# TheClimateCorporation/photon-ml

Measured on AMD Instinct MI355X. Metric: examples/sec/node, logistic L-BFGS 1B×1M-sparse, higher is better.
Workload: dtype bf16; 1 GPU; model=logistic_regression_l2_lbfgs, global_batch=125000000, rows_per_gpu=125000000, features=1000000, nnz_per_row=100, parallelism=dp1, optimizer_state=replicated, layout=tiled

## Files before the change

photon_ml_amd/data/synthetic.py:

```python
from __future__ import annotations

import math
from typing import Optional

import numpy as np
import scipy.sparse as sp
import torch

from ..constants import TaskType
from .matrix import LabeledData


INLIER_PROBABILITY = 0.90
INLIER_STANDARD_DEVIATION = 1e-3
OUTLIER_STANDARD_DEVIATION = 1.0
SAMPLE_KINDS = ("benign", "outlier", "invalid_features", "invalid_labels")


def draw_samples(task, kind: str, seed: int, size: int, dimensionality: int,
                 desired_sparsity: float = 0.1) -> LabeledData:
    task = TaskType.parse(task)
    if kind not in SAMPLE_KINDS:
        raise ValueError(f"unknown sample kind {kind!r}, expected one of {SAMPLE_KINDS}")
    rng = np.random.default_rng(5000 * seed)
    n, d = int(size), int(dimensionality)
    u = rng.random(n)
    binary = task in (TaskType.LOGISTIC_REGRESSION, TaskType.SMOOTHED_HINGE_LOSS_LINEAR_SVM)
    if kind == "invalid_labels":
        y = np.array([np.inf, -np.inf, np.nan])[rng.integers(0, 3, n)]
        x0 = 0.1 + 0.9 * u
    elif binary:
        y = (rng.random(n) <= 0.5).astype(np.float64)
        x0 = np.where(y == 1.0, 1.0, -1.0) * (0.1 + 0.9 * u)
    elif task == TaskType.POISSON_REGRESSION:
        y = 1.0 + 10.0 * u
        x0 = (np.log(y) + rng.normal(size=n) * INLIER_STANDARD_DEVIATION) / np.log(11.0)
    elif kind == "benign":
        y = 2.0 * u - 1.0
        x0 = y + rng.normal(size=n) * INLIER_STANDARD_DEVIATION
    else:
        y = 1.0 + u
        x0 = y - 1.0 + rng.normal(size=n) * OUTLIER_STANDARD_DEVIATION
    tail_end = d - 3 if kind == "invalid_features" else d
    mask = rng.random((n, max(tail_end - 1, 0))) < desired_sparsity
    rows, cols = np.nonzero(mask)
    cols = cols + 1
    k = rows.size
    if kind in ("benign", "invalid_labels"):
        vals = 2.0 * (rng.random(k) - 0.5)
    else:
        inlier = rng.random(k) < INLIER_PROBABILITY
        if kind == "outlier":
            bad = np.where(rng.random(k) < 0.5, 1.0, -1.0)
        else:
            bad = np.array([np.nan, np.inf, -np.inf])[rng.integers(0, 3, k)]
        vals = np.where(inlier, rng.normal(size=k) * INLIER_STANDARD_DEVIATION, bad)
    r_all = [np.arange(n), rows]
    c_all = [np.zeros(n, np.int64), cols]
    v_all = [x0, vals]
    if kind == "invalid_features":
        for j, v in zip((d - 3, d - 2, d - 1), (np.nan, np.inf, -np.inf)):
            r_all.append(np.arange(n))
            c_all.append(np.full(n, j))
            v_all.append(np.full(n, v))
    x = sp.csr_matrix((np.concatenate(v_all), (np.concatenate(r_all), np.concatenate(c_all))), shape=(n, d))
    x.sort_indices()
    return LabeledData(x, y)


def generate_glm_data(task, n_rows: int, n_features: int, density: float = 0.2, seed: int = 7,
                      intercept: bool = True, noise: float = 1e-3, kind: str = "benign"):
    task = TaskType.parse(task)
    rng = np.random.default_rng(seed)
    d_feat = n_features - (1 if intercept else 0)
    x = sp.random(n_rows, d_feat, density=density, format="csr", random_state=seed,
                  data_rvs=lambda k: rng.uniform(-1, 1, size=k))
    if kind == "outlier":
        x.data *= np.where(rng.random(x.data.size) < 0.01, 1e3, 1.0)
    if intercept:
        x = sp.hstack([x, np.ones((n_rows, 1))], format="csr")
    w = rng.normal(size=n_features)
    z = x @ w
    if task == TaskType.LOGISTIC_REGRESSION or task == TaskType.SMOOTHED_HINGE_LOSS_LINEAR_SVM:
        y = (rng.random(n_rows) < 1.0 / (1.0 + np.exp(-z))).astype(np.float64)
    elif task == TaskType.POISSON_REGRESSION:
        w *= 0.2
        z = x @ w
        y = rng.poisson(np.exp(np.clip(z, -20, 5))).astype(np.float64)
    else:
        y = z + rng.normal(scale=noise, size=n_rows)
    if kind == "invalid":
        y[0] = np.nan
    return LabeledData(x, y), w


def zipf_cdf(n: int, s: float, device) -> torch.Tensor:
    k = torch.arange(1, n + 1, dtype=torch.float64, device=device)
    p = k.pow(-s)
    c = torch.cumsum(p, 0)
    return (c / c[-1]).to(torch.float32)


def generate_device_shard(n_rows: int, n_features: int, nnz_per_row: int, device="cuda", precision: str = "bf16",
                          seed: int = 1234567890, chunk_rows: int = 1 << 20, zipf_s: float = 1.1,
                          task=TaskType.LOGISTIC_REGRESSION, rank: int = 0, progress=None, layout: str = "auto"):
    from ..ops.device import DeviceGLMData, SegChunk, VAL_DTYPE, resolve_layout
    from ..ops.tiled import TLFwdChunk, TLTChunk, shard_tall

    dev = torch.device(device)
    prec = {"bf16": 0, "f32": 1, "f64": 2}[precision]
    vdt = VAL_DTYPE[prec]
    n_fields = nnz_per_row - 1
    if n_fields < 1:
        raise ValueError("nnz_per_row must be >= 2 (intercept + >= 1 field)")
    fs = (n_features - 1) // n_fields
    if fs < 1:
        raise ValueError("not enough features for the requested nnz per row")
    layout = resolve_layout(layout, n_features, chunk_rows)
    cdf = zipf_cdf(fs, zipf_s, dev)
    field_base = (torch.arange(n_fields, device=dev, dtype=torch.int32) * fs)
    gen = torch.Generator(device=dev)
    gen.manual_seed(seed + 7919 * rank)
    starts = list(range(0, n_rows, chunk_rows)) + [n_rows]
    k = nnz_per_row
    raw = []
    counts = torch.zeros(n_features, dtype=torch.int64, device=dev)
    for ci, (a, b) in enumerate(zip(starts[:-1], starts[1:])):
        m = b - a
        u = torch.rand((m, n_fields), generator=gen, device=dev)
        rank_ = torch.searchsorted(cdf, u).clamp_(max=fs - 1).to(torch.int32)
        del u
        idx = torch.empty((m, k), dtype=torch.int32, device=dev)
        idx[:, :n_fields] = rank_ + field_base
        idx[:, n_fields] = n_features - 1
        del rank_
        val = torch.empty((m, k), dtype=torch.float32, device=dev)
        val[:, :n_fields] = torch.rand((m, n_fields), generator=gen, device=dev) + 0.5
        val[:, n_fields] = 1.0
        idx = idx.reshape(-1)
        counts += torch.bincount(idx.to(torch.int64), minlength=n_features)
        raw.append((idx, val.to(vdt).reshape(-1)))
        if (m + 1) * k >= 2 ** 31:
            raise ValueError("chunk too large for int32 offsets: lower chunk_rows")
    import torch.distributed as dist
    from ..parallel.dist import is_dist
    if is_dist():
        cc = counts if dist.get_backend() == "nccl" else counts.cpu()
        dist.all_reduce(cc)
        counts = cc.to(dev)
    old_of_new = torch.argsort(counts, descending=True, stable=True)
    new_of_old = torch.empty_like(old_of_new)
    new_of_old[old_of_new] = torch.arange(n_features, device=dev)
    new_of_old32 = new_of_old.to(torch.int32)
    del counts
    csr, csc = [], []
    from ..ops.tiled import shard_t_config
    cbits, item_entries = shard_t_config(n_rows * k, n_rows, n_features, chunk_rows)
    for ci, ((a, b), (idx, val)) in enumerate(zip(zip(starts[:-1], starts[1:]), raw)):
        m = b - a
        idx = new_of_old32[idx.to(torch.int64)]
        if layout == "tiled":
            rp = torch.arange(0, (m + 1) * k, k, dtype=torch.int64, device=dev)
            col = idx.to(torch.int64)
            del idx
            csr.append(TLFwdChunk(rp, col, val, n_features, tall=shard_tall(n_features, min(chunk_rows, n_rows))))
            csc.append(TLTChunk(rp, col, val, n_features, chunk_rows, cbits=cbits, item_entries=item_entries))
            raw[ci] = None
            del col, val, rp
            if progress is not None:
                progress(ci + 1, len(starts) - 1)
            continue
        seg_ptr = np.arange(0, (m + 1) * k, k, dtype=np.int64).astype(np.int32)
        csr.append(SegChunk(seg_ptr, idx, val, dev, forward=True))
        perm = torch.argsort(idx, stable=True)
        cidx = (perm // k).to(torch.int32)
        cval = val[perm]
        colptr = torch.zeros(n_features + 1, dtype=torch.int64, device=dev)
        colptr[1:] = torch.cumsum(torch.bincount(idx.to(torch.int64), minlength=n_features), 0)
        del perm
        csc.append(SegChunk(colptr.cpu().numpy().astype(np.int32), cidx, cval, dev))
        raw[ci] = None
        del cidx, cval, colptr, idx, val
        if progress is not None:
            progress(ci + 1, len(starts) - 1)
    y = torch.zeros(n_rows, dtype=torch.float32, device=dev)
    data = DeviceGLMData(csr, csc, starts, y, torch.zeros_like(y), torch.ones_like(y), n_features, precision, dev,
                         old_of_new)
    wgen = torch.Generator(device=dev)
    wgen.manual_seed(seed)
    w_true = torch.randn(n_features, generator=wgen, device=dev, dtype=torch.float64) * 0.3
    w_true[torch.rand(n_features, generator=wgen, device=dev) < 0.5] = 0.0
    w_true[-1] = -1.0
    z = data.margins(w_true)
    p = torch.sigmoid(z)
    task = TaskType.parse(task)
    if task == TaskType.LOGISTIC_REGRESSION:
        yy = (torch.rand(n_rows, generator=gen, device=dev, dtype=torch.float64) < p).to(torch.float32)
    elif task == TaskType.POISSON_REGRESSION:
        yy = torch.poisson(torch.exp(z.clamp(max=5.0)) * 0.2, generator=gen).to(torch.float32)
    else:
        yy = (z + 0.1 * torch.randn(n_rows, generator=gen, device=dev, dtype=torch.float64)).to(torch.float32)
    data.y.copy_(yy.to(data.vdt))
    return data, w_true


def _device_csr_to_host(counts: torch.Tensor, cols: torch.Tensor, vals: torch.Tensor, n_cols: int) -> sp.csr_matrix:
    indptr = torch.zeros(counts.numel() + 1, dtype=torch.int64, device=counts.device)
    torch.cumsum(counts, 0, out=indptr[1:])
    x = sp.csr_matrix((vals.cpu().numpy(), cols.to(torch.int32).cpu().numpy(), indptr.cpu().numpy()),
                      shape=(counts.numel(), n_cols))
    x.has_canonical_format = True
    return x


def generate_game_bench_data_device(n_entities: int, rows_per_entity: int, re_dim: int = 100, re_nnz: int = 10,
                                    fe_dim: int = 100_000, fe_nnz: int = 30, re_vocab: int = 1 << 20, seed: int = 7,
                                    entity_offset: int = 0, task: str = "LOGISTIC_REGRESSION", pool: str = "random",
                                    int_ids: bool = False, sizes: str = "uniform", size_alpha: float = 1.3,
                                    max_rows: int = 20000, device="cuda", label_bias: float = 0.0,
                                    heavy_rows=()):
    from ..data.game_data import GameData
    dev = torch.device(device)
    gen = torch.Generator(device=dev)
    gen.manual_seed(int(seed))
    rnd = lambda *shape: torch.rand(shape, generator=gen, device=dev, dtype=torch.float64)
    if sizes == "powerlaw":
        if pool == "exact":
            raise ValueError("pool='exact' needs equal entity sizes")
        u = rnd(n_entities)
        target = n_entities * rows_per_entity
        xm = float(rows_per_entity) * (size_alpha - 1) / size_alpha
        for _ in range(30):
            cnt = torch.clamp(torch.ceil(xm * u ** (-1.0 / size_alpha)), max=max_rows).to(torch.int64)
            tot = int(cnt.sum())
            if abs(tot - target) <= 0.001 * target:
                break
            xm *= target / tot
    elif sizes == "uniform":
        cnt = torch.full((n_entities,), rows_per_entity, dtype=torch.int64, device=dev)
    else:
        raise ValueError(f"unknown entity size law {sizes!r}")
    if len(heavy_rows):
        cnt[:len(heavy_rows)] = torch.tensor([int(r) for r in heavy_rows], dtype=torch.int64, device=dev)
    n = int(cnt.sum())
    ent_sorted = torch.repeat_interleave(torch.arange(n_entities, device=dev), cnt, output_size=n)
    perm = torch.randperm(n, generator=gen, device=dev)
    ent = ent_sorted[perm]
    p = torch.arange(1, fe_dim, device=dev, dtype=torch.float64) ** -1.1
    cdf = torch.cumsum(p, 0)
    cdf /= cdf[-1].clone()
    fcol = torch.searchsorted(cdf, rnd(n, fe_nnz)).clamp_(max=fe_dim - 2)
    fcol, _ = torch.sort(fcol, dim=1)
    keep = torch.ones_like(fcol, dtype=torch.bool)
    keep[:, 1:] = fcol[:, 1:] != fcol[:, :-1]
    fval = rnd(n, fe_nnz) + 0.5
    fcol = torch.cat([fcol, torch.full((n, 1), fe_dim - 1, device=dev, dtype=fcol.dtype)], 1)
    fval = torch.cat([fval, torch.ones(n, 1, device=dev, dtype=torch.float64)], 1)
    keep = torch.cat([keep, torch.ones(n, 1, device=dev, dtype=torch.bool)], 1)
    xg = _device_csr_to_host(keep.sum(1), fcol[keep], fval[keep], fe_dim)
    wg = torch.randn(fe_dim, generator=gen, device=dev, dtype=torch.float64) * 0.2
    wg[-1] = -0.5
    zg = (fval * wg[fcol] * keep).sum(1)
    del fcol, fval, keep
    if pool == "exact":
        if re_nnz > re_dim:
            raise ValueError("pool='exact' needs re_nnz <= re_dim")
        start = torch.zeros(n_entities, dtype=torch.int64, device=dev)
        torch.cumsum(cnt[:-1], 0, out=start[1:])
        within = perm - start[ent]
        slot = (within[:, None] * re_nnz + torch.arange(re_nnz, device=dev)[None, :]) % re_dim
        del within, start
    else:
        slot = torch.randint(0, re_dim, (n, re_nnz), generator=gen, device=dev)
    del ent_sorted, perm
    gid = ent + entity_offset
    base = (gid * 2654435761) % (re_vocab - 1)
    rcol = (base[:, None] + slot * 40503) % (re_vocab - 1)
    rval = torch.randn(n, re_nnz, generator=gen, device=dev, dtype=torch.float64)
    wgen = torch.Generator(device=dev)
    wgen.manual_seed(int(seed) + 1)
    w_slot = torch.randn(re_dim, generator=wgen, device=dev, dtype=torch.float64) * 0.5
    rcol, order = torch.sort(rcol, dim=1)
    slot = torch.gather(slot, 1, order)
    rval = torch.gather(rval, 1, order)
    del order
    rkeep = torch.ones_like(rcol, dtype=torch.bool)
    rkeep[:, 1:] = rcol[:, 1:] != rcol[:, :-1]
    zr = (rval * w_slot[slot] * rkeep).sum(1) + 0.3 * torch.sin(gid.to(torch.float64))
    del slot
    rcol = torch.cat([rcol, torch.full((n, 1), re_vocab - 1, device=dev, dtype=rcol.dtype)], 1)
    rval = torch.cat([rval, torch.ones(n, 1, device=dev, dtype=torch.float64)], 1)
    rkeep = torch.cat([rkeep, torch.ones(n, 1, device=dev, dtype=torch.bool)], 1)
    xr = _device_csr_to_host(rkeep.sum(1), rcol[rkeep], rval[rkeep], re_vocab)
    del rcol, rval, rkeep
    z = zg + zr
    task = TaskType.parse(task)
    if task == TaskType.LOGISTIC_REGRESSION:
        y = (rnd(n) < torch.sigmoid(z + label_bias)).to(torch.float64)
    elif task == TaskType.POISSON_REGRESSION:
        y = torch.poisson(torch.exp(torch.clamp(z * 0.3, -10, 3)), generator=gen)
    else:
        y = z + 0.1 * torch.randn(n, generator=gen, device=dev, dtype=torch.float64)
    gid_h = gid.cpu().numpy()
    ids = gid_h.copy() if int_ids else np.char.add("e", gid_h.astype(str)).astype(object)
    return GameData(y.cpu().numpy(), {"global": xg, "entity": xr}, {"entityId": ids})


def generate_game_bench_data(n_entities: int, rows_per_entity: int, re_dim: int = 100, re_nnz: int = 10,
                             fe_dim: int = 100_000, fe_nnz: int = 30, re_vocab: int = 1 << 20, seed: int = 7,
                             entity_offset: int = 0, task: str = "LOGISTIC_REGRESSION", pool: str = "random",
                             int_ids: bool = False, sizes: str = "uniform", size_alpha: float = 1.3,
                             max_rows: int = 20000):
    from ..data.game_data import GameData
    rng = np.random.default_rng(seed)
    if sizes == "powerlaw":
        if pool == "exact":
            raise ValueError("pool='exact' needs equal entity sizes")
        u = rng.random(n_entities)
        target = n_entities * rows_per_entity
# ... 74 lines not shown
```

photon_ml_amd/ops/csrc/glm_kernels.hip:

```cpp

#include <hip/hip_runtime.h>
#include <stdint.h>
#include <math.h>
#include <algorithm>
#include <type_traits>

#define NB 4096
#define NTHREADS 256
#define VEC 8
#define MAXSEG 1024

#define LAUNCH_CHECK()                                         \
  do {                                                         \
    hipError_t e_ = hipGetLastError();                         \
    if (e_ != hipSuccess) return (int)e_;                      \
  } while (0)

enum LossId { LOSS_LOGISTIC = 0, LOSS_POISSON = 1, LOSS_SQUARED = 2, LOSS_HINGE = 3 };
enum FwdMode { FWD_MARGIN = 0, FWD_VALUE_GRAD = 1, FWD_HV = 2, FWD_DZZ = 3, FWD_LS = 4 };

struct bf16x8 { uint4 u; };

template <typename VT, typename AT> struct Loader;
template <> struct Loader<uint16_t, float> {
// ... 989 lines not shown
  if (live && !live[b]) return;
  const int* q = blk + 8 * b;
  const unsigned long long* pc = ptrs + 6 * q[0];
  const TLNarrow nar = {(const uint16_t*)pc[2], (const void*)pc[3], (const int*)pc[4], (const int*)pc[5]};
  tl_fwd_block<VT, XT, RT, AT, MAXR, U, NW, P>(b, q[1], q[2], q[3], q[4], q[6], q[7], rbits, (const uint32_t*)pc[0],
                                              (const VT*)pc[1], nar, x + q[5], a, stats, acc, red);
}

#define TL_TALL_BITS 12
#define TL_TALL_SUB 10
template <typename VT, typename XT, typename RT, int PT>
__device__ __forceinline__ void tl_fwd_tall_block(int row_lo, int nrows, int e_lo, int e_hi,
                                                  const int* __restrict__ nq ,
                                                  const uint32_t* __restrict__ pack, const VT* __restrict__ val,
                                                  const TLNarrow& nar, const XT* __restrict__ x,
                                                  const FwdArgs<XT, RT>& a, double* __restrict__ stats, double* acc) {
  constexpr int NW = 4;
  for (int i = threadIdx.x; i < (1 << TL_TALL_BITS); i += NW * 64) acc[i] = 0.0;
  __syncthreads();
  const int w = __builtin_amdgcn_readfirstlane(threadIdx.x >> 6);
  const int n_lo = w == 0 ? nq[0] : nq[1 + w], n_hi = w == NW - 1 ? nq[1] : nq[2 + w];
  if (n_hi > n_lo)
    tl_narrow<VT, XT, double, false, 1, (PT >= 5 ? 4 : 2)>(nar, n_lo, n_hi, TL_TALL_SUB, x, acc + (w << TL_TALL_SUB));
  __syncthreads();
  if (w == 0) {
    if (PT == 6) tl_stream_ring<VT, XT, double, false, 1, 5, 2>(pack, val, x, e_lo, e_hi, TL_TALL_BITS, acc, nar.wbase);
    else if (PT == 5) tl_stream_ring<VT, XT, double, false, 1, 3, 1>(pack, val, x, e_lo, e_hi, TL_TALL_BITS, acc, nar.wbase);
    else tl_stream_ring<VT, XT, double, false, 1, 2, 0>(pack, val, x, e_lo, e_hi, TL_TALL_BITS, acc, nar.wbase);
  }
  __syncthreads();
  const int t = ((w & 1) << 6) | (threadIdx.x & 63);
  double Fk[2], Sk[2];
#pragma unroll
  for (int j = 0; j < 2; ++j) {
    const int k0 = ((w >> 1) * 2 + j) << TL_TALL_SUB;
    const int nk = min(nrows - k0, 1 << TL_TALL_SUB);
    double F = 0.0, S = 0.0;
    for (int r = k0 + t; r < k0 + nk; r += 128) {
      const int s = row_lo + r;
      fwd_finish(a, s, acc[r], fwd_prefetch(a, s), F, S);
    }
    Fk[j] = F; Sk[j] = S;
  }
  if (stats) {
    const int sb = nq[5];
#pragma unroll
    for (int j = 0; j < 2; ++j) { Fk[j] = wave_sum(Fk[j]); Sk[j] = wave_sum(Sk[j]); }
    __syncthreads();
    if ((threadIdx.x & 63) == 0) {
#pragma unroll
      for (int j = 0; j < 2; ++j) {
        const int k = (w >> 1) * 2 + j;
        acc[4 * k + 2 * (w & 1)] = Fk[j]; acc[4 * k + 2 * (w & 1) + 1] = Sk[j];
      }
    }
    __syncthreads();
    const int k = threadIdx.x;
    if (k < 4 && (k << TL_TALL_SUB) < nrows) {
      double F = 0.0, S = 0.0;
      for (int i = 0; i < 2; ++i) { F += acc[4 * k + 2 * i]; S += acc[4 * k + 2 * i + 1]; }
      stats[2 * (sb + k)] = F; stats[2 * (sb + k) + 1] = S;
    }
  }
}

template <typename VT, typename XT, typename RT, int PT>
__global__ __launch_bounds__(256) void tl_fwd_tall_kernel(const int* __restrict__ blk,
                                                           const uint32_t* __restrict__ pack,
                                                           const VT* __restrict__ val, TLNarrow nar,
                                                           const XT* __restrict__ x, FwdArgs<XT, RT> a,
                                                           double* __restrict__ stats,
                                                           const unsigned char* __restrict__ live) {
  __shared__ double acc[1 << TL_TALL_BITS];
  const int b = blockIdx.x;
  if (live && !live[b]) return;
  const int* q = blk + 10 * b;
  tl_fwd_tall_block<VT, XT, RT, PT>(q[0], q[1], q[2], q[3], q + 4, pack, val, nar, x, a, stats, acc);
}

template <typename VT, typename XT, typename RT, int PT>
__global__ __launch_bounds__(256) void tl_fwd_tall_multi_kernel(const int* __restrict__ blk,
                                                                 const unsigned long long* __restrict__ ptrs,
                                                                 const XT* __restrict__ x, FwdArgs<XT, RT> a,
                                                                 double* __restrict__ stats,
                                                                 const unsigned char* __restrict__ live) {
  __shared__ double acc[1 << TL_TALL_BITS];
  const int b = blockIdx.x;
  if (live && !live[b]) return;
  const int* q = blk + 12 * b;
  const unsigned long long* pc = ptrs + 6 * q[0];
  const TLNarrow nar = {(const uint16_t*)pc[2], (const void*)pc[3], (const int*)pc[4], (const int*)pc[5]};
  tl_fwd_tall_block<VT, XT, RT, PT>(q[1], q[2], q[3], q[4], q + 6, (const uint32_t*)pc[0], (const VT*)pc[1], nar,
                                    x + q[5], a, stats, acc);
}

template <typename VT, typename XT, typename AT, bool SQ, int MAXR, int U, int NW, int P>
__device__ __forceinline__ void tl_t_item(int tile, int e_lo, int e_hi, int part, int n_lo, int n_hi, int cbits,
                                          const uint32_t* __restrict__ pack, const VT* __restrict__ val,
                                          const TLNarrow& nar, const XT* __restrict__ x, double* __restrict__ G,
                                          int dim, double* __restrict__ parts, AT (*acc)[MAXR]) {
  const int C = 1 << cbits;
  for (int i = threadIdx.x; i < C; i += NW * 64)
#pragma unroll
    for (int w = 0; w < NW; ++w) acc[w][i] = AT(0);
  __syncthreads();
  if (n_hi > n_lo)
    tl_narrow<VT, XT, AT, SQ, NW, (P >= 5 ? 4 : 2)>(nar, n_lo, n_hi, cbits, x, acc[threadIdx.x >> 6]);
  tl_stream<VT, XT, AT, SQ, U, NW, P>(pack, val, x, e_lo, e_hi, cbits, acc[threadIdx.x >> 6], nar.wbase);
  __syncthreads();
  const int c0 = tile << cbits;
  for (int c = threadIdx.x; c < C; c += NW * 64) {
    double s = static_cast<double>(acc[0][c]);
#pragma unroll
    for (int w = 1; w < NW; ++w) s += static_cast<double>(acc[w][c]);
    if (part < 0) {
      if (c0 + c < dim) G[c0 + c] += s;
    } else {
      parts[(size_t)part * C + c] = s;
    }
  }
}

template <typename VT, typename XT, typename AT, bool SQ, int MAXR, int U, int NW, int P>
__global__ __launch_bounds__(NW * 64) void tl_t_kernel(const int* __restrict__ items, int cbits,
                                                        const uint32_t* __restrict__ pack,
                                                        const VT* __restrict__ val, TLNarrow nar,
                                                        const XT* __restrict__ x, double* __restrict__ G, int dim,
                                                        double* __restrict__ parts,
                                                        const unsigned char* __restrict__ live) {
  __shared__ AT acc[NW][MAXR];
  if (live && !live[blockIdx.x]) return;
  const int* q = items + 6 * blockIdx.x;
  tl_t_item<VT, XT, AT, SQ, MAXR, U, NW, P>(q[0], q[1], q[2], q[3], q[4], q[5], cbits, pack, val, nar, x, G, dim,
                                            parts, acc);
}

template <typename VT, typename XT, typename AT, bool SQ, int MAXR, int U, int NW, int P>
__global__ __launch_bounds__(NW * 64) void tl_t_multi_kernel(const int* __restrict__ items, int cbits,
                                                              const unsigned long long* __restrict__ ptrs,
                                                              const XT* __restrict__ x, double* __restrict__ G,
                                                              int dim, double* __restrict__ parts,
                                                              const unsigned char* __restrict__ live,
                                                              const int* __restrict__ gate) {
  __shared__ AT acc[NW][MAXR];
  if (gate && *gate == 0) return;
  if (live && !live[blockIdx.x]) return;
  const int* q = items + 8 * blockIdx.x;
  const unsigned long long* pc = ptrs + 6 * q[0];
  const TLNarrow nar = {(const uint16_t*)pc[2], (const void*)pc[3], (const int*)pc[4], (const int*)pc[5]};
  tl_t_item<VT, XT, AT, SQ, MAXR, U, NW, P>(q[1], q[2], q[3], q[4], q[6], q[7], cbits, (const uint32_t*)pc[0],
                                            (const VT*)pc[1], nar, x + q[5], G, dim, parts, acc);
}

__device__ __forceinline__ double rows_sum64(const double* __restrict__ src, int C, int r0, int r1, int c,
                                             double* sh) {
  const int w = threadIdx.x >> 6, lane = threadIdx.x & 63;
  const int n = r1 - r0;
  const int q0 = r0 + (n * w) / 4, q1 = r0 + (n * (w + 1)) / 4;
  double s0 = 0.0, s1 = 0.0, s2 = 0.0, s3 = 0.0;
  if (c < C) {
    int r = q0;
    for (; r + 3 < q1; r += 4) {
      s0 += src[(size_t)r * C + c];
      s1 += src[(size_t)(r + 1) * C + c];
      s2 += src[(size_t)(r + 2) * C + c];
      s3 += src[(size_t)(r + 3) * C + c];
    }
    for (; r < q1; ++r) s0 += src[(size_t)r * C + c];
  }
  sh[w * 64 + lane] = (s0 + s1) + (s2 + s3);
  __syncthreads();
  return (sh[lane] + sh[64 + lane]) + (sh[128 + lane] + sh[192 + lane]);
}

__global__ __launch_bounds__(NTHREADS) void tl_t_combine1_kernel(const int* __restrict__ cu, int cbits,
                                                                 const double* __restrict__ parts,
                                                                 double* __restrict__ l1,
                                                                 const unsigned char* __restrict__ live_mt) {
  __shared__ double sh[NTHREADS];
  const int u = blockIdx.x;
  if (live_mt && !live_mt[cu[3 * u]]) return;
  const int C = 1 << cbits;
  const int c = blockIdx.y * 64 + (threadIdx.x & 63);
  const double s = rows_sum64(parts, C, cu[3 * u + 1], cu[3 * u + 2], c, sh);
  if (threadIdx.x < 64 && c < C) l1[(size_t)u * C + c] = s;
}

__global__ __launch_bounds__(NTHREADS) void tl_t_combine2_kernel(const int* __restrict__ mt_tiles,
                                                                 const int* __restrict__ mt_ptr, int cbits,
                                                                 const double* __restrict__ l1,
                                                                 double* __restrict__ G, int dim,
                                                                 const unsigned char* __restrict__ live_mt) {
  __shared__ double sh[NTHREADS];
  const int t = blockIdx.x;
  if (live_mt && !live_mt[t]) return;
  const int C = 1 << cbits;
  const int c = blockIdx.y * 64 + (threadIdx.x & 63);
  const double s = rows_sum64(l1, C, mt_ptr[t], mt_ptr[t + 1], c, sh);
  if (threadIdx.x < 64 && c < C) {
    const int col = (mt_tiles[t] << cbits) + c;
    if (col < dim) G[col] += s;
  }
}

struct TLFwdDesc { const int* blk; int nblk; int rbits; const uint32_t* pack; const void* val; int il; TLNarrow nar;
                  const unsigned char* live; int tbits; };
struct TLFwdMultiDesc { const int* blk; int nblk; int rbits; const unsigned long long* ptrs; int il;
                       const unsigned char* live; int tbits; };
struct TLTDesc {
  const int* items; int nitems; int cbits; const uint32_t* pack; const void* val;
  const int* mt_tiles; const int* mt_ptr; int nmt; int dim;
  const int* cu; int ncu;
  int nparts_total;
  int il;
  TLNarrow nar;
  const unsigned char* live;
  const unsigned char* live_mt;
};
struct TLTMultiDesc {
  const int* items; int nitems; int cbits; const unsigned long long* ptrs;
  const int* mt_tiles; const int* mt_ptr; int nmt; int dim;
  const int* cu; int ncu; int nparts_total; int il;
  const unsigned char* live;
  const unsigned char* live_mt;
};

static int g_ablate = 0;
static double* g_ls_z0 = nullptr;
static double g_ls_t0 = 0.0, g_ls_tpend = 0.0;
static const int* g_gate = nullptr;
static const double* g_ls_z0_in = nullptr;
static const double* g_ls_zd_in = nullptr;
template <typename A>
static inline A& with_ls_in(A& a) {
  a.z0_in = g_ls_z0_in ? g_ls_z0_in : g_ls_z0;
  a.zd_in = g_ls_zd_in ? g_ls_zd_in : a.z_out;
  return a;
}
template <typename XT>
static FwdArgs<XT, XT> fwd_args(int mode, int loss, double shift, const void* y, const void* off, const void* wt,
                                void* coef, void* dzz, double* z_out, int with_offset) {
  FwdArgs<XT, XT> a{mode, loss, shift, (const XT*)y, (const XT*)off, (const XT*)wt, (XT*)coef, (XT*)dzz, z_out,
                    with_offset, g_ablate, 0, g_ls_z0, g_ls_t0, g_ls_tpend};
  return with_ls_in(a);
}
template <typename F>
static int with_prec(int prec, F f) {
  if (prec == 2) return f(double{}, double{});
  if (prec == 1) return f(float{}, float{});
  return f(uint16_t{}, float{});
}
template <typename F>
static int with_prec_sq(int prec, int square, F f) {
  return with_prec(prec, [&](auto vt, auto xt) {
    return square ? f(vt, xt, std::true_type{}) : f(vt, xt, std::false_type{});
  });
}
static int g_tl_acc64 = 1;
static int g_tl_waves = 4;
static int g_tl_waves_t = 4;
static int g_tl_pipe = 0;
static int g_tl_pipe_t = 0;
static int g_rs_variant = 5;
static int g_tl_deep = 0;
static int g_tl_deep_t = 0;

#ifdef PML_TL_EXPERIMENT
constexpr bool TL_EXPERIMENT = true;
#else
constexpr bool TL_EXPERIMENT = false;
#endif

template <typename AT_, int MAXR_> struct TLAcc { using AT = AT_; static constexpr int MAXR = MAXR_; };
template <int NW_, int P_> struct TLPipe { static constexpr int NW = NW_, P = P_; };

template <typename XT> static inline int tl_maxbits() { return sizeof(XT) == 8 ? 11 : TL_MAXBITS; }
template <typename XT, typename F>
static int tl_with_acc(int bits, F f) {
  if (bits < 1 || bits > tl_maxbits<XT>()) return -22;
  if constexpr (sizeof(XT) != 8) {
    if (bits == 12) { f(TLAcc<float, 4096>{}); return 0; }
    if constexpr (TL_EXPERIMENT) {
      if (!g_tl_acc64) {
        if (bits <= 10) f(TLAcc<float, 1024>{}); else f(TLAcc<float, 2048>{});
        return 0;
      }
    }
  }
  if (bits <= 10) f(TLAcc<double, 1024>{}); else f(TLAcc<double, 2048>{});
  return 0;
}

template <int NW_PROD, int ALT_P, typename F>
static void tl_with_pipe(int il, int waves, int deep, int pipe, F f) {
  if constexpr (!TL_EXPERIMENT) {
    if (il) f(TLPipe<NW_PROD, 3>{}); else f(TLPipe<NW_PROD, 0>{});
  } else {
    auto with_p = [&](auto nw) {
      constexpr int NW = decltype(nw)::value;
      if (il) {
        if (deep == 2) f(TLPipe<NW, 6>{}); else if (deep) f(TLPipe<NW, 5>{}); else f(TLPipe<NW, 3>{});
      } else if (pipe == ALT_P) f(TLPipe<NW, ALT_P>{});
      else f(TLPipe<NW, 0>{});
    };
    if (waves == 2) with_p(std::integral_constant<int, 2>{}); else with_p(std::integral_constant<int, 4>{});
  }
}

#define TL_TALL_P 6
template <typename XT, typename F>
static int tl_with_tall(int tbits, int rbits, int il, F f) {
  if constexpr (sizeof(XT) == 8) {
    return -22;
  } else {
    if (tbits != TL_TALL_BITS || rbits != TL_TALL_SUB || !il) return -22;
    if constexpr (TL_EXPERIMENT) {
      if (g_tl_deep == 2) f(std::integral_constant<int, 6>{});
      else if (g_tl_deep) f(std::integral_constant<int, 5>{});
      else f(std::integral_constant<int, 3>{});
    } else {
      f(std::integral_constant<int, TL_TALL_P>{});
    }
    return 0;
  }
}

template <typename VT, typename XT, typename RT>
static int tl_fwd_impl(const TLFwdDesc* c, const void* x, FwdArgs<XT, RT> a, double* stats, hipStream_t st) {
  if (c->nblk <= 0) return 0;
  if (c->tbits) {
    const int rt = tl_with_tall<XT>(c->tbits, c->rbits, c->il, [&](auto pt) {
      hipLaunchKernelGGL((tl_fwd_tall_kernel<VT, XT, RT, decltype(pt)::value>), dim3(c->nblk), dim3(256), 0, st,
                         c->blk, c->pack, (const VT*)c->val, c->nar, (const XT*)x, a, stats, c->live);
    });
    if (rt) return rt;
    LAUNCH_CHECK();
    return 0;
  }
  const int rc = tl_with_acc<XT>(c->rbits, [&](auto acc) {
    tl_with_pipe<2, 1>(c->il, g_tl_waves, g_tl_deep, g_tl_pipe, [&](auto pipe) {
      using A = decltype(acc); using Q = decltype(pipe);
      hipLaunchKernelGGL((tl_fwd_kernel<VT, XT, RT, typename A::AT, A::MAXR, 2, Q::NW, Q::P>), dim3(c->nblk),
                         dim3(Q::NW * 64), 0, st, c->blk, c->rbits, c->pack, (const VT*)c->val, c->nar, (const XT*)x,
                         a, stats, c->live);
    });
  });
  if (rc) return rc;
  LAUNCH_CHECK();
  return 0;
}

template <typename VT, typename XT, typename RT>
static int tl_fwd_multi_impl(const TLFwdMultiDesc* c, const void* x, FwdArgs<XT, RT> a, double* stats,
                             hipStream_t st) {
  if (c->nblk <= 0) return 0;
  if (c->tbits) {
    const int rt = tl_with_tall<XT>(c->tbits, c->rbits, c->il, [&](auto pt) {
      hipLaunchKernelGGL((tl_fwd_tall_multi_kernel<VT, XT, RT, decltype(pt)::value>), dim3(c->nblk), dim3(256), 0,
                         st, c->blk, c->ptrs, (const XT*)x, a, stats, c->live);
    });
    if (rt) return rt;
    LAUNCH_CHECK();
    return 0;
  }
  const int rc = tl_with_acc<XT>(c->rbits, [&](auto acc) {
    tl_with_pipe<2, 2>(c->il, g_tl_waves, g_tl_deep, g_tl_pipe, [&](auto pipe) {
      using A = decltype(acc); using Q = decltype(pipe);
      hipLaunchKernelGGL((tl_fwd_multi_kernel<VT, XT, RT, typename A::AT, A::MAXR, 2, Q::NW, Q::P>), dim3(c->nblk),
                         dim3(Q::NW * 64), 0, st, c->blk, c->rbits, c->ptrs, (const XT*)x, a, stats, c->live);
    });
  });
  if (rc) return rc;
  LAUNCH_CHECK();
  return 0;
}

template <typename Desc>
static int tl_t_combine(const Desc* c, double* G, double* parts, hipStream_t st) {
  if (c->nmt <= 0) return 0;
  const int C = 1 << c->cbits;
  double* l1 = parts + (size_t)c->nparts_total * C;
  hipLaunchKernelGGL(tl_t_combine1_kernel, dim3(c->ncu, (C + 63) / 64), dim3(NTHREADS), 0, st, c->cu, c->cbits,
                     parts, l1, c->live_mt);
  LAUNCH_CHECK();
  hipLaunchKernelGGL(tl_t_combine2_kernel, dim3(c->nmt, (C + 63) / 64), dim3(NTHREADS), 0, st,
                     c->mt_tiles, c->mt_ptr, c->cbits, l1, G, c->dim, c->live_mt);
  LAUNCH_CHECK();
  return 0;
}

template <typename VT, typename XT, bool SQ>
static int tl_t_impl(const TLTDesc* c, const void* x, double* G, double* parts, hipStream_t st) {
  if (c->nitems <= 0) return 0;
  const int rc = tl_with_acc<XT>(c->cbits, [&](auto acc) {
    tl_with_pipe<4, 1>(c->il, g_tl_waves_t, g_tl_deep_t, g_tl_pipe_t, [&](auto pipe) {
      using A = decltype(acc); using Q = decltype(pipe);
      hipLaunchKernelGGL((tl_t_kernel<VT, XT, typename A::AT, SQ, A::MAXR, 2, Q::NW, Q::P>), dim3(c->nitems),
                         dim3(Q::NW * 64), 0, st, c->items, c->cbits, c->pack, (const VT*)c->val, c->nar, (const XT*)x,
                         G, c->dim, parts, c->live);
    });
  });
  if (rc) return rc;
  LAUNCH_CHECK();
  return tl_t_combine(c, G, parts, st);
}

template <typename VT, typename XT, bool SQ>
static int tl_t_multi_impl(const TLTMultiDesc* c, const void* x, double* G, double* parts, hipStream_t st) {
  if (c->nitems <= 0) return 0;
  const int rc = tl_with_acc<XT>(c->cbits, [&](auto acc) {
    tl_with_pipe<4, 2>(c->il, g_tl_waves_t, g_tl_deep_t, g_tl_pipe_t, [&](auto pipe) {
      using A = decltype(acc); using Q = decltype(pipe);
      hipLaunchKernelGGL((tl_t_multi_kernel<VT, XT, typename A::AT, SQ, A::MAXR, 2, Q::NW, Q::P>), dim3(c->nitems),
                         dim3(Q::NW * 64), 0, st, c->items, c->cbits, c->ptrs, (const XT*)x, G, c->dim, parts, c->live,
                         g_gate);
    });
  });
  if (rc) return rc;
  LAUNCH_CHECK();
  return tl_t_combine(c, G, parts, st);
}

template <typename VT> __device__ __forceinline__ void cs_vals(const typename TLVals<VT>::Raw& raw, double* v) {
  typename TLValT<VT>::T t[TL_VEC];
  TLVals<VT>::get(raw, t);
#pragma unroll
  for (int k = 0; k < TL_VEC; ++k) v[k] = static_cast<double>(t[k]);
}

template <typename VT, int NW, typename F>
__device__ __forceinline__ void cs_for_each(const int* __restrict__ q, int cbits, const uint32_t* __restrict__ pack,
                                            const VT* __restrict__ val, const TLNarrow& nar, int il, F f) {
  typedef typename TLVals<VT>::Raw Raw;
  const int lane = threadIdx.x & 63;
  const int w = __builtin_amdgcn_readfirstlane(threadIdx.x >> 6);
  const uint32_t smask = (1u << cbits) - 1u;
  const int e_lo = q[1], e_hi = q[2], n_lo = q[4], n_hi = q[5];
  double v[TL_VEC];
  {
    const int nr = n_hi - n_lo;
    const int r0 = n_lo + (int)(((long long)nr * w) / NW), r1 = n_lo + (int)(((long long)nr * (w + 1)) / NW);
    bool fused = false;
    if constexpr (sizeof(VT) == 2) fused = nar.val == nullptr;
    for (int r = r0; r < r1; ++r) {
      const size_t e = (size_t)r * TL_ROUND + lane * TL_VEC;
      v2u pk;
      if (fused) {
        if constexpr (sizeof(VT) == 2) {
          const v4u rec = ldg_nt((const v4u*)(nar.pack + 2 * e));
          pk.x = rec.x; pk.y = rec.y;
          v2u u; u.x = rec.z; u.y = rec.w;
          cs_vals<VT>(u, v);
        }
      } else {
        pk = ldg_nt((const v2u*)(nar.pack + e));
        const Raw raw = TLVals<VT>::load((const VT*)nar.val + e);
        cs_vals<VT>(raw, v);
      }
      f(pk.x & 0xffffu & smask, v[0]);
      f((pk.x >> 16) & smask, v[1]);
      f(pk.y & 0xffffu & smask, v[2]);
      f((pk.y >> 16) & smask, v[3]);
    }
  }
  if (il) {
    const int n = e_hi - e_lo;
    const int nr = (n + TL_ROUND - 1) / TL_ROUND;
    const int r0 = (int)(((long long)nr * w) / NW), r1 = (int)(((long long)nr * (w + 1)) / NW);
    for (int r = r0; r < r1; ++r) {
      const size_t e = (size_t)e_lo + (size_t)r * TL_ROUND + lane * TL_VEC;
      const v4u pk = ldg_nt((const v4u*)(pack + e));
      const Raw raw = TLVals<VT>::load(val + e);
      cs_vals<VT>(raw, v);
      const int j = r * TL_ROUND + lane;
#pragma unroll
      for (int k = 0; k < TL_VEC; ++k)
        if (j + 64 * k < n) f(pk[k] & smask, v[k]);
    }
  } else {
    const int lo = e_lo & ~(TL_VEC - 1);
    const int nr = (e_hi - lo + TL_ROUND - 1) / TL_ROUND;
    const int r0 = (int)(((long long)nr * w) / NW), r1 = (int)(((long long)nr * (w + 1)) / NW);
    for (int r = r0; r < r1; ++r) {
      const int e = lo + r * TL_ROUND + lane * TL_VEC;
      if (e >= e_hi) continue;
      const v4u pk = ldg_nt((const v4u*)(pack + e));
      const Raw raw = TLVals<VT>::load(val + e);
      cs_vals<VT>(raw, v);
#pragma unroll
      for (int k = 0; k < TL_VEC; ++k)
        if (e + k >= e_lo && e + k < e_hi) f(pk[k] & smask, v[k]);
    }
  }
}

template <typename VT, int MAXR, int NW>
__global__ __launch_bounds__(NW * 64) void tl_colsum_kernel(const int* __restrict__ items, int cbits,
                                                            const uint32_t* __restrict__ pack,
                                                            const VT* __restrict__ val, TLNarrow nar, int il,
                                                            int which, double* __restrict__ G, int dim,
                                                            double* __restrict__ parts) {
  __shared__ double acc[NW][MAXR];
  const int* q = items + 6 * blockIdx.x;
  const int C = 1 << cbits;
  for (int i = threadIdx.x; i < C; i += NW * 64)
#pragma unroll
    for (int w = 0; w < NW; ++w) acc[w][i] = 0.0;
  __syncthreads();
  double* mine = acc[threadIdx.x >> 6];
  cs_for_each<VT, NW>(q, cbits, pack, val, nar, il, [&](uint32_t slot, double v) {
    const double t = which == 0 ? v : which == 1 ? v * v : which == 2 ? fabs(v) : 1.0;
    atomicAdd(&mine[slot], t);
  });
  __syncthreads();
  const int c0 = q[0] << cbits, part = q[3];
  for (int c = threadIdx.x; c < C; c += NW * 64) {
    double s = acc[0][c];
#pragma unroll
    for (int w = 1; w < NW; ++w) s += acc[w][c];
    if (part < 0) {
      if (c0 + c < dim) G[c0 + c] += s;
    } else {
      parts[(size_t)part * C + c] = s;
    }
  }
}

template <typename VT, int MAXR>
__global__ __launch_bounds__(NTHREADS) void tl_colminmax_kernel(const int* __restrict__ items, int cbits,
                                                                const uint32_t* __restrict__ pack,
                                                                const VT* __restrict__ val, TLNarrow nar, int il,
                                                                double* __restrict__ mx, double* __restrict__ mn,
                                                                int dim) {
  __shared__ double smx[MAXR];
  __shared__ double smn[MAXR];
  const int* q = items + 6 * blockIdx.x;
  const int C = 1 << cbits;
  for (int i = threadIdx.x; i < C; i += NTHREADS) { smx[i] = -INFINITY; smn[i] = INFINITY; }
  __syncthreads();
  cs_for_each<VT, TL_WAVES>(q, cbits, pack, val, nar, il, [&](uint32_t slot, double v) {
    __hip_atomic_fetch_max(&smx[slot], v, __ATOMIC_RELAXED, __HIP_MEMORY_SCOPE_WORKGROUP);
    __hip_atomic_fetch_min(&smn[slot], v, __ATOMIC_RELAXED, __HIP_MEMORY_SCOPE_WORKGROUP);
  });
  __syncthreads();
  const int c0 = q[0] << cbits;
  for (int c = threadIdx.x; c < C; c += NTHREADS) {
    if (c0 + c >= dim || smx[c] == -INFINITY) continue;
    __hip_atomic_fetch_max(&mx[c0 + c], smx[c], __ATOMIC_RELAXED, __HIP_MEMORY_SCOPE_AGENT);
    __hip_atomic_fetch_min(&mn[c0 + c], smn[c], __ATOMIC_RELAXED, __HIP_MEMORY_SCOPE_AGENT);
  }
}

template <typename VT>
static int tl_colstats_impl(const TLTDesc* c, double* const* sums, double* mx, double* mn, double* parts,
                            hipStream_t st) {
  if (c->cbits < 1 || c->cbits > (sizeof(VT) == 8 ? 11 : TL_MAXBITS)) return -22;
  if (c->nitems <= 0) return 0;
  for (int which = 0; which < 4; ++which) {
    auto launch = [&](auto maxr, auto nw) {
      constexpr int MAXR = decltype(maxr)::value, NW = decltype(nw)::value;
      hipLaunchKernelGGL((tl_colsum_kernel<VT, MAXR, NW>), dim3(c->nitems), dim3(NW * 64), 0, st, c->items, c->cbits,
                         c->pack, (const VT*)c->val, c->nar, c->il, which, sums[which], c->dim, parts);
    };
    if (c->cbits <= 10) launch(std::integral_constant<int, 1024>{}, std::integral_constant<int, 4>{});
    else if (c->cbits == 11) launch(std::integral_constant<int, 2048>{}, std::integral_constant<int, 4>{});
    else if constexpr (sizeof(VT) != 8) launch(std::integral_constant<int, 4096>{}, std::integral_constant<int, 2>{});
    LAUNCH_CHECK();
    const int rc = tl_t_combine(c, sums[which], parts, st);
    if (rc) return rc;
  }
  auto launch_mm = [&](auto maxr) {
    constexpr int MAXR = decltype(maxr)::value;
    hipLaunchKernelGGL((tl_colminmax_kernel<VT, MAXR>), dim3(c->nitems), dim3(NTHREADS), 0, st, c->items, c->cbits,
                       c->pack, (const VT*)c->val, c->nar, c->il, mx, mn, c->dim);
  };
  if (c->cbits <= 11) launch_mm(std::integral_constant<int, 2048>{});
  else if constexpr (sizeof(VT) != 8) launch_mm(std::integral_constant<int, 4096>{});
  LAUNCH_CHECK();
  return 0;
}

__global__ __launch_bounds__(NTHREADS) void segdot_kernel(const double* __restrict__ a, const double* __restrict__ b,
                                                          int mode, const long long* __restrict__ ptr, int nseg,
                                                          double* __restrict__ out) {
  const int wv = (blockIdx.x * NTHREADS + threadIdx.x) >> 6;
  const int lane = threadIdx.x & 63;
  if (wv >= nseg) return;
  const long long lo = ptr[wv], hi = ptr[wv + 1];
  double s = 0.0;
  for (long long i = lo + lane; i < hi; i += 64) {
    const double x = a[i];
    s += mode == 0 ? x * b[i] : (mode == 1 ? x : fabs(x));
  }
  s = wave_sum(s);
  if (lane == 0) out[wv] = s;
}

#define SEGDOT_C 4096
__device__ __forceinline__ int seg_of(const long long* __restrict__ ptr, int nseg, long long i) {
  int lo = 0, hi = nseg - 1;
  while (lo < hi) {
    const int mid = (lo + hi + 1) >> 1;
    if (ptr[mid] <= i) lo = mid; else hi = mid - 1;
  }
  return lo;
}

__device__ __forceinline__ double seg_range_sum(const double* __restrict__ a, const double* __restrict__ b, int mode,
                                                long long lo, long long hi, int lane) {
  double s = 0.0;
  for (long long i = lo + lane; i < hi; i += 64) {
    const double x = a[i];
    s += mode == 0 ? x * b[i] : (mode == 1 ? x : fabs(x));
  }
  return wave_sum(s);
}

__global__ __launch_bounds__(NTHREADS) void segdot_long_kernel(const double* __restrict__ a,
                                                               const double* __restrict__ b, int mode,
                                                               const long long* __restrict__ ptr, int nseg,
                                                               int nseg_w, long long n, double* __restrict__ head,
                                                               double* __restrict__ tail, double* __restrict__ out) {
  const int wv = (blockIdx.x * NTHREADS + threadIdx.x) >> 6;
  const int lane = threadIdx.x & 63;
  if (wv < nseg_w) {
    if (wv >= nseg) return;
    const long long lo = ptr[wv], hi = ptr[wv + 1];
    if (hi - lo > SEGDOT_C) return;
    const double s = seg_range_sum(a, b, mode, lo, hi, lane);
    if (lane == 0) out[wv] = s;
    return;
  }
  const long long w = wv - nseg_w;
  const long long c0 = w * SEGDOT_C, c1 = c0 + SEGDOT_C < n ? c0 + SEGDOT_C : n;
  if (c0 >= n) return;
  const int s0 = seg_of(ptr, nseg, c0), s1 = seg_of(ptr, nseg, c1 - 1);
  double h = 0.0, t = 0.0;
  if (ptr[s0 + 1] - ptr[s0] > SEGDOT_C) h = seg_range_sum(a, b, mode, c0, ptr[s0 + 1] < c1 ? ptr[s0 + 1] : c1, lane);
  if (s1 != s0 && ptr[s1 + 1] - ptr[s1] > SEGDOT_C) t = seg_range_sum(a, b, mode, ptr[s1], c1, lane);
  if (lane == 0) { head[w] = h; tail[w] = t; }
}

__global__ __launch_bounds__(NTHREADS) void segdot_combine_kernel(const long long* __restrict__ ptr, int nseg,
                                                                  const double* __restrict__ head,
                                                                  const double* __restrict__ tail,
                                                                  double* __restrict__ out) {
  const int s = blockIdx.x * NTHREADS + threadIdx.x;
  if (s >= nseg) return;
  const long long lo = ptr[s], hi = ptr[s + 1];
  if (hi - lo <= SEGDOT_C) return;
  const long long w0 = lo / SEGDOT_C, w1 = (hi - 1) / SEGDOT_C;
  double acc = lo == w0 * SEGDOT_C ? head[w0] : tail[w0];
  for (long long w = w0 + 1; w <= w1; ++w) acc += head[w];
  out[s] = acc;
}

template <typename T>
__global__ __launch_bounds__(NTHREADS) void seg_expand_kernel(const long long* __restrict__ ptr, int nseg,
                                                              const T* __restrict__ src, T* __restrict__ out) {
  const int e = (blockIdx.x * NTHREADS + threadIdx.x) >> 6;
  const int lane = threadIdx.x & 63;
  if (e >= nseg) return;
  const long long lo = ptr[e], hi = ptr[e + 1];
  const T v = src[e];
  for (long long i = lo + lane; i < hi; i += 64) out[i] = v;
}

__global__ __launch_bounds__(NTHREADS) void seg_cg_step_kernel(const long long* __restrict__ ptr, int nseg,
                                                               double* __restrict__ step, double* __restrict__ r,
                                                               double* __restrict__ d, const double* __restrict__ Hd,
                                                               double* __restrict__ rtr, unsigned char* __restrict__ on,
                                                               const double* __restrict__ delta, double l2) {
  const int e = (blockIdx.x * NTHREADS + threadIdx.x) >> 6;
  const int lane = threadIdx.x & 63;
  if (e >= nseg || !on[e]) return;
  const long long lo = ptr[e], hi = ptr[e + 1];
  double dhd = 0.0, std_ = 0.0, sts = 0.0, dtd = 0.0;
  for (long long i = lo + lane; i < hi; i += 64) {
    const double di = d[i], si = step[i];
    dhd += di * (Hd[i] + l2 * di);
    std_ += si * di;
    sts += si * si;
    dtd += di * di;
  }
  dhd = wave_sum(dhd); std_ = wave_sum(std_); sts = wave_sum(sts); dtd = wave_sum(dtd);
  const double rt = rtr[e];
  const double alpha = rt / (dhd == 0.0 ? 1.0 : dhd);
  double tn = 0.0;
  for (long long i = lo + lane; i < hi; i += 64) {
    const double t = step[i] + alpha * d[i];
    tn += t * t;
  }
  tn = wave_sum(tn);
  const double dl = delta[e];
  const bool hit = sqrt(tn > 0.0 ? tn : 0.0) > dl;
  double a = alpha;
  if (hit) {
    const double dsq = dl * dl;
    const double q = std_ * std_ + dtd * (dsq - sts);
    const double rad = sqrt(q > 0.0 ? q : 0.0);
    const double den1 = std_ + rad, den2 = dtd;
    a = std_ >= 0.0 ? (dsq - sts) / (den1 > 1e-300 ? den1 : 1e-300) : (rad - std_) / (den2 > 1e-300 ? den2 : 1e-300);
  }
  double rn = 0.0;
  for (long long i = lo + lane; i < hi; i += 64) {
    const double di = d[i];
    step[i] = step[i] + a * di;
    const double ri = r[i] - a * (Hd[i] + l2 * di);
    r[i] = ri;
// ... 2085 lines not shown
```

photon_ml_amd/ops/device.py:

```python
from __future__ import annotations

import ctypes
import os
import threading
from dataclasses import dataclass
from typing import List, Optional, Sequence

import numpy as np
import scipy.sparse as sp
import torch

from ..data.matrix import LabeledData
from .native import SegChunkDesc, check, require_glm_lib, stream_handle
from .reference import GLMComputable
from .tiled import DEFAULT_ITEM_ENTRIES, TLFwdChunk, TLTChunk, shard_tall, tl_supported
from ..utils.timing import phase, trace_range

H2D_GATE = threading.Event()

LAYOUTS = ("auto", "tiled", "segmented")


def resolve_layout(layout: str, dim: int, chunk_rows: int) -> str:
    import os
    if layout == "auto":
        layout = os.environ.get("PML_LAYOUT", "auto")
    if layout not in LAYOUTS:
        raise ValueError(f"unknown layout {layout}")
    if layout == "auto":
        layout = "tiled" if tl_supported(dim, chunk_rows) else "segmented"
    if layout == "tiled" and not tl_supported(dim, chunk_rows):
        raise ValueError(f"tiled layout cannot pack dim={dim} with chunk_rows={chunk_rows}")
    return layout

PRECISIONS = {"bf16": 0, "f32": 1, "f64": 2}
VAL_DTYPE = {0: torch.bfloat16, 1: torch.float32, 2: torch.float64}
VEC_DTYPE = {0: torch.float32, 1: torch.float32, 2: torch.float64}

FWD_MARGIN, FWD_VALUE_GRAD, FWD_HV, FWD_DZZ, FWD_LS = 0, 1, 2, 3, 4


def _pad8(n: int) -> int:
    return ((n + 7) // 8) * 8 + 8


def _ptr(t: Optional[torch.Tensor]) -> Optional[int]:
    return None if t is None else t.data_ptr()


class SegChunk:

    def __init__(self, seg_ptr: np.ndarray, idx: torch.Tensor, val: torch.Tensor, device, nb: Optional[int] = None,
                 maxseg: Optional[int] = None, forward: bool = False):
        lib = require_glm_lib()
        seg_ptr = np.ascontiguousarray(seg_ptr, dtype=np.int32)
        nseg = len(seg_ptr) - 1
        nb = nb or lib.pml_nb()
        maxseg = maxseg or (lib.pml_maxseg_fwd() if forward else lib.pml_maxseg())
        nblk, nlong, npart = ctypes.c_int(), ctypes.c_int(), ctypes.c_int()
        check(lib.pml_build_blocks(seg_ptr.ctypes.data, nseg, nb, maxseg, None, ctypes.byref(nblk), None, None,
                                   ctypes.byref(nlong), ctypes.byref(npart)), "count blocks")
        blk = np.zeros(max(5 * nblk.value, 5), dtype=np.int32)
        long_seg = np.zeros(max(nlong.value, 1), dtype=np.int32)
        long_ptr = np.zeros(nlong.value + 1, dtype=np.int32)
        check(lib.pml_build_blocks(seg_ptr.ctypes.data, nseg, nb, maxseg, blk.ctypes.data, ctypes.byref(nblk),
                                   long_seg.ctypes.data, long_ptr.ctypes.data, ctypes.byref(nlong),
                                   ctypes.byref(npart)), "build blocks")
        self.nseg, self.nblk, self.nlong, self.npart = nseg, nblk.value, nlong.value, npart.value
        self.nnz = int(seg_ptr[-1])
        dev = torch.device(device)
        self.seg_ptr = torch.from_numpy(seg_ptr).to(dev)
        self.blk = torch.from_numpy(blk).to(dev)
        self.long_seg = torch.from_numpy(long_seg).to(dev)
        self.long_ptr = torch.from_numpy(long_ptr).to(dev)
        n_pad = _pad8(self.nnz)
        if idx.numel() < n_pad:
            idx = torch.cat([idx.to(dev, torch.int32), torch.zeros(n_pad - idx.numel(), dtype=torch.int32, device=dev)])
        if val.numel() < n_pad:
            val = torch.cat([val.to(dev), torch.zeros(n_pad - val.numel(), dtype=val.dtype, device=dev)])
        self.idx = idx.contiguous()
        self.val = val.contiguous()
        self.desc = SegChunkDesc(self.blk.data_ptr(), self.nblk, self.seg_ptr.data_ptr(), self.nseg,
                                 self.idx.data_ptr(), self.val.data_ptr(), self.long_seg.data_ptr(),
                                 self.long_ptr.data_ptr(), self.nlong, self.npart)

    kind = "seg"

    @property
    def nstats(self) -> int:
        return self.nblk

    @property
    def parts_needed(self) -> int:
        return self.npart

    def nbytes(self) -> int:
        return sum(t.numel() * t.element_size() for t in (self.seg_ptr, self.blk, self.long_seg, self.long_ptr,
                                                           self.idx, self.val))


MASK_STATS = [] if os.environ.get("PML_TRON_STATS") == "1" else None

NARROW_FILTER_BELOW = float(os.environ.get("PML_DS_NARROW_FILTER_BELOW", "0.23"))

OFFSET_SHIFT_CACHE = os.environ.get("PML_OFFSET_SHIFT_CACHE", "1") != "0"


class VecKey:

    __slots__ = ("src", "ver")

    def __init__(self, w: torch.Tensor):
        self.src = w
        self.ver = w._version

    @property
    def shape(self):
        return self.src.shape

    def matches(self, w: torch.Tensor) -> bool:
        if w is self.src and w._version == self.ver:
            return True
        if self.src._version != self.ver or self.src.shape != w.shape:
            return False
        return bool(torch.equal(self.src, w.to(self.src.device, self.src.dtype)))


def _window_align(chunk_rows: int, precision: str) -> int:
    from .tiled import t_bits
    cb = t_bits(chunk_rows, precision == "f64")
    return 1 << cb if cb is not None else 1


class DeviceGLMData(GLMComputable):

    def __init__(self, csr: List[SegChunk], csc: List[SegChunk], row_starts: Sequence[int], y, offsets, weights,
                 dim: int, precision: str = "f64", device="cuda", old_of_new: Optional[torch.Tensor] = None):
        self.lib = require_glm_lib()
        self.device = torch.device(device)
        if self.device.type == "cuda":
            from .native import check_lds_add_order
            check_lds_add_order(self.device)
        self.prec = PRECISIONS[precision]
        self.precision = precision
        self.vdt = VEC_DTYPE[self.prec]
        self.csr, self.csc = csr, csc
        self.row_starts = list(row_starts)
        self.n_rows = self.row_starts[-1]
        self.dim = int(dim)
        rdt = self.vdt
        self.y = torch.as_tensor(y, device=self.device).to(rdt).contiguous()
        self.o = torch.as_tensor(offsets, device=self.device).to(rdt).contiguous()
        self.wt = torch.as_tensor(weights, device=self.device).to(rdt).contiguous()
        n = self.n_rows
        self.coef = torch.zeros(max(n, 1), dtype=rdt, device=self.device)
        self.dzz = torch.zeros(max(n, 1), dtype=rdt, device=self.device)
        self.track_hessian = False
        self._dzz_key: Optional[torch.Tensor] = None
        self._dzz_shift = None
        self.layout = "tiled" if csr and csr[0].kind == "tl" else "segmented"
        self.col_lo = [0] * len(csr)
        self.blk_off = np.cumsum([0] + [c.nstats for c in csr]).tolist()
        self.long_off = np.cumsum([0] + [getattr(c, "nlong", 0) for c in csr]).tolist()
        self.stats = torch.zeros(2 * max(self.blk_off[-1], 1), dtype=torch.float64, device=self.device)
        self.long_stats = torch.zeros(2 * max(self.long_off[-1], 1), dtype=torch.float64, device=self.device)
        maxpart = max([c.parts_needed for c in csr + csc] + [1])
        self.parts = torch.zeros(maxpart, dtype=torch.float64, device=self.device)
        self.red_scratch = torch.zeros(512, dtype=torch.float64, device=self.device)
        self.out2 = torch.zeros(2, dtype=torch.float64, device=self.device)
        self.n_passes = 0
        self.old_of_new = None if old_of_new is None else old_of_new.to(self.device, torch.int64)
        if self.old_of_new is not None:
            self.new_of_old = torch.empty_like(self.old_of_new)
            self.new_of_old[self.old_of_new] = torch.arange(self.dim, device=self.device)
        if os.environ.get("PML_CHECK_KERNEL_INPUTS", "0") == "1":
            self.validate()

    def validate(self):
        from .tiled import il_phys
        for c, (f, t) in enumerate(zip(self.csr, self.csc)):
            if f.kind != "tl":
                continue
            m = self.row_starts[c + 1] - self.row_starts[c]
            b = f.blk.cpu().to(torch.int64)
            if f.nblk and (int(b[:, 0].min()) < 0 or int((b[:, 0] + b[:, 1]).max()) > m
                           or int(b[:, 1].max()) > (1 << f.ubits)):
                raise ValueError(f"chunk {c}: forward block rows out of range")
            q = 256 if f.il else 4
            end = b[:, 2] + (b[:, 3] - b[:, 2] + q - 1) // q * q if f.il else (b[:, 3] + 3) // 4 * 4
            if f.nblk and (int(b[:, 2].min()) < 0 or int(end.max()) > f.pack.numel()):
                raise ValueError(f"chunk {c}: forward block window outside the stream")
            if f.il and f.nblk and bool((b[:, 2] % 256 != 0).any()):
                raise ValueError(f"chunk {c}: interleaved forward windows not round-aligned")
            ncols = int(self.dim) - self.col_lo[c]
            self._validate_narrow(c, f, b, ncols, "forward")
            pk, _ = f.logical()
            p = pk.cpu().to(torch.int64)
            wb = getattr(f, "wbase", None)
            if wb is not None and wb.numel() and int(wb.min()) < 0:
                raise ValueError(f"chunk {c}: negative wide-round base")
            if p.numel() and int((p >> f.ubits).max()) >= ncols:
                raise ValueError(f"chunk {c}: forward gather index >= column window")
            counts = f.unit_counts().cpu()
            blk_rows = torch.repeat_interleave(b[:, 1], counts)
            if p.numel() and bool(((p & ((1 << f.ubits) - 1)) >= blk_rows).any()):
                raise ValueError(f"chunk {c}: forward LDS slot >= block rows")
            it = t.items.cpu().to(torch.int64)
            if t.nitems:
                if int(it[:, 1].min()) < 0 or int(it[:, 2].max()) > t.pack.numel():
                    raise ValueError(f"chunk {c}: transpose item window outside the stream")
                if int(it[:, 3].max()) >= max(t.nparts, 1) and t.nparts:
                    raise ValueError(f"chunk {c}: transpose partial-row slot out of range")
                self._validate_narrow(c, t, it, m, "transpose")
                tp, _ = t.logical()
                q = tp.cpu().to(torch.int64) & 0xFFFFFFFF
                if q.numel() and int((q >> t.cbits).max()) >= m:
                    raise ValueError(f"chunk {c}: transpose gather row >= chunk rows")
                cols = (torch.repeat_interleave(it[:, 0], t.unit_counts().cpu()) << t.cbits) + (q & ((1 << t.cbits) - 1))
                if q.numel() and int(cols.max()) >= t.dim:
                    raise ValueError(f"chunk {c}: transpose column >= dim")
        if self.parts.numel() < max([c.parts_needed for c in self.csr + self.csc] + [1]):
            raise ValueError("partial-row scratch too small")
        self._validate_multi()
        return True

    def _validate_multi(self):
        mb = getattr(self, "_multi", None)
        if mb is not None and not isinstance(mb, str):
            t = self._multi_blk.cpu().to(torch.int64)
            for c, ch in enumerate(self.csr):
                r = t[t[:, 0] == c]
                if ch.il and r.shape[0] and (int(r[:, 3].min()) < 0 or int((r[:, 3] + (r[:, 4] - r[:, 3] + 255) // 256 * 256).max())
                                   > ch.pack.numel() or int(r[:, 7].max()) > ch.nbase.numel() * (ch.n_narrow_rounds > 0)):
                    raise ValueError(f"chunk {c}: shard-wide forward table outside the chunk's streams")
        mt = getattr(self, "_multi_t", None)
        if mt is not None and not isinstance(mt, str):
            if self.parts.numel() < mt.parts_needed:
                raise ValueError("partial-row scratch too small for the shard-wide transpose")
            t = mt.items.cpu().to(torch.int64)
            for c, ch in enumerate(self.csc):
                r = t[t[:, 0] == c]
                if ch.il and r.shape[0] and (int(r[:, 2].min()) < 0 or int((r[:, 2] + (r[:, 3] - r[:, 2] + 255) // 256 * 256).max())
                                   > ch.pack.numel() or int(r[:, 7].max()) > ch.nbase.numel() * (ch.n_narrow_rounds > 0)):
                    raise ValueError(f"chunk {c}: shard-wide transpose table outside the chunk's streams")

    @staticmethod
    def _validate_narrow(c: int, ch, table: torch.Tensor, xlen: int, what: str):
        if table.shape[0] == 0:
            return
        n_lo, n_hi = table[:, 4], table[:, 5]
        nrounds = ch.nbase.numel() if ch.n_narrow_rounds else 0
        if bool((n_hi < n_lo).any()) or int(n_hi.max()) > nrounds or bool((n_lo[1:] != n_hi[:-1]).any()):
            raise ValueError(f"chunk {c}: {what} narrow round ranges inconsistent")
        if nrounds:
            base = ch.nbase.cpu().to(torch.int64)
            if ch.npack.numel() < 256 * nrounds or ch.nval.numel() < 256 * nrounds:
                raise ValueError(f"chunk {c}: {what} narrow stream shorter than its rounds")
            if ch.fused and (ch.nrec.numel() < 512 * nrounds or ch.val.element_size() != 2
                             or not ch.nrec.is_contiguous()):
                raise ValueError(f"chunk {c}: {what} fused narrow records need 2-byte values, 16 B per lane and round")
            if int(base.min()) < 0 or int(base.max()) + 64 > xlen:
                raise ValueError(f"chunk {c}: {what} narrow key window outside the gathered vector")

    @staticmethod
    def from_labeled(data: LabeledData, device="cuda", precision: str = "f64", chunk_rows: int = 1 << 20,
                     relabel: bool = True, layout: str = "auto", item_entries: Optional[int] = None,
                     col_windows: bool = False):
        if col_windows:
            relabel = False
        prec = PRECISIONS[precision]
        vdt = VAL_DTYPE[prec]
        dev = torch.device(device)
        x = data.x.tocsr()
        n, d = x.shape
        if dev.type == "cuda" and n and resolve_layout(layout, d, chunk_rows) == "tiled":
            return DeviceGLMData._from_labeled_device(x, data, dev, precision, chunk_rows, relabel, item_entries,
                                                      col_windows)
        if hasattr(x, "to_scipy"):
            x = x.to_scipy()
        old_of_new = None
        from ..parallel.dist import is_dist
        shared = relabel and is_dist() and not col_windows
        if shared or (relabel and x.nnz > 0):
            counts = np.bincount(x.indices, minlength=d).astype(np.int64)
            if shared:
                import torch.distributed as tdist
                from ..parallel.sharding import comm_device
                ct = torch.from_numpy(counts).to(comm_device())
                tdist.all_reduce(ct)
                counts = ct.cpu().numpy()
            old_of_new_np = np.argsort(-counts, kind="stable")
            new_of_old_np = np.empty(d, dtype=np.int64)
            new_of_old_np[old_of_new_np] = np.arange(d)
            x = sp.csr_matrix((x.data, new_of_old_np[x.indices], x.indptr), shape=x.shape)
            old_of_new = torch.from_numpy(old_of_new_np)
        starts = list(range(0, n, chunk_rows)) + [n]
        if n == 0:
            starts = [0, 0]
        csr, csc = [], []
        col_lo = []
        wins = []
        align = _window_align(chunk_rows, precision)
        for a, b in zip(starts[:-1], starts[1:]):
            xc = x[a:b]
            if col_windows and xc.nnz:
                lo, hi = int(xc.indices.min()), int(xc.indices.max()) + 1
                lo -= lo % align
            else:
                lo, hi = 0, d
            wins.append((lo, hi))
        dmax = max([hi - lo for lo, hi in wins] + [1])
        layout = resolve_layout(layout, dmax, chunk_rows)
        cbits = None
        if layout == "tiled" and not col_windows and item_entries is None:
            from .tiled import shard_t_config
            cbits, item_entries = shard_t_config(int(x.nnz), n, d, chunk_rows)
        for (a, b), (lo, hi) in zip(zip(starts[:-1], starts[1:]), wins):
            xc = x[a:b]
            col_lo.append(lo)
            if lo != 0 or hi != d:
                xc = sp.csr_matrix((xc.data, xc.indices - lo, xc.indptr), shape=(b - a, hi - lo))
            dc = hi - lo
            if layout == "tiled":
                rp = torch.from_numpy((xc.indptr - xc.indptr[0]).astype(np.int64)).to(dev)
                col = torch.from_numpy(xc.indices.astype(np.int64)).to(dev)
                val = torch.from_numpy(xc.data.astype(np.float64)).to(dev).to(vdt)
                csr.append(TLFwdChunk(rp, col, val, dc, tall=shard_tall(dmax, min(chunk_rows, n))))
                csc.append(TLTChunk(rp, col, val, dc, chunk_rows, cbits=cbits, item_entries=item_entries))
                continue
            sp_ = (xc.indptr - xc.indptr[0]).astype(np.int32)
            csr.append(SegChunk(sp_, torch.from_numpy(xc.indices.astype(np.int32)),
                                torch.from_numpy(xc.data.astype(np.float64)).to(vdt), dev, forward=True))
            xt = xc.tocsc()
            xt.sort_indices()
            xc = xc.copy()
            csc.append(SegChunk(xt.indptr.astype(np.int32), torch.from_numpy(xt.indices.astype(np.int32)),
                                torch.from_numpy(xt.data.astype(np.float64)).to(vdt), dev))
        out = DeviceGLMData(csr, csc, starts, torch.from_numpy(data.y), torch.from_numpy(data.offsets),
                            torch.from_numpy(data.weights), d, precision, dev, old_of_new)
        out.col_lo = col_lo
        return out

    @staticmethod
    def _from_labeled_device(x, data: LabeledData, dev, precision: str, chunk_rows: int, relabel: bool,
                             item_entries: Optional[int], col_windows: bool):
        n, d = x.shape
        with phase("tiled build: upload"):
            if isinstance(x.indptr, torch.Tensor):
                indptr, col, val = x.indptr.to(dev), x.indices.to(dev).to(torch.int64), x.data.to(dev)
            else:
                indptr = torch.from_numpy(np.ascontiguousarray(x.indptr, dtype=np.int64)).to(dev)
                col = torch.from_numpy(np.ascontiguousarray(x.indices)).to(dev).to(torch.int64)
                val = torch.from_numpy(np.ascontiguousarray(x.data)).to(dev)
        H2D_GATE.set()
        old_of_new = None
        from ..parallel.dist import is_dist
        shared = relabel and is_dist() and not col_windows
        relabel_phase = phase("tiled build: hottest-first relabel")
        relabel_phase.__enter__()
        if shared or (relabel and col.numel() > 0):
            from .native import key_histogram
            counts = key_histogram(col, d)
            if shared:
                import torch.distributed as tdist
                from ..parallel.sharding import comm_device
                ct = counts.to(comm_device())
                tdist.all_reduce(ct)
                counts = ct.to(dev)
            oon = torch.argsort(-counts, stable=True)
            non = torch.empty_like(oon)
            non[oon] = torch.arange(d, device=dev)
            col = non[col]
            old_of_new = (oon, non)
            del counts
        relabel_phase.__exit__(None, None, None)
        out = DeviceGLMData.from_device_csr(indptr, col, val, torch.from_numpy(data.y), torch.from_numpy(data.offsets),
                                            torch.from_numpy(data.weights), d, dev, precision, chunk_rows,
                                            item_entries=item_entries, col_windows=col_windows)
        if old_of_new is not None:
            out.old_of_new, out.new_of_old = old_of_new
        return out

    @staticmethod
    def from_device_csr(indptr: torch.Tensor, col: torch.Tensor, val: torch.Tensor, y, offsets, weights, dim: int,
                        device="cuda", precision: str = "f64", chunk_rows: int = 1 << 20,
                        item_entries: Optional[int] = None, col_windows: bool = False,
                        tall: Optional[bool] = None):
        dev = torch.device(device)
        vdt = VAL_DTYPE[PRECISIONS[precision]]
        indptr = indptr.to(dev, torch.int64)
        col = col.to(dev, torch.int64)
        n = indptr.numel() - 1
        starts = list(range(0, n, chunk_rows)) + [n] if n else [0, 0]
        ip = indptr[torch.tensor(starts, device=dev)].tolist()
        wins = []
        align = _window_align(chunk_rows, precision)
        for i in range(len(starts) - 1):
            ea, eb = ip[i], ip[i + 1]
            if col_windows and eb > ea:
                lo, hi = torch.aminmax(col[ea:eb])
                lo = int(lo)
                wins.append((lo - lo % align, int(hi) + 1))
            else:
                wins.append((0, dim))
        dmax = max([hi - lo for lo, hi in wins] + [1])
        if resolve_layout("auto", dmax, chunk_rows) != "tiled":
            raise ValueError(f"from_device_csr needs the tiled layout (window {dmax} columns)")
        cbits = None
        if not col_windows and item_entries is None:
            from .tiled import shard_t_config
            cbits, item_entries = shard_t_config(int(ip[-1] - ip[0]), n, dim, chunk_rows)
        csr, csc, col_lo = [], [], []
        chunk_phase = phase(f"tiled build: {len(wins)} chunk layouts")
        chunk_phase.__enter__()
        for i, (lo, hi) in enumerate(wins):
            a, b = starts[i], starts[i + 1]
            ea, eb = ip[i], ip[i + 1]
            rp = indptr[a:b + 1] - ea
            c = col[ea:eb] - lo if lo else col[ea:eb]
            v = val[ea:eb].to(dev).to(vdt)
            csr.append(TLFwdChunk(rp, c, v, hi - lo,
                                  tall=shard_tall(dmax, min(chunk_rows, n)) if tall is None else tall))
            csc.append(TLTChunk(rp, c, v, hi - lo, chunk_rows, cbits=cbits, item_entries=item_entries))
            col_lo.append(lo)
            del c, v
        chunk_phase.__exit__(None, None, None)
        out = DeviceGLMData(csr, csc, starts, y, offsets, weights, dim, precision, dev, None)
        out.col_lo = col_lo
        return out

    def nbytes(self) -> int:
        return sum(c.nbytes() for c in self.csr + self.csc)

    def row_sampled(self, keep: torch.Tensor) -> Optional["DeviceGLMData"]:
        from .tiled import RowCompaction, stream_ptr_table
        from .native import TLFwdMultiDesc
        if self.layout != "tiled" or not self.csr or not all(getattr(ch, "il", 0) for ch in self.csr + self.csc):
            return None
        if any(getattr(ch, "wbase", None) is not None for ch in self.csr):
            return None
        keep = keep.to(self.device, torch.uint8).contiguous()
        assert keep.numel() >= self.n_rows
        n = self.n_rows
        if getattr(self, "_multi", "unset") == "unset":
            self._build_multi()
        if getattr(self, "_multi_t", "unset") == "unset":
            self._build_multi_t()
        frac = float(keep[:n].sum()) / max(n, 1)
        filt = frac < NARROW_FILTER_BELOW
        jobs = []
        for c in range(len(self.csr)):
            kc = keep[self.row_starts[c]: self.row_starts[c + 1]]
            jobs.append(RowCompaction(self.csr[c], kc, True, filt))
            jobs.append(RowCompaction(self.csc[c], kc, False, filt))
        sizes = torch.stack([torch.stack([j.total, j.kept]) for j in jobs]).tolist()
        out = [j.finish(int(t), int(k)) for j, (t, k) in zip(jobs, sizes)]
        view = DeviceGLMData(out[0::2], out[1::2], self.row_starts, self.y, self.o, self.wt, self.dim,
                             self.precision, self.device, None)
        view.col_lo = list(self.col_lo)
        view.old_of_new = self.old_of_new
        if self.old_of_new is not None:
            view.new_of_old = self.new_of_old
        view.sampled_from = self
        view.kept_fraction = frac
        view._frob_sq = self.frob_sq()
        if getattr(self, "z_cache", None) is not None and getattr(self, "_z_key", None) is not None:
            view.enable_margin_cache()
            view.z_cache.copy_(self.z_cache)
            view.zd.copy_(self.zd)
            view._z_key, view._z_chain, view._tpend = self._z_key, self._z_chain, self._tpend
        if self._multi is not None:
            nb = self._multi_blk.clone()
            cb = torch.cat([ch.blk for ch in view.csr])
            nb[:, 3:5] = cb[:, 2:4]
            nb[:, 6:6 + min(cb.shape[1], 9) - 4] = cb[:, 4:9]
            view._multi_blk = nb
            view._multi_ptrs = stream_ptr_table(view.csr, self.device)
            view._multi = TLFwdMultiDesc(nb.data_ptr(), nb.shape[0], self._multi.rbits, view._multi_ptrs.data_ptr(),
                                         self._multi.il, tbits=self._multi.tbits)
        view._multi_t = None if self._multi_t is None else self._multi_t.restreamed(view.csc)
        gb = getattr(self, "_gbuckets", None)
        if gb is not None and gb[1] is not None:
            view._gbuckets = (gb[0], [(mt.restreamed(view.csc), c0, c1) for mt, c0, c1 in gb[1]])
        view.parts = self.parts
        if os.environ.get("PML_CHECK_KERNEL_INPUTS", "0") == "1":
            view.validate()
        return view

    def set_offsets_sum(self, base: torch.Tensor, part: torch.Tensor) -> bool:
        n = self.n_rows
        if not (n > 0 and base.is_cuda and part.is_cuda and base.dtype == part.dtype == torch.float64
                and base.numel() == part.numel() == n == self.o.numel() and base.is_contiguous()
                and part.is_contiguous() and base.device == self.o.device == part.device):
            return False
        from .native import offset_update
        zc = getattr(self, "z_cache", None)
        shift = (zc is not None and getattr(self, "_z_key", None) is not None and self._z_chain + 1 < self.LS_REFRESH
                 and getattr(self, "_masked", None) is None and OFFSET_SHIFT_CACHE)
        offset_update(base, part, self.o, zc[:n] if shift else None)
        if shift:
            self._z_chain += 1
            self._ls_t0 = None
        else:
            self._z_key = None
        self._step_base = None
        self._dzz_key = None
        return True

    def set_offsets(self, offsets):
        new = torch.as_tensor(offsets, device=self.device).to(self.vdt)
        zc = getattr(self, "z_cache", None)
        if (zc is not None and getattr(self, "_z_key", None) is not None and self._z_chain + 1 < self.LS_REFRESH
                and getattr(self, "_masked", None) is None and OFFSET_SHIFT_CACHE):
            n = self.n_rows
            zc[:n].add_(new[:n].to(torch.float64) - self.o[:n].to(torch.float64))
            self._z_chain += 1
            self._ls_t0 = None
        else:
            self._z_key = None
        self.o.copy_(new)
        self._step_base = None
        self._dzz_key = None

    def mark_weights_changed(self):
        self._dzz_key = None
        self._ls_t0 = None

    LS_REFRESH = 50

    def enable_margin_cache(self):
        if getattr(self, "z_cache", None) is None:
            n = max(self.n_rows, 1)
            self.z_cache = torch.zeros(n, dtype=torch.float64, device=self.device)
            self.zd = torch.zeros(n, dtype=torch.float64, device=self.device)
            self.ls_stats = torch.zeros(2 * 4096, dtype=torch.float64, device=self.device)
            self.ls_out = torch.zeros(2, dtype=torch.float64, device=self.device)
            self._z_key, self._z_chain, self._tpend, self._ls_t0 = None, 0, 0.0, None
        return True

    def _z_valid_for(self, w_eff, shift) -> bool:
        key = getattr(self, "_z_key", None)
        return (key is not None and key[1] == float(shift) and self._z_chain < self.LS_REFRESH
                and key[0].matches(w_eff))

    def ls_begin(self, w0_eff, shift0, d_eff, d_shift, t0: float = 1.0, loss=None, alt: bool = False,
                 stats_out: Optional[torch.Tensor] = None) -> bool:
        if loss is None:
            return False
        if getattr(self, "z_cache", None) is None:
            if alt:
                return False
            self.enable_margin_cache()
        if not self._z_valid_for(w0_eff, shift0):
            if alt:
                return False
            self.fwd_all(self._vec(w0_eff), FWD_MARGIN, 0, shift0, None, None, z_out=self.z_cache, with_offset=1,
                         stats=False)
            self._z_key, self._z_chain, self._tpend = (VecKey(w0_eff), float(shift0)), 0, 0.0
        if alt:
            from .native import KERNEL_CONFIG
            if getattr(self, "_multi", "unset") == "unset":
                self._build_multi()
            if (self._multi is None or not KERNEL_CONFIG.get("tl_multi", 1)
                    or getattr(self, "_masked", None) is not None):
                return False
        with trace_range("K1' direction pass (margins of d + first trial)"):
            if alt:
                zin, din = self.z_cache, self.zd
                if getattr(self, "_zalt", None) is None:
                    self._zalt = (torch.empty_like(zin), torch.empty_like(din))
                zout, dout = self._zalt
                self.lib.pml_set_ls_in(zin.data_ptr(), din.data_ptr())
            else:
                zout, dout = self.z_cache, self.zd
            self.lib.pml_set_ls_args(zout.data_ptr(), float(t0), float(self._tpend))
            try:
                self.fwd_all(self._vec(d_eff), FWD_LS, loss.loss_id, d_shift, self.coef, None, z_out=dout)
            finally:
                self.lib.pml_set_ls_args(None, 0.0, 0.0)
                if alt:
                    self.lib.pml_set_ls_in(None, None)
            if alt:
                self.z_cache, self.zd, self._zalt = zout, dout, (zin, din)
            self._tpend = 0.0
            self._ls_t0 = float(t0)
            self._coef_stale = False
            if stats_out is None:
                stats_out = torch.empty(2, dtype=torch.float64, device=self.device)
            self._ls_t0_dev = self._reduce_stats(stats_out)
            self._ls_t0_host = None
        return True

    _LS_STATE = ("z_cache", "zd", "_zalt", "_tpend", "_ls_t0", "_ls_t0_dev", "_ls_t0_host", "_z_key", "_z_chain",
                 "_track_u", "_dzz_key", "_dzz_shift", "_coef_stale", "_step_base")

    def ls_checkpoint(self) -> dict:
        return {k: getattr(self, k, None) for k in self._LS_STATE}

    def ls_restore(self, ck: dict, t0_host=None):
        for k, v in ck.items():
            setattr(self, k, v)
        self._coef_stale = True
        if t0_host is not None and self._ls_t0 is not None:
            self._ls_t0_host = tuple(float(v) for v in t0_host)

    @property
    def _ls_t0_vals(self):
        if self._ls_t0_host is None:
            self._ls_t0_host = tuple(self._ls_t0_dev.tolist())
        return self._ls_t0_host

    def _ls(self, loss, t, final, out):
        dzz = self.dzz if (final and self.track_hessian and loss.twice_differentiable) else None
        check(self.lib.pml_ls_eval(self.prec, self.n_rows, float(t), loss.loss_id, self.z_cache.data_ptr(),
                                   self.zd.data_ptr(), self.y.data_ptr(), self.wt.data_ptr(), int(final),
                                   self.coef.data_ptr() if final else None, None if dzz is None else dzz.data_ptr(),
                                   self.ls_stats.data_ptr(), out.data_ptr(), stream_handle(self.device)), "ls_eval")

    def ls_eval(self, loss, t: float):
        if self._ls_t0 is not None and float(t) == self._ls_t0:
            return self._ls_t0_vals
        with trace_range("line-search trial (margin space)"):
            self._ls(loss, t, 0, self.ls_out)
            f, d = self.ls_out.tolist()
        return f, d

    def ls_gate_supported(self) -> bool:
        from .native import KERNEL_CONFIG
        if getattr(self, "_multi_t", "unset") == "unset":
            self._build_multi_t()
        return (self._multi_t is not None and KERNEL_CONFIG.get("tl_multi", 1) and getattr(self, "_masked", None) is None
                and getattr(self, "_ls_t0", None) == 1.0 and not getattr(self, "_coef_stale", False)
                and getattr(self, "_ls_t0_dev", None) is not None and self.z_cache.is_cuda)

    def ls_finish_gated(self, loss, pre: torch.Tensor, f0: float, l2: float, c1: float, c2: float,
# ... 127 lines not shown
    def step_add(self, alpha: float):
        self.zd.add_(self.u_dir, alpha=float(alpha))

    def _u_out(self):
        return self.u_dir if getattr(self, "_track_u", False) else None

    def set_weights(self, weights):
        self.wt.copy_(torch.as_tensor(weights, device=self.device).to(self.vdt))
        self.mark_weights_changed()

    def _rows(self, t: torch.Tensor, c: int) -> int:
        return t.data_ptr() + self.row_starts[c] * t.element_size()

    def _fwd(self, c: int, x: torch.Tensor, mode: int, loss_id: int, shift: float, coef: Optional[torch.Tensor],
             dzz: Optional[torch.Tensor], z_out: Optional[torch.Tensor] = None, with_offset: int = 0,
             stats: bool = True):
        ch = self.csr[c]
        st = self.stats.data_ptr() + 2 * 8 * self.blk_off[c] if stats else None
        xp = x.data_ptr() + self.col_lo[c] * x.element_size()
        if ch.kind == "tl":
            masked = getattr(self, "_masked", None)
            desc = masked[0][c] if masked is not None and isinstance(masked[0], list) else ch.desc
            check(self.lib.pml_tl_fwd(
                self.prec, ctypes.byref(desc), xp, mode, loss_id, float(shift),
                self._rows(self.y, c), self._rows(self.o, c), self._rows(self.wt, c),
                None if coef is None else self._rows(coef, c), None if dzz is None else self._rows(dzz, c),
                None if z_out is None else self._rows(z_out, c), with_offset, st, stream_handle(self.device)),
                "tl_fwd")
            return
        lst = self.long_stats.data_ptr() + 2 * 8 * self.long_off[c] if stats else None
        check(self.lib.pml_seg_fwd(
            self.prec, ctypes.byref(ch.desc), xp, mode, loss_id, float(shift),
            self._rows(self.y, c), self._rows(self.o, c), self._rows(self.wt, c),
            None if coef is None else self._rows(coef, c), None if dzz is None else self._rows(dzz, c),
            None if z_out is None else self._rows(z_out, c), with_offset, st, lst, self.parts.data_ptr(),
            stream_handle(self.device)), "seg_fwd")

    def _t(self, c: int, x: torch.Tensor, G: torch.Tensor, square: int = 0):
        ch = self.csc[c]
        gp = G.data_ptr() + self.col_lo[c] * G.element_size()
        if ch.kind == "tl":
            masked = getattr(self, "_masked", None)
            desc = ch.desc if masked is None else masked[1][c]
            check(self.lib.pml_tl_t(self.prec, ctypes.byref(desc), self._rows(x, c), square, gp,
                                    self.parts.data_ptr(), stream_handle(self.device)), "tl_t")
            return
        check(self.lib.pml_seg_t(self.prec, ctypes.byref(ch.desc), self._rows(x, c), square, gp,
                                 self.parts.data_ptr(), stream_handle(self.device)), "seg_t")

    def _build_multi(self):
        self._multi = None
        if (not self.csr or any(ch.kind != "tl" for ch in self.csr) or len({ch.rbits for ch in self.csr}) != 1
                or len({ch.tbits for ch in self.csr}) != 1):
            return
        tabs = []
        for c, ch in enumerate(self.csr):
            b = ch.blk.to(torch.int64)
            t = torch.empty((b.shape[0], b.shape[1] + 2), dtype=torch.int64, device=b.device)
            t[:, 0] = c
            t[:, 1] = b[:, 0] + self.row_starts[c]
            t[:, 2:5] = b[:, 1:4]
            t[:, 5] = self.col_lo[c]
            t[:, 6:] = b[:, 4:]
            if ch.tbits:
                t[:, 11] += self.blk_off[c]
            tabs.append(t)
        self._multi_blk = torch.cat(tabs).to(torch.int32).contiguous()
        from .tiled import stream_ptr_table
        self._multi_ptrs = stream_ptr_table(self.csr, self.device)
        from .native import TLFwdMultiDesc
        if len({ch.il for ch in self.csr}) != 1:
            return
        self._multi = TLFwdMultiDesc(self._multi_blk.data_ptr(), self._multi_blk.shape[0], self.csr[0].rbits,
                                     self._multi_ptrs.data_ptr(), self.csr[0].il, tbits=self.csr[0].tbits)

    def _build_multi_t(self):
        self._multi_t = None
        if not self.csc or any(ch.kind != "tl" for ch in self.csc) or len({ch.cbits for ch in self.csc}) != 1:
            return
        C = 1 << self.csc[0].cbits
        if any(lo % C for lo in self.col_lo):
            return
        from .tiled import TLTMulti
        self._multi_t = TLTMulti(self.csc, self.row_starts, self.dim,
                                 tile_offsets=[lo // C for lo in self.col_lo] if any(self.col_lo) else None)
        need = self._multi_t.parts_needed
        if need > self.parts.numel():
            self.parts = torch.zeros(need, dtype=torch.float64, device=self.device)

    def fwd_all(self, x, mode, loss_id, shift, coef, dzz, z_out=None, with_offset=0, stats=True):
        from .native import KERNEL_CONFIG
        self.n_fwd = getattr(self, "n_fwd", 0) + 1
        if getattr(self, "_multi", "unset") == "unset":
            self._build_multi()
        if self._multi is not None and KERNEL_CONFIG.get("tl_multi", 1):
            p = lambda t: None if t is None else t.data_ptr()
            masked = getattr(self, "_masked", None)
            desc = self._multi if masked is None or isinstance(masked[0], list) else masked[0]
            check(self.lib.pml_tl_fwd_multi(
                self.prec, ctypes.byref(desc), x.data_ptr(), mode, loss_id, float(shift), self.y.data_ptr(),
                self.o.data_ptr(), self.wt.data_ptr(), p(coef), p(dzz), p(z_out), with_offset,
                self.stats.data_ptr() if stats else None, stream_handle(self.device)), "tl_fwd_multi")
            return
        for c in range(len(self.csr)):
            self._fwd(c, x, mode, loss_id, shift, coef, dzz, z_out, with_offset, stats)

    def t_all(self, x, G, square: int = 0, build_multi: bool = True):
        from .native import KERNEL_CONFIG
        self.n_t = getattr(self, "n_t", 0) + 1
        if getattr(self, "_multi_t", "unset") == "unset":
            if not build_multi:
                for c in range(len(self.csc)):
                    self._t(c, x, G, square)
                return
            self._build_multi_t()
        if (self._multi_t is not None and KERNEL_CONFIG.get("tl_multi", 1)
                and getattr(self, "_masked", None) is None):
            check(self.lib.pml_tl_t_multi(self.prec, ctypes.byref(self._multi_t.desc), x.data_ptr(), square,
                                          G.data_ptr(), self.parts.data_ptr(), stream_handle(self.device)),
                  "tl_t_multi")
            return
        for c in range(len(self.csc)):
            self._t(c, x, G, square)

    def entity_mask_geometry(self, row_entity: torch.Tensor, col_entity: torch.Tensor):
        cached = getattr(self, "_mgeo", None)
        if cached is not None:
            return cached
        self._mgeo = False
        if getattr(self, "_multi", "unset") == "unset":
            self._build_multi()
        if (self.old_of_new is not None or not self.csc or any(ch.kind != "tl" for ch in self.csc + self.csr)
                or not self.n_rows):
            return False
        nr, nc = row_entity.numel(), col_entity.numel()
        rspan = lambda lo, cnt: (row_entity[lo.clamp(0, nr - 1)], row_entity[(lo + cnt - 1).clamp(0, nr - 1)])
        if self._multi is not None:
            blk = self._multi_blk.to(torch.int64)
            f0, f1 = rspan(blk[:, 1], blk[:, 2])
            f_off = [0, int(blk.shape[0])]
        else:
            parts = [rspan(ch.blk[: ch.nblk, 0].to(torch.int64) + self.row_starts[c], ch.blk[: ch.nblk, 1].to(torch.int64))
                     for c, ch in enumerate(self.csr)]
            f0 = torch.cat([p[0] for p in parts])
            f1 = torch.cat([p[1] for p in parts])
            f_off = np.cumsum([0] + [int(ch.nblk) for ch in self.csr]).tolist()
        firsts, lasts, i_off, m_off = [], [], [0], [0]
        for c, ch in enumerate(self.csc):
            C = 1 << ch.cbits
            hi = self.col_lo[c] + ch.dim - 1
            for t in (ch.items[: ch.nitems, 0].to(torch.int64), ch.mt_tiles[: ch.nmt].to(torch.int64)):
                firsts.append(col_entity[(self.col_lo[c] + t * C).clamp(0, nc - 1)])
                lasts.append(col_entity[torch.clamp(self.col_lo[c] + (t + 1) * C - 1, max=hi).clamp(0, nc - 1)])
            i_off.append(i_off[-1] + int(ch.nitems) + int(ch.nmt))
            m_off.append(i_off[-2] + int(ch.nitems))
        t0, t1 = torch.cat(firsts), torch.cat(lasts)
        self._mgeo = (f0, f1, f_off, t0, t1, i_off, m_off)
        return self._mgeo

    def set_entity_mask(self, active: Optional[torch.Tensor], geometry=None):
        self._masked = None
        if active is None or not geometry:
            return
        f0, f1, f_off, t0, t1, i_off, m_off = geometry
        dup = lambda d: type(d).from_buffer_copy(d)
        cs = torch.zeros(active.numel() + 1, dtype=torch.int32, device=active.device)
        torch.cumsum(active.to(torch.int32), 0, out=cs[1:])
        live_f = ((cs[f1 + 1] - cs[f0]) > 0).to(torch.uint8)
        live_t = ((cs[t1 + 1] - cs[t0]) > 0).to(torch.uint8)
        keep = [live_f, live_t]
        if self._multi is not None:
            fdesc = dup(self._multi)
            fdesc.live = live_f.data_ptr()
        else:
            fdesc = []
            for c, ch in enumerate(self.csr):
                d = dup(ch.desc)
                d.live = live_f.data_ptr() + f_off[c]
                fdesc.append(d)
        tdescs = []
        for c, ch in enumerate(self.csc):
            d = dup(ch.desc)
            d.live = live_t.data_ptr() + i_off[c]
            d.live_mt = live_t.data_ptr() + m_off[c + 1]
            tdescs.append(d)
        self._masked = (fdesc, tdescs, keep)
        if MASK_STATS is not None:
            MASK_STATS.append((float(live_f.float().mean()), float(live_t.float().mean())))

    def grad_buckets(self, nb: int):
        cache = getattr(self, "_gbuckets", None)
        if cache is not None and cache[0] == nb:
            return cache[1]
        if getattr(self, "_multi_t", "unset") == "unset":
            self._build_multi_t()
        if self._multi_t is None or nb < 2:
            self._gbuckets = (nb, None)
            return None
        from .tiled import TLTMulti
        C = 1 << self._multi_t.cbits
        ntiles = (self.dim + C - 1) // C
        work = np.zeros(ntiles, np.int64)
        for ch in self.csc:
            it = ch.items[: ch.nitems].cpu().numpy().astype(np.int64)
            np.add.at(work, it[:, 0], it[:, 2] - it[:, 1])
        cum = np.cumsum(work)
        cuts = [0] + [int(np.searchsorted(cum, cum[-1] * k / nb, side="right")) for k in range(1, nb)] + [ntiles]
        cuts = sorted(set(min(max(c, 0), ntiles) for c in cuts))
        out = []
        for t0, t1 in zip(cuts[:-1], cuts[1:]):
            if t1 > t0:
                mt = TLTMulti(self.csc, self.row_starts, self.dim, tile_range=(t0, t1))
                out.append((mt, t0 * C, min(t1 * C, self.dim)))
                if mt.parts_needed > self.parts.numel():
                    self.parts = torch.zeros(mt.parts_needed, dtype=torch.float64, device=self.device)
        self._gbuckets = (nb, out)
        return out

    def _packed_bucketed(self, x, G, start_reduce, nb: int, square: int = 0):
        self.n_t = getattr(self, "n_t", 0) + 1
        for mt, c0, c1 in self.grad_buckets(nb):
            check(self.lib.pml_tl_t_multi(self.prec, ctypes.byref(mt.desc), x.data_ptr(), square, G.data_ptr(),
                                          self.parts.data_ptr(), stream_handle(self.device)), "tl_t_multi")
            start_reduce(G[c0:c1])

    def value_grad_packed_overlap(self, loss, w_eff, margin_shift, start_reduce, nb: int = 4) -> torch.Tensor:
        with trace_range("K1 value+grad pass (bucketed)"):
            out = torch.zeros(self.dim + 2, dtype=torch.float64, device=self.device)
            if self._zero_point(loss, w_eff):
                self._zero_coef(loss, margin_shift, out[self.dim:])
                start_reduce(out[self.dim:])
                self._packed_bucketed(self.coef, out[: self.dim], start_reduce, nb)
                self.n_passes += 1
                return out
            if self._cached_point(w_eff, margin_shift):
                self._ls(loss, self._tpend, 1, out[self.dim:])
                self._ls_t0 = None
                if self.track_hessian and loss.twice_differentiable:
                    self._dzz_key, self._dzz_shift = VecKey(w_eff), float(margin_shift)
                start_reduce(out[self.dim:])
                self._packed_bucketed(self.coef, out[: self.dim], start_reduce, nb)
                self.n_passes += 1
                return out
            x = self._vec(w_eff)
            dzz = self.dzz if (self.track_hessian and loss.twice_differentiable) else None
            zc = getattr(self, "z_cache", None)
            self.fwd_all(x, FWD_VALUE_GRAD, loss.loss_id, margin_shift, self.coef, dzz, z_out=zc)
            if zc is not None:
                self._z_key, self._z_chain, self._tpend, self._ls_t0 = (VecKey(w_eff),
                                                                         float(margin_shift)), 0, 0.0, None
            out[self.dim:] = self._reduce_stats()
            start_reduce(out[self.dim:])
            self._packed_bucketed(self.coef, out[: self.dim], start_reduce, nb)
            if dzz is not None:
                self._dzz_key = VecKey(w_eff)
                self._dzz_shift = float(margin_shift)
            self.n_passes += 1
            return out

    def hv_packed_overlap(self, loss, w_eff, margin_shift, v_eff, v_shift, start_reduce, nb: int = 4):
        with trace_range("K2 Hessian-vector pass (bucketed)"):
            self._ensure_dzz(loss, w_eff, margin_shift)
            out = torch.zeros(self.dim + 2, dtype=torch.float64, device=self.device)
            x = self._vec(v_eff)
            self.fwd_all(x, FWD_HV, loss.loss_id, v_shift, self.coef, self.dzz, z_out=self._u_out())
            out[self.dim:] = self._reduce_stats()
            start_reduce(out[self.dim:])
            self._packed_bucketed(self.coef, out[: self.dim], start_reduce, nb)
            self.n_passes += 1
            return out

    def perm_fingerprint(self) -> float:
        if self.old_of_new is None:
            return 0.0
        k = torch.arange(self.dim, device=self.device, dtype=torch.float64)
        return float((self.old_of_new.to(torch.float64) * torch.sin(k * 0.618 + 0.1)).sum()) + 1.0

    def _reduce_stats(self, out: Optional[torch.Tensor] = None) -> torch.Tensor:
        out = self.out2 if out is None else out
        st = stream_handle(self.device)
        check(self.lib.pml_reduce_stats(self.stats.data_ptr(), self.blk_off[-1], out.data_ptr(), 0,
                                        self.red_scratch.data_ptr(), st), "reduce")
        if self.long_off[-1] > 0:
            check(self.lib.pml_reduce_stats(self.long_stats.data_ptr(), self.long_off[-1], out.data_ptr(), 1,
                                            None, st), "reduce")
        elif self.blk_off[-1] == 0:
            out.zero_()
        return out

    def _vec(self, w: torch.Tensor) -> torch.Tensor:
        w = w.to(self.device)
        perm = self.old_of_new
        if (w.is_cuda and w.dtype == torch.float64 and w.dim() == 1 and w.is_contiguous()
                and (perm is None or (perm.device == w.device and perm.dtype == torch.int64))):
            from .native import perm_cast
            return perm_cast(w, perm, self.vdt)
        if perm is not None:
            w = w[perm]
        return w.to(self.vdt).contiguous()

    def _unperm(self, g: torch.Tensor) -> torch.Tensor:
        return g if self.old_of_new is None else g[self.new_of_old]

    def _grad_target(self, out: torch.Tensor) -> torch.Tensor:
        if self.old_of_new is None:
            return out[: self.dim]
        g = getattr(self, "_gscr", None)
        if g is None or g.numel() != self.dim:
            g = self._gscr = torch.empty(self.dim, dtype=torch.float64, device=self.device)
        return g.zero_()

    def _grad_finish(self, G: torch.Tensor, out: torch.Tensor):
        if self.old_of_new is not None:
            torch.index_select(G, 0, self.new_of_old, out=out[: self.dim])

    def value_grad_packed(self, loss, w_eff, margin_shift) -> torch.Tensor:
        with trace_range("K1 value+grad pass"):
            return self._value_grad_packed(loss, w_eff, margin_shift)

    def _cached_point(self, w_eff, shift) -> bool:
        return (getattr(self, "z_cache", None) is not None and getattr(self, "_masked", None) is None
                and self._z_valid_for(w_eff, shift))

    def _zero_point(self, loss, w_eff) -> bool:
        return bool(getattr(w_eff, "_pml_zero", False)) and not (self.track_hessian and loss.twice_differentiable)

    def _zero_coef(self, loss, margin_shift, stats_out: torch.Tensor):
        n = self.n_rows
        o = self.o[:n]
        z0 = o if (o.dtype == torch.float64 and float(margin_shift) == 0.0 and o.is_contiguous()) else \
            o.to(torch.float64) + float(margin_shift)
        check(self.lib.pml_ls_eval(self.prec, n, 0.0, loss.loss_id, z0.data_ptr(), z0.data_ptr(), self.y.data_ptr(),
                                   self.wt.data_ptr(), 1, self.coef.data_ptr(), None, self.ls_stats_buf().data_ptr(),
                                   stats_out.data_ptr(), stream_handle(self.device)), "ls_eval(zero)")

    def frob_sq(self) -> torch.Tensor:
        c = getattr(self, "_frob_sq", None)
        if c is None:
            parts = []
            for ch in self.csr:
                for v in (ch.val, getattr(ch, "nval", None)):
                    if v is not None and v.numel():
                        v64 = v.reshape(-1).to(torch.float64)
                        parts.append(torch.dot(v64, v64))
                        del v64
            c = torch.stack(parts).sum() if parts else torch.zeros((), dtype=torch.float64, device=self.device)
            self._frob_sq = c
        return c

    def zero_point_sums(self, loss, margin_shift) -> list:
        out = torch.empty(4, dtype=torch.float64, device=self.device)
        self._zero_coef(loss, margin_shift, out[:2])
        out[2] = torch.linalg.vector_norm(self.coef[: self.n_rows], dtype=torch.float64) ** 2
        out[3] = self.frob_sq()
        return out.tolist()

    def ls_stats_buf(self) -> torch.Tensor:
        buf = getattr(self, "ls_stats", None)
        if buf is None:
            self.ls_stats = buf = torch.zeros(2 * 4096, dtype=torch.float64, device=self.device)
        return buf

    def _value_grad_packed(self, loss, w_eff, margin_shift) -> torch.Tensor:
        out = (torch.zeros if self.old_of_new is None else torch.empty)(self.dim + 2, dtype=torch.float64,
                                                                        device=self.device)
        G = self._grad_target(out)
        if self._zero_point(loss, w_eff):
            self._zero_coef(loss, margin_shift, out[self.dim:])
            self.t_all(self.coef, G)
            self._grad_finish(G, out)
            self.n_passes += 1
            return out
        if self._cached_point(w_eff, margin_shift):
            self._ls(loss, self._tpend, 1, out[self.dim:])
            self._ls_t0 = None
            if self.track_hessian and loss.twice_differentiable:
                self._dzz_key, self._dzz_shift = VecKey(w_eff), float(margin_shift)
            self.t_all(self.coef, G)
            self._grad_finish(G, out)
            self.n_passes += 1
            return out
        x = self._vec(w_eff)
        dzz = self.dzz if (self.track_hessian and loss.twice_differentiable) else None
        zc = getattr(self, "z_cache", None)
        self.fwd_all(x, FWD_VALUE_GRAD, loss.loss_id, margin_shift, self.coef, dzz, z_out=zc)
        if zc is not None:
            self._z_key, self._z_chain, self._tpend, self._ls_t0 = (VecKey(w_eff), float(margin_shift)), \
                0, 0.0, None
        self.t_all(self.coef, G)
        out[self.dim:] = self._reduce_stats()
        self._grad_finish(G, out)
        if dzz is not None:
            self._dzz_key = VecKey(w_eff)
            self._dzz_shift = float(margin_shift)
        self.n_passes += 1
        return out

    def value_grad_sums(self, loss, w_eff, margin_shift):
        out = self.value_grad_packed(loss, w_eff, margin_shift)
        fs = out[self.dim:].tolist()
        return fs[0], fs[1], out[: self.dim]

    def _ensure_dzz(self, loss, w_eff, shift):
        key = self._dzz_key
        if key is not None and self._dzz_shift == float(shift) and key.matches(w_eff):
            return
        x = self._vec(w_eff)
        self.fwd_all(x, FWD_DZZ, loss.loss_id, shift, self.dzz, None, stats=False)
        self._dzz_key = VecKey(w_eff)
        self._dzz_shift = float(shift)

    def hv_packed(self, loss, w_eff, margin_shift, v_eff, v_shift) -> torch.Tensor:
        with trace_range("K2 Hessian-vector pass"):
            return self._hv_packed(loss, w_eff, margin_shift, v_eff, v_shift)

    def _hv_packed(self, loss, w_eff, margin_shift, v_eff, v_shift) -> torch.Tensor:
        self._ensure_dzz(loss, w_eff, margin_shift)
        out = (torch.zeros if self.old_of_new is None else torch.empty)(self.dim + 2, dtype=torch.float64,
                                                                        device=self.device)
        H = self._grad_target(out)
        x = self._vec(v_eff)
        self.fwd_all(x, FWD_HV, loss.loss_id, v_shift, self.coef, self.dzz, z_out=self._u_out())
        self.t_all(self.coef, H)
        out[self.dim:] = self._reduce_stats()
        self._grad_finish(H, out)
        self.n_passes += 1
        return out

    def hv_sums(self, loss, w_eff, margin_shift, v_eff, v_shift):
        out = self.hv_packed(loss, w_eff, margin_shift, v_eff, v_shift)
        return out[: self.dim], float(out[self.dim + 1])

    def hdiag_sums(self, loss, w):
        x = self._vec(w)
        out = torch.zeros(self.dim, dtype=torch.float64, device=self.device)
        self.fwd_all(x, FWD_DZZ, loss.loss_id, 0.0, self.coef, None, stats=False)
        self.t_all(self.coef, out, square=1)
        self._dzz_key = None
        return self._unperm(out)

    def matvec(self, w) -> torch.Tensor:
        return self.margins(w, 0.0, False)

    def rmatvec(self, r, square: bool = False, build_multi: bool = True) -> torch.Tensor:
        rr = torch.as_tensor(r, device=self.device).to(self.vdt).contiguous()
        if rr.numel() < max(self.n_rows, 1):
            rr = torch.cat([rr, torch.zeros(max(self.n_rows, 1) - rr.numel(), dtype=self.vdt, device=self.device)])
        out = torch.zeros(self.dim, dtype=torch.float64, device=self.device)
        self.t_all(rr, out, square=int(square), build_multi=build_multi)
        return self._unperm(out)

    def column_stats(self):
        if self.layout != "tiled" or any(getattr(ch, "kind", None) != "tl" for ch in self.csc):
            raise ValueError("column_stats needs the tiled layout")
        if self.device.type != "cuda":
            raise RuntimeError("column_stats runs the HIP column-statistics kernels: the shard must be on a GPU")
        from .native import tl_colstats
        z = lambda: torch.zeros(self.dim, dtype=torch.float64, device=self.device)
        outs = [z(), z(), z(), z(),
                torch.full((self.dim,), float("-inf"), dtype=torch.float64, device=self.device),
                torch.full((self.dim,), float("inf"), dtype=torch.float64, device=self.device)]
        for c, ch in enumerate(self.csc):
            tl_colstats(self.prec, ch, self.col_lo[c], outs, self.parts)
        return tuple(self._unperm(t) for t in outs)

    def margins(self, w, margin_shift: float = 0.0, with_offsets: bool = False):
        if (getattr(self, "_masked", None) is None and getattr(self, "z_cache", None) is not None
                and isinstance(w, torch.Tensor) and self._z_valid_for(w, margin_shift)):
            n = self.n_rows
            if self.z_cache.is_cuda and self.o.dtype in (torch.float32, torch.float64):
                from .native import cached_margins
                return cached_margins(self.z_cache, self.zd if self._tpend else None, self._tpend,
                                      None if with_offsets else self.o, n)
            z = self.z_cache[:n].clone()
            if self._tpend:
                z.add_(self.zd[:n], alpha=self._tpend)
            if not with_offsets:
                z.sub_(self.o[:n].to(torch.float64))
            return z
        alloc = torch.empty if getattr(self, "_masked", None) is None else torch.zeros
        z = alloc(max(self.n_rows, 1), dtype=torch.float64, device=self.device)
        x = self._vec(w)
        self.fwd_all(x, FWD_MARGIN, 0, margin_shift, None, None, z_out=z, with_offset=int(with_offsets),
                     stats=False)
        return z[: self.n_rows]
```

photon_ml_amd/ops/native.py:

```python
from __future__ import annotations

import ctypes
import os
from pathlib import Path
from typing import Optional

import numpy as np
import torch

from .build import StaleLibraryError, expected_id, lib_path, verified_path

c_int = ctypes.c_int
c_double = ctypes.c_double
c_void_p = ctypes.c_void_p
P_int = ctypes.POINTER(ctypes.c_int)


class SegChunkDesc(ctypes.Structure):
    _fields_ = [
        ("blk", c_void_p), ("nblk", c_int),
        ("seg_ptr", c_void_p), ("nseg", c_int),
        ("idx", c_void_p), ("val", c_void_p),
        ("long_seg", c_void_p), ("long_ptr", c_void_p), ("nlong", c_int), ("npart", c_int),
    ]


class TLNarrow(ctypes.Structure):
    _fields_ = [("pack", c_void_p), ("val", c_void_p), ("base", c_void_p), ("wbase", c_void_p)]


class TLFwdDesc(ctypes.Structure):
    _fields_ = [("blk", c_void_p), ("nblk", c_int), ("rbits", c_int), ("pack", c_void_p), ("val", c_void_p),
                ("il", c_int), ("nar", TLNarrow), ("live", c_void_p), ("tbits", c_int)]


class TLFwdMultiDesc(ctypes.Structure):
    _fields_ = [("blk", c_void_p), ("nblk", c_int), ("rbits", c_int), ("ptrs", c_void_p), ("il", c_int),
                ("live", c_void_p), ("tbits", c_int)]


class TLTMultiDesc(ctypes.Structure):
    _fields_ = [("items", c_void_p), ("nitems", c_int), ("cbits", c_int), ("ptrs", c_void_p),
                ("mt_tiles", c_void_p), ("mt_ptr", c_void_p), ("nmt", c_int), ("dim", c_int), ("cu", c_void_p),
                ("ncu", c_int), ("nparts_total", c_int), ("il", c_int), ("live", c_void_p), ("live_mt", c_void_p)]


class CmpArgs(ctypes.Structure):
    _fields_ = [("units", c_void_p), ("col_e", c_int), ("row_col", c_int), ("seg", c_void_p), ("nseg", c_int),
                ("sbits", c_int), ("key_is_row", c_int), ("pack", c_void_p), ("val", c_void_p),
                ("npack", c_void_p), ("nval", c_void_p), ("nbase", c_void_p), ("keep", c_void_p),
                ("seg_cnt", c_void_p), ("seg_first", c_void_p), ("unit_lo", c_void_p), ("opack", c_void_p),
                ("oval", c_void_p), ("ustride", c_int), ("wbits", c_int)]


class SegRankArgs(ctypes.Structure):
    _fields_ = [("seg_ptr", c_void_p), ("perm", c_void_p), ("scores", c_void_p), ("wts", c_void_p),
                ("flag", c_void_p), ("list", c_void_p), ("lptr", c_void_p), ("out", c_void_p),
                ("nan_flag", c_void_p), ("n_list", ctypes.c_longlong), ("n_rows", ctypes.c_longlong),
                ("n_groups", ctypes.c_longlong), ("k", c_int)]


class AucCountArgs(ctypes.Structure):
    _fields_ = [("scores", c_void_p), ("flag", c_void_p), ("summ", c_void_p), ("out", c_void_p),
                ("n", ctypes.c_longlong), ("n_blocks", ctypes.c_longlong)]


class TLTDesc(ctypes.Structure):
    _fields_ = [
        ("items", c_void_p), ("nitems", c_int), ("cbits", c_int), ("pack", c_void_p), ("val", c_void_p),
        ("mt_tiles", c_void_p), ("mt_ptr", c_void_p), ("nmt", c_int), ("dim", c_int),
        ("cu", c_void_p), ("ncu", c_int), ("nparts_total", c_int), ("il", c_int), ("nar", TLNarrow),
        ("live", c_void_p), ("live_mt", c_void_p),
    ]


_LIBS = {}


def _load(name: str, auto_build: bool = True) -> Optional[ctypes.CDLL]:
    if name in _LIBS:
        return _LIBS[name]
    override = {"glm": "PML_GLM_LIB", "re": "PML_RE_LIB"}.get(name)
    if override and os.environ.get(override):
        path = Path(os.environ[override])
        want = None
    else:
        try:
            path = verified_path("hip", name, auto_build=auto_build)
        except FileNotFoundError:
            _LIBS[name] = None
            return None
        want = expected_id("hip", name)
    lib = ctypes.CDLL(str(path), mode=ctypes.RTLD_GLOBAL)
    if want is not None:
        lib.pml_build_id.restype = ctypes.c_char_p
        got = lib.pml_build_id().decode()
        if got != want:
            raise StaleLibraryError(f"{path}: loaded build id {got} != {want} of the tree's sources")
    _LIBS[name] = lib
    return lib


def glm_lib() -> Optional[ctypes.CDLL]:
    lib = _load("glm")
    if lib is not None and not getattr(lib, "_pml_typed", False):
        lib.pml_build_blocks.argtypes = [c_void_p, c_int, c_int, c_int, c_void_p, P_int, c_void_p, c_void_p,
                                         P_int, P_int]
        lib.pml_seg_fwd.argtypes = [c_int, ctypes.POINTER(SegChunkDesc), c_void_p, c_int, c_int, c_double,
                                    c_void_p, c_void_p, c_void_p, c_void_p, c_void_p, c_void_p, c_int, c_void_p,
                                    c_void_p, c_void_p, c_void_p]
        lib.pml_seg_t.argtypes = [c_int, ctypes.POINTER(SegChunkDesc), c_void_p, c_int, c_void_p, c_void_p,
                                  c_void_p]
        lib.pml_reduce_stats.argtypes = [c_void_p, c_int, c_void_p, c_int, c_void_p, c_void_p]
        lib.pml_lds_add_order_probe.argtypes = [c_void_p, c_void_p, c_int, c_void_p]
        lib.pml_lds_add_order_probe.restype = c_int
        lib.pml_tl_fwd.argtypes = [c_int, ctypes.POINTER(TLFwdDesc), c_void_p, c_int, c_int, c_double, c_void_p,
                                   c_void_p, c_void_p, c_void_p, c_void_p, c_void_p, c_int, c_void_p, c_void_p]
        lib.pml_tl_t.argtypes = [c_int, ctypes.POINTER(TLTDesc), c_void_p, c_int, c_void_p, c_void_p, c_void_p]
        lib.pml_tl_colstats.argtypes = [c_int, ctypes.POINTER(TLTDesc)] + [c_void_p] * 8
        lib.pml_tl_config.argtypes = [c_int, c_int, c_int, c_int]
        lib.pml_tl_t_multi.argtypes = [c_int, ctypes.POINTER(TLTMultiDesc), c_void_p, c_int, c_void_p, c_void_p,
                                       c_void_p]
        lib.pml_tl_fwd_multi.argtypes = [c_int, ctypes.POINTER(TLFwdMultiDesc), c_void_p, c_int, c_int, c_double,
                                         c_void_p, c_void_p, c_void_p, c_void_p, c_void_p, c_void_p, c_int, c_void_p,
                                         c_void_p]
        lib.pml_segdot.argtypes = [c_void_p, c_void_p, c_int, c_void_p, c_int, c_void_p, c_void_p]
        lib.pml_segdot_long.argtypes = [c_void_p, c_void_p, c_int, c_void_p, c_int, ctypes.c_longlong, c_void_p,
                                        c_void_p, c_void_p]
        lib.pml_seg_expand.argtypes = [c_void_p, c_int, c_void_p, c_void_p, c_int, c_void_p]
        lib.pml_seg_cg_step.argtypes = [c_void_p, c_int] + [c_void_p] * 7 + [c_double, c_void_p]
        lib.pml_bgemv.argtypes = [c_int, c_int, c_void_p, c_void_p, c_void_p, c_int, c_void_p]
        lib.pml_btrsv.argtypes = [c_int, c_int, c_void_p, c_void_p, c_void_p, c_int, c_void_p]
        lib.pml_bhv.argtypes = [c_int, c_int, c_void_p, c_void_p, c_void_p, c_double, c_void_p, c_void_p]
        lib.pml_set_ls_args.argtypes = [c_void_p, c_double, c_double]
        lib.pml_set_ls_in.argtypes = [c_void_p, c_void_p]
        lib.pml_set_gate.argtypes = [c_void_p]
        lib.pml_ls_gate.argtypes = [c_void_p, c_void_p, c_double, c_double, c_double, c_double, c_void_p, c_void_p,
                                    c_void_p]
        lib.pml_ls_gate.restype = c_int
        lib.pml_gram_grid.argtypes = [ctypes.c_longlong]
        lib.pml_gram.argtypes = [c_void_p, c_int, ctypes.c_longlong, c_void_p, c_void_p]
        lib.pml_lincomb.argtypes = [c_void_p, c_void_p, c_int, ctypes.c_longlong, c_void_p, c_void_p]
        lib.pml_lbfgs_pair.argtypes = [c_void_p] * 4 + [ctypes.c_longlong] + [c_void_p] * 6
        lib.pml_ls_dots.argtypes = [c_void_p] * 3 + [ctypes.c_longlong] + [c_void_p] * 4
        lib.pml_perm_cast.argtypes = [c_void_p, c_void_p, ctypes.c_longlong, c_int, c_void_p, c_void_p]
        lib.pml_perm_cast.restype = c_int
        lib.pml_ls_step_grad.argtypes = [c_void_p, c_void_p, c_double, c_void_p, c_void_p, c_double,
                                         ctypes.c_longlong, c_void_p, c_void_p, c_void_p]
        lib.pml_ls_step_grad.restype = c_int
        lib.pml_masked_gather.argtypes = [c_void_p, c_void_p, ctypes.c_longlong, c_void_p, c_void_p]
        lib.pml_masked_gather.restype = c_int
        lib.pml_offset_update.argtypes = [c_void_p, c_void_p, ctypes.c_longlong, c_int, c_void_p, c_void_p, c_void_p]
        lib.pml_cached_margins.argtypes = [c_void_p, c_void_p, c_double, c_int, c_void_p, ctypes.c_longlong,
                                           c_void_p, c_void_p]
        lib.pml_cached_margins.restype = c_int
        lib.pml_offset_update.restype = c_int
        lib.pml_two_loop_chain.argtypes = [c_int] + [c_void_p] * 5 + [ctypes.c_longlong] + [c_void_p] * 4 + \
            [c_int, c_void_p]
        lib.pml_two_loop_gram.argtypes = [c_int, c_void_p, c_void_p, c_void_p, ctypes.c_longlong, c_void_p, c_void_p,
                                          c_void_p, c_int, c_void_p]
        lib.pml_two_loop_gram_grid.argtypes = [ctypes.c_longlong]
        lib.pml_tl_set_deep.argtypes = [c_int, c_int]
        lib.pml_rs_set_variant.argtypes = [c_int]
        lib.pml_rs_set_variant(int(os.environ.get("PML_RS_VARIANT", "5")))
        lib.pml_ls_eval.argtypes = [c_int, c_int, c_double, c_int, c_void_p, c_void_p, c_void_p, c_void_p, c_int,
                                    c_void_p, c_void_p, c_void_p, c_void_p, c_void_p]
        lib.pml_ls_eval_multi.argtypes = [c_int, c_int, c_int, ctypes.POINTER(c_double), c_int, c_void_p, c_void_p,
                                          c_void_p, c_void_p, c_void_p, c_void_p, c_void_p]
        lib.pml_ls_eval_multi.restype = c_int
        lib.pml_rs_tron.argtypes = [c_int, c_int] + [c_void_p] * 8 + [c_int, c_double, c_double, c_int, c_int, c_int,
                                                                      c_void_p, c_void_p, c_void_p]
        for f in ("pml_seg_fwd", "pml_seg_t", "pml_reduce_stats", "pml_build_blocks", "pml_tl_fwd", "pml_tl_t",
                  "pml_tl_colstats",
                  "pml_tl_maxbits", "pml_segdot", "pml_segdot_long", "pml_tl_fwd_multi", "pml_tl_t_multi", "pml_seg_cg_step",
                  "pml_seg_expand", "pml_bgemv", "pml_btrsv", "pml_bhv", "pml_rs_tron", "pml_ls_eval", "pml_gram_grid", "pml_gram",
                  "pml_lincomb", "pml_lbfgs_pair", "pml_ls_dots", "pml_two_loop_chain", "pml_two_loop_gram",
                  "pml_two_loop_gram_grid"):
            getattr(lib, f).restype = c_int
        lib.pml_set_config.argtypes = [c_int, c_int, c_int, c_int]
        lib._pml_typed = True
        configure()
    return lib


KERNEL_CONFIG = {"fwd_strided": 0, "t_strided": 0, "hot_n": 0, "fwd_grid": 1024, "tl_acc64": 1, "tl_waves": 2,
                 "tl_waves_t": 4, "tl_pipe": 0, "tl_pipe_t": 0, "tl_multi": 1, "tl_deep": 0, "tl_deep_t": 0}


def configure(**kw):
    KERNEL_CONFIG.update({k: v for k, v in kw.items() if v is not None})
    for k in list(KERNEL_CONFIG):
        env = os.environ.get("PML_" + k.upper())
        if env is not None and k not in kw:
            KERNEL_CONFIG[k] = int(env)
    lib = _LIBS.get("glm")
    if lib is not None:
        lib.pml_set_config(KERNEL_CONFIG["fwd_strided"], KERNEL_CONFIG["t_strided"], KERNEL_CONFIG["hot_n"],
                           KERNEL_CONFIG["fwd_grid"])
        lib.pml_tl_config(KERNEL_CONFIG["tl_acc64"], KERNEL_CONFIG["tl_waves"], KERNEL_CONFIG["tl_waves_t"],
                          (KERNEL_CONFIG["tl_pipe"] & 3) | ((KERNEL_CONFIG["tl_pipe_t"] & 3) << 2))
        lib.pml_tl_set_deep(KERNEL_CONFIG["tl_deep"], KERNEL_CONFIG["tl_deep_t"])
    return dict(KERNEL_CONFIG)


def tl_experiment_build() -> bool:
    lib = glm_lib()
    return lib is not None and bool(lib.pml_tl_experiment())


def require_glm_lib() -> ctypes.CDLL:
    lib = glm_lib()
    if lib is None:
        raise RuntimeError(
            f"native GLM kernel library missing ({lib_path('hip', 'glm')}); run python -m photon_ml_amd.ops.build")
    return lib


def segdot(a: torch.Tensor, b: Optional[torch.Tensor], ptr: torch.Tensor, mode: int = 0) -> torch.Tensor:
    nseg = ptr.numel() - 1
    if a.device.type != "cuda":
        import numpy as np
        v = (a * b if mode == 0 else (a if mode == 1 else a.abs())).detach().cpu().numpy()
        p = ptr.cpu().numpy()
        out = np.zeros(nseg)
        nz = p[1:] > p[:-1]
# ... 1254 lines not shown
```

photon_ml_amd/ops/tiled.py:

```python
from __future__ import annotations

import ctypes
import math
import os
from typing import Optional, Sequence, Tuple

import numpy as np
import torch

from .native import TLFwdDesc, TLTDesc

TL_MAXBITS = 12
TL_MAXBITS_F64 = 11
TL_MINBITS = 5
DEFAULT_RBITS = int(os.environ.get("PML_TL_RBITS", 10))
DEFAULT_CBITS = int(os.environ.get("PML_TL_CBITS", 10))
DEFAULT_ITEM_ENTRIES = 1 << 18
_PAD = 8
COMBINE_SEG = 16


XCD_GROUPS = int(os.environ.get("PML_TL_XCD", "0"))


def xcd_order(chunk_of_item: np.ndarray, groups: int) -> np.ndarray:
    stream = np.asarray(chunk_of_item) % groups
    lists = [np.flatnonzero(stream == k) for k in range(groups)]
    longest = max(len(l) for l in lists)
    grid = np.full((longest, groups), -1, dtype=np.int64)
    for k, l in enumerate(lists):
        grid[: len(l), k] = l
    order = grid.reshape(-1)
    return order[order >= 0]


def combine_seg(k: int) -> int:
    return max(COMBINE_SEG, int(math.ceil(math.sqrt(k))))
IL_ROUND = 256
TL_VEC = 4
INTERLEAVE = int(os.environ.get("PML_TL_IL", "1"))
NARROW = int(os.environ.get("PML_TL_NARROW", "1"))
NARROW_W = 64
FUSE = int(os.environ.get("PML_TL_FUSE", "1"))
WIDE_BASE = int(os.environ.get("PML_TL_WIDE_BASE", "1"))
TALL = os.environ.get("PML_TL_TALL")
TALL = None if TALL is None else bool(int(TALL))
TALL_DEFAULT = True
TALL_BITS = 12
TALL_SUB_BITS = 10
TALL_MIN_DIM = 1 << 16
TALL_COLS = 10


def narrow_width(sbits: int) -> int:
    return min(NARROW_W, 1 << max(16 - sbits, 0))


def _bits(n: int) -> int:
    return max(1, int(n - 1).bit_length())


def _cap(want: int, f64: bool) -> int:
    return min(want, TL_MAXBITS_F64 if f64 else TL_MAXBITS)


F64_WIDE_RBITS = 11


def default_rbits(dim: int, f64: bool) -> int:
    if f64 and dim >= (1 << 16) and "PML_TL_RBITS" not in os.environ:
        return F64_WIDE_RBITS
    return DEFAULT_RBITS


def fwd_bits(dim: int, f64: bool = False, want: Optional[int] = None) -> Optional[int]:
    r = min(_cap(default_rbits(dim, f64) if want is None else want, f64), 32 - _bits(dim))
    return r if r >= TL_MINBITS else None


def t_bits(chunk_rows: int, f64: bool = False, want: Optional[int] = None) -> Optional[int]:
    c = min(_cap(DEFAULT_CBITS if want is None else want, f64), 32 - _bits(chunk_rows))
    return c if c >= TL_MINBITS else None


SPARSE_TILE_ENTRIES = 1 << 16


def shard_t_config(nnz: int, n_rows: int, dim: int, chunk_rows: int):
    if "PML_TL_CBITS" in os.environ or "PML_TL_ITEM_ENTRIES" in os.environ or n_rows <= 0 or dim < (1 << 16):
        return None, None
    per_tile = (nnz / n_rows) * min(chunk_rows, n_rows) / math.ceil(dim / 1024)
    if per_tile < SPARSE_TILE_ENTRIES:
        return 11, 1 << 17
    return None, None


def tl_supported(dim: int, chunk_rows: int) -> bool:
    return fwd_bits(dim) is not None and t_bits(chunk_rows) is not None


def _to_u32_bits(x64: torch.Tensor) -> torch.Tensor:
    return torch.where(x64 >= (1 << 31), x64 - (1 << 32), x64).to(torch.int32)


def _pad(t: torch.Tensor) -> torch.Tensor:
    return torch.cat([t, torch.zeros(_PAD, dtype=t.dtype, device=t.device)]).contiguous()


def il_phys(e_lo: torch.Tensor, n: torch.Tensor) -> torch.Tensor:
    e_lo = e_lo.to(torch.int64)
    n = n.to(torch.int64)
    tot = int(n.sum())
    unit = torch.repeat_interleave(torch.arange(n.numel(), device=n.device), n)
    j = torch.arange(tot, device=n.device) - (torch.cumsum(n, 0) - n)[unit]
    t = j & (IL_ROUND - 1)
    return e_lo[unit] + (j - t) + ((t & 63) << 2) + (t >> 6)


def _interleave(pack: torch.Tensor, val: torch.Tensor, n: torch.Tensor, tail: int = _PAD):
    n = n.to(torch.int64)
    padded = (n + IL_ROUND - 1) // IL_ROUND * IL_ROUND
    new_lo = torch.cumsum(padded, 0) - padded
    total = int(padded.sum()) + tail
    phys = il_phys(new_lo, n)
    p = torch.zeros(total, dtype=pack.dtype, device=pack.device)
    v = torch.zeros(total, dtype=val.dtype, device=val.device)
    p[phys] = pack
    v[phys] = val
    return p, v, new_lo


def _empty_narrow(val: torch.Tensor):
    dev = val.device
    return (torch.zeros(IL_ROUND, dtype=torch.int16, device=dev), torch.zeros(IL_ROUND, dtype=val.dtype, device=dev),
            torch.zeros(1, dtype=torch.int32, device=dev))


def split_narrow(pack: torch.Tensor, val: torch.Tensor, n: torch.Tensor, sbits: int, xlen: int, enable: bool = True):
    dev = pack.device
    n = n.to(torch.int64)
    U = n.numel()
    gcount = n // IL_ROUND
    W = narrow_width(sbits)
    ok = enable and NARROW and W >= 16 and xlen >= NARROW_W and int(gcount.sum()) > 0
    if not ok:
        z = torch.zeros(U, dtype=torch.int64, device=dev)
        return (pack, val, n, *_empty_narrow(val), z)
    starts = torch.cumsum(n, 0) - n
    gu = torch.repeat_interleave(torch.arange(U, device=dev), gcount)
    gi = torch.arange(gu.numel(), device=dev) - (torch.cumsum(gcount, 0) - gcount)[gu]
    gs = starts[gu] + IL_ROUND * gi
    key = pack >> sbits
    first, last = key[gs], key[gs + IL_ROUND - 1]
    base = torch.clamp(first, max=xlen - NARROW_W)
    nar = (last - base) < W
    gs_n, base = gs[nar], base[nar]
    idx = gs_n[:, None] + torch.arange(IL_ROUND, device=dev)[None, :]
    p16 = ((key[idx] - base[:, None]) << sbits) | (pack[idx] & ((1 << sbits) - 1))
    il = lambda t: t.reshape(-1, TL_VEC, 64).transpose(1, 2).reshape(-1)
    npack = il(torch.where(p16 >= 32768, p16 - 65536, p16).to(torch.int16)).contiguous()
    nval = il(val[idx]).contiguous()
    if FUSE and val.dtype == torch.bfloat16:
        npack = torch.cat([npack.view(-1, TL_VEC), nval.view(torch.int16).view(-1, TL_VEC)], 1).reshape(-1)
        nval = None
    nbase = base.to(torch.int32).contiguous()
    cs = torch.zeros(nar.numel() + 1, dtype=torch.int64, device=dev)
    torch.cumsum(nar.to(torch.int64), 0, out=cs[1:])
    ge = torch.cumsum(gcount, 0)
    nrounds = cs[ge] - cs[ge - gcount]
    keep = torch.ones(pack.numel(), dtype=torch.bool, device=dev)
    keep[idx.reshape(-1)] = False
    del idx, p16
    return pack[keep], val[keep], n - IL_ROUND * nrounds, npack, nval, nbase, nrounds



def narrow_logical(npack: torch.Tensor, nval: torch.Tensor, nbase: torch.Tensor, r_lo, r_hi, sbits: int):
    r = torch.arange(int(r_lo), int(r_hi), device=npack.device)
    if not r.numel():
        return torch.zeros(0, dtype=torch.int64, device=npack.device), nval[:0].reshape(-1)
    ph = (r[:, None] * IL_ROUND + torch.arange(IL_ROUND, device=npack.device)[None, :]).reshape(-1, 64, TL_VEC)
    ph = ph.transpose(1, 2).reshape(-1)
    rl, rh = int(r_lo) * IL_ROUND, int(r_hi) * IL_ROUND
    ph = ph - rl
    p16 = npack.reshape(-1, TL_VEC)[rl // TL_VEC:rh // TL_VEC].reshape(-1)[ph].to(torch.int64) & 0xFFFF
    base = nbase[r].to(torch.int64).repeat_interleave(IL_ROUND)
    return ((((p16 >> sbits) + base) << sbits) | (p16 & ((1 << sbits) - 1)),
            nval.reshape(-1, TL_VEC)[rl // TL_VEC:rh // TL_VEC].reshape(-1)[ph])


class _NarrowMixin:

    wbase = None

    nrec = None

    def _set_narrow(self, npack, nval, nbase):
        from .native import TLNarrow
        self.nrec = npack if nval is None else None
        if nval is None:
            rec = npack.view(-1, 2 * TL_VEC)
            npack, nval = rec[:, :TL_VEC], rec[:, TL_VEC:].view(torch.bfloat16)
        self.npack, self.nval, self.nbase = npack, nval, nbase
        self.nar = TLNarrow(npack.data_ptr(), None if self.fused else nval.data_ptr(), nbase.data_ptr(),
                            None if self.wbase is None else self.wbase.data_ptr())

    @property
    def fused(self) -> bool:
        return self.nrec is not None

    @property
    def n_narrow_rounds(self) -> int:
        t = self._table()
        return int((t[:, 5] - t[:, 4]).sum()) if t.shape[0] else 0

    def unit_counts(self) -> torch.Tensor:
        t = self._table().to(torch.int64)
        lo, hi = self._ew
        return (t[:, hi] - t[:, lo]) + IL_ROUND * (t[:, 5] - t[:, 4])

    def narrow_window(self, r_lo: int, r_hi: int):
        return narrow_logical(self.npack, self.nval, self.nbase, r_lo, r_hi, self._sbits)

    def _logical_all(self, wide_pack, wide_val):
        t = self._table().to(torch.int64)
        dev = wide_pack.device
        lo, hi = self._ew
        nn = IL_ROUND * (t[:, 5] - t[:, 4])
        nw = t[:, hi] - t[:, lo]
        if int(nn.sum()) == 0:
            return wide_pack, wide_val
        npk, nvl = narrow_logical(self.npack, self.nval, self.nbase, 0, int(t[:, 5].max()), self._sbits)
        U = t.shape[0]
        nu = torch.repeat_interleave(torch.arange(U, device=dev), nn.to(dev))
        nj = torch.arange(int(nn.sum()), device=dev) - (torch.cumsum(nn, 0) - nn).to(dev)[nu]
        npos = t[:, 4].to(dev)[nu] * IL_ROUND + nj
        wu = torch.repeat_interleave(torch.arange(U, device=dev), nw.to(dev))
        unit = torch.cat([nu, wu])
        order = torch.sort(unit, stable=True).indices
        wp = wide_pack.to(torch.int64) & 0xFFFFFFFF if wide_pack.dtype == torch.int32 else wide_pack.to(torch.int64)
        pk = torch.cat([npk[npos], wp])[order]
        vl = torch.cat([nvl[npos], wide_val])[order]
        return pk, vl


def tall_engages(tall: Optional[bool], dim: int, m: int, dtype, il: int, want_rbits: int) -> bool:
    if not (il and NARROW and dtype != torch.float64 and want_rbits == TALL_SUB_BITS):
        return False
    if tall is None:
        tall = TALL
    if tall is None:
        tall = TALL_DEFAULT and dim >= TALL_MIN_DIM and m >= (1 << TALL_BITS)
    return bool(tall)


def shard_tall(dim: int, chunk_rows: int) -> Optional[bool]:
    if TALL is not None:
        return None
    return bool(TALL_DEFAULT and dim >= TALL_MIN_DIM and chunk_rows >= (1 << TALL_BITS))


class TLFwdChunk(_NarrowMixin):

    kind = "tl"

    def __init__(self, rowptr: torch.Tensor, col: torch.Tensor, val: torch.Tensor, dim: int,
                 rbits: Optional[int] = None, il: Optional[int] = None, tall: Optional[bool] = None):
        dev = val.device
        self.il = INTERLEAVE if il is None else int(il)
        rowptr = rowptr.to(dev, torch.int64)
        col = col.to(dev, torch.int64)
        m = rowptr.numel() - 1
        f64 = val.dtype == torch.float64
        self.rbits = fwd_bits(dim, f64, rbits)
        if self.rbits is None:
            raise ValueError(f"tiled forward layout cannot pack dim={dim}")
        want = _cap(default_rbits(dim, f64) if rbits is None else rbits, f64)
        self.tbits = 0
        if tall_engages(tall, dim, m, val.dtype, self.il, want) and self._init_tall(rowptr, col, val, dim, m):
            return
        use_base = bool(self.il) and WIDE_BASE and want > self.rbits
        if use_base:
            self.rbits = want
        R = 1 << self.rbits
        kbits = _bits(dim) + self.rbits
        nnz = col.numel()
        rows = torch.repeat_interleave(torch.arange(m, device=dev), rowptr[1:] - rowptr[:-1]) if nnz else \
            torch.zeros(0, dtype=torch.int64, device=dev)
        pack = (col << self.rbits) | (rows & (R - 1))
        key = ((rows >> self.rbits) << kbits) | pack
        key, perm = torch.sort(key, stable=True)
        nblk = (m + R - 1) // R
        b = torch.arange(nblk, device=dev)
        lo = b * R
        hi = torch.clamp(lo + R, max=m)
        e_lo, e_hi = rowptr[lo], rowptr[hi]
        self._sbits, self._ew = self.rbits, (2, 3)
        n_lo = n_hi = torch.zeros(nblk, dtype=torch.int64, device=dev)
        if self.il:
            wp, wv, wn, npk, nvl, nbs, nr = split_narrow(key & ((1 << kbits) - 1), val[perm], e_hi - e_lo,
                                                         self.rbits, dim)
            del key, perm
            if use_base:
                wp = self._rebase(wp, wn)
                if wp is None:
                    del wv, npk, nvl, nbs
                    self.__init__(rowptr, col, val, dim, fwd_bits(dim, f64, rbits), il, tall=False)
                    return
            self.pack, self.val, e_lo = _interleave(_to_u32_bits(wp), wv, wn)
            e_hi = e_lo + wn
            n_hi = torch.cumsum(nr, 0)
            n_lo = n_hi - nr
            del wp, wv
        else:
            self.pack = _pad(_to_u32_bits(key & ((1 << kbits) - 1)))
            self.val = _pad(val[perm].contiguous())
            npk, nvl, nbs = _empty_narrow(val)
            del key, perm
        del rows
        self._set_narrow(npk, nvl, nbs)
        self.blk = torch.stack([lo, hi - lo, e_lo, e_hi, n_lo, n_hi], 1).to(torch.int32).contiguous()
        self.nblk, self.m, self.nnz = nblk, m, nnz
        self.desc = TLFwdDesc(self.blk.data_ptr(), nblk, self.rbits, self.pack.data_ptr(), self.val.data_ptr(),
                              self.il, self.nar)

    def _init_tall(self, rowptr: torch.Tensor, col: torch.Tensor, val: torch.Tensor, dim: int, m: int) -> bool:
        dev = val.device
        S, T = TALL_SUB_BITS, TALL_BITS
        cb = _bits(dim)
        nnz = col.numel()
        rows = torch.repeat_interleave(torch.arange(m, device=dev), rowptr[1:] - rowptr[:-1]) if nnz else \
            torch.zeros(0, dtype=torch.int64, device=dev)
        key = ((rows >> S) << (cb + S)) | (col << S) | (rows & ((1 << S) - 1))
        del rows
        key, perm = torch.sort(key, stable=True)
        nunit = (m + (1 << T) - 1) >> T
        nsub = nunit << (T - S)
        slo = torch.clamp(torch.arange(nsub, device=dev) << S, max=m)
        cnt = rowptr[torch.clamp(slo + (1 << S), max=m)] - rowptr[slo]
        wp, wv, wn, npk, nvl, nbs, nr = split_narrow(key & ((1 << (cb + S)) - 1), val[perm], cnt, S, dim)
        del key, perm
        sub = torch.repeat_interleave(torch.arange(nsub, device=dev), wn)
        tp = ((wp >> S) << T) | ((sub & ((1 << (T - S)) - 1)) << S) | (wp & ((1 << S) - 1))
        ukey = ((sub >> (T - S)) << cb) | (wp >> S)
        del sub, wp
        if _bits(max(nunit, 1)) + cb <= 31:
            ukey = ukey.to(torch.int32)
        tperm = torch.sort(ukey, stable=True).indices
        del ukey
        tp, wv = tp[tperm], wv[tperm]
        del tperm
        un = wn.view(nunit, -1).sum(1)
        if cb + T > 32:
            tp = self._rebase(tp, un, T) if WIDE_BASE else None
            if tp is None:
                self.wbase = None
                return False
        self.rbits, self.tbits = S, T
        self.pack, self.val, e_lo = _interleave(_to_u32_bits(tp), wv, un, tail=0)
        del tp, wv
        nh = torch.cumsum(nr, 0)
        nl = (nh - nr).view(nunit, -1)
        ulo = torch.arange(nunit, device=dev) << T
        self._sbits, self._ew = S, (2, 3)
        self._set_narrow(npk, nvl, nbs)
        self.blk = torch.stack([ulo, torch.clamp(ulo + (1 << T), max=m) - ulo, e_lo, e_lo + un, nl[:, 0],
                                nh.view(nunit, -1)[:, -1], nl[:, 1], nl[:, 2], nl[:, 3], ulo >> S],
                               1).to(torch.int32).contiguous()
        self.nblk, self.m, self.nnz = nunit, m, nnz
        self.desc = TLFwdDesc(self.blk.data_ptr(), nunit, S, self.pack.data_ptr(), self.val.data_ptr(), 1, self.nar,
                              tbits=T)
        return True

    @property
    def ubits(self) -> int:
        return self.tbits or self.rbits

    def _rebase(self, wp: torch.Tensor, wn: torch.Tensor, bits: Optional[int] = None) -> Optional[torch.Tensor]:
        dev = wp.device
        bits = self.rbits if bits is None else bits
        n = wn.to(torch.int64)
        tot = int(n.sum())
        padded = (n + IL_ROUND - 1) // IL_ROUND * IL_ROUND
        nrounds = int(padded.sum()) // IL_ROUND
        wbase = torch.zeros(nrounds + 1, dtype=torch.int64, device=dev)
        if tot:
            unit = torch.repeat_interleave(torch.arange(n.numel(), device=dev), n, output_size=tot)
            j = torch.arange(tot, device=dev) - (torch.cumsum(n, 0) - n)[unit]
            rid = ((torch.cumsum(padded, 0) - padded)[unit] + j) // IL_ROUND
            del unit
            key = wp >> bits
            first = (j % IL_ROUND) == 0
            del j
            wbase[rid[first]] = key[first]
            rel = key - wbase[rid]
            del rid, key, first
            if int(rel.max()) >= 1 << (32 - bits):
                return None
            wp = (rel << bits) | (wp & ((1 << bits) - 1))
        self.wbase = wbase.to(torch.int32).contiguous()
        return wp

    @property
    def nstats(self) -> int:
        return (self.m + (1 << self.rbits) - 1) >> self.rbits if self.tbits else self.nblk

    parts_needed = 0

    def _table(self):
        return self.blk

    def nbytes(self) -> int:
        return sum(t.numel() * t.element_size() for t in (self.blk, self.pack, self.val, self.npack, self.nval,
                                                           self.nbase) + (() if self.wbase is None else (self.wbase,)))

    def logical(self):
        if not self.il:
            return self.pack[: self.nnz].to(torch.int64) & 0xFFFFFFFF, self.val[: self.nnz]
        ph = il_phys(self.blk[:, 2], self.blk[:, 3] - self.blk[:, 2])
        wp = self.pack[ph].to(torch.int64) & 0xFFFFFFFF
        ub = self.ubits
        if self.wbase is not None:
            wp = ((self.wbase[ph // IL_ROUND].to(torch.int64) + (wp >> ub)) << ub) | (wp & ((1 << ub) - 1))
        if not self.tbits:
            return self._logical_all(wp, self.val[ph])
        t = self.blk.to(torch.int64)
        dev = wp.device
        U = t.shape[0]
        if not U or int((t[:, 5] - t[:, 4]).sum()) == 0:
            return wp, self.val[ph]
        S, T = self.rbits, self.tbits
        npk, nvl = narrow_logical(self.npack, self.nval, self.nbase, 0, int(t[-1, 5]), S)
        bounds = torch.stack([t[:, 4], t[:, 6], t[:, 7], t[:, 8], t[:, 5]], 1)
        per_sub = (bounds[:, 1:] - bounds[:, :-1]).reshape(-1)
        esub = torch.repeat_interleave(torch.arange(per_sub.numel(), device=dev), IL_ROUND * per_sub.to(dev))
        npk = ((npk >> S) << T) | ((esub & ((1 << (T - S)) - 1)) << S) | (npk & ((1 << S) - 1))
        unit = torch.cat([esub >> (T - S), torch.repeat_interleave(torch.arange(U, device=dev),
                                                                   (t[:, 3] - t[:, 2]).to(dev))])
        order = torch.sort(unit, stable=True).indices
        return torch.cat([npk, wp])[order], torch.cat([nvl, self.val[ph]])[order]

    def emulate_matvec(self, x: torch.Tensor) -> torch.Tensor:
        pk, vl = self.logical()
        p = pk.to(torch.int64)
        col = p >> self.ubits
        blk_of_entry = torch.repeat_interleave(torch.arange(self.nblk, device=p.device), self.unit_counts())
        row = (blk_of_entry << self.ubits) + (p & ((1 << self.ubits) - 1))
        z = torch.zeros(self.m, dtype=torch.float64, device=p.device)
        return z.index_add_(0, row, vl.to(torch.float64) * x.to(torch.float64)[col])


class TLTChunk(_NarrowMixin):

    kind = "tl"

    def __init__(self, rowptr: torch.Tensor, col: torch.Tensor, val: torch.Tensor, dim: int, chunk_rows: int,
                 cbits: Optional[int] = None, item_entries: Optional[int] = None, il: Optional[int] = None):
        self.il = INTERLEAVE if il is None else int(il)
        if item_entries is None:
            item_entries = int(os.environ.get("PML_TL_ITEM_ENTRIES", DEFAULT_ITEM_ENTRIES))
        dev = val.device
        rowptr = rowptr.to(dev, torch.int64)
        col = col.to(dev, torch.int64)
        m = rowptr.numel() - 1
        self.cbits = t_bits(max(chunk_rows, m), val.dtype == torch.float64, cbits)
        if self.cbits is None:
            raise ValueError(f"tiled transpose layout cannot pack chunk_rows={chunk_rows}")
        C = 1 << self.cbits
        nnz = col.numel()
        rows = torch.repeat_interleave(torch.arange(m, device=dev), rowptr[1:] - rowptr[:-1]) if nnz else \
            torch.zeros(0, dtype=torch.int64, device=dev)
        tile = col >> self.cbits
        pack = (rows << self.cbits) | (col & (C - 1))
        key = (tile << 32) | pack
        del rows, pack
        key, perm = torch.sort(key, stable=True)
        del tile
        ntiles = (dim + C - 1) // C
        tptr = torch.searchsorted(key >> 32, torch.arange(ntiles + 1, device=dev)).cpu().numpy().astype(np.int64)
        counts = np.diff(tptr)
        pack = _to_u32_bits(key & 0xFFFFFFFF)
        val = val[perm]
        del key, perm
        nz = np.nonzero(counts)[0]
        n_it = np.maximum(1, -(-counts[nz] // item_entries))
        it_tile = np.repeat(nz, n_it)
        it_i = np.arange(len(it_tile)) - np.repeat(np.cumsum(n_it) - n_it, n_it)
        it_k = np.repeat(n_it, n_it)
        a, b = tptr[it_tile], tptr[it_tile + 1]
        lo, hi = a + (b - a) * it_i // it_k, a + (b - a) * (it_i + 1) // it_k
        split = it_k > 1
        part_of = np.full(len(it_tile), -1, np.int64)
        part_of[split] = np.arange(int(split.sum()))
        km = n_it[n_it > 1]
        plo = np.cumsum(km) - km
        sg = np.maximum(COMBINE_SEG, np.ceil(np.sqrt(km)).astype(np.int64)) if len(km) else km
        nu = -(-km // sg)
        u_mt = np.repeat(np.arange(len(km)), nu)
        u_first = np.repeat(plo, nu) + np.repeat(sg, nu) * (np.arange(int(nu.sum())) - np.repeat(np.cumsum(nu) - nu, nu))
        u_last = np.minimum(u_first + np.repeat(sg, nu), np.repeat(plo + km, nu))
        cu = np.column_stack([u_mt, u_first, u_last]) if len(km) else np.zeros((0, 3), np.int64)
        mt_tiles = nz[n_it > 1].tolist()
        mt_ptr = np.r_[0, np.cumsum(nu)].tolist() if len(km) else [0]
        self.nitems, self.nmt, self.nparts, self.ncu = len(it_tile), len(mt_tiles), int(km.sum()), len(cu)
        items = np.column_stack([it_tile, lo, hi, part_of]).astype(np.int64).reshape(-1, 4)
        items = np.column_stack([items, np.zeros((len(items), 2), np.int64)])
        self._sbits, self._ew = self.cbits, (1, 2)
        if self.il:
            cnt = torch.from_numpy(items[:, 2] - items[:, 1]).to(dev)
            wp, wv, wn, npk, nvl, nbs, nr = split_narrow(pack.to(torch.int64) & 0xFFFFFFFF, val, cnt, self.cbits, m)
            del pack, val
            self.pack, self.val, new_lo = _interleave(_to_u32_bits(wp), wv, wn)
            del wp, wv
            items[:, 1] = new_lo.cpu().numpy()
            items[:, 2] = items[:, 1] + wn.cpu().numpy()
            nr = nr.cpu().numpy()
            items[:, 5] = np.cumsum(nr)
            items[:, 4] = items[:, 5] - nr
        else:
            self.pack, self.val = _pad(pack), _pad(val.contiguous())
            npk, nvl, nbs = _empty_narrow(val)
            del pack, val
        self._set_narrow(npk, nvl, nbs)
        self.items = torch.tensor(items.astype(np.int32), device=dev)
        self.mt_tiles = torch.tensor(np.asarray(mt_tiles or [0], dtype=np.int32), device=dev)
        self.mt_ptr = torch.tensor(np.asarray(mt_ptr, dtype=np.int32), device=dev)
        self.cu = torch.tensor(np.asarray(cu if len(cu) else [(0, 0, 0)], dtype=np.int32).reshape(-1, 3), device=dev)
        self.m, self.nnz, self.dim = m, nnz, dim
        self.desc = TLTDesc(self.items.data_ptr(), self.nitems, self.cbits, self.pack.data_ptr(),
                            self.val.data_ptr(), self.mt_tiles.data_ptr(), self.mt_ptr.data_ptr(), self.nmt, dim,
                            self.cu.data_ptr(), self.ncu, self.nparts, self.il, self.nar)

    @property
    def parts_needed(self) -> int:
        return (self.nparts + self.ncu) << self.cbits

    def _table(self):
        return self.items

    def nbytes(self) -> int:
        return sum(t.numel() * t.element_size() for t in (self.items, self.mt_tiles, self.mt_ptr, self.cu, self.pack,
                                                           self.val, self.npack, self.nval, self.nbase))

    def window(self, e_lo: int, e_hi: int):
        if not self.il:
            return self.pack[e_lo:e_hi], self.val[e_lo:e_hi]
        ph = il_phys(torch.tensor([e_lo]), torch.tensor([e_hi - e_lo])).to(self.pack.device)
        return self.pack[ph], self.val[ph]

    def logical(self):
        if not self.il:
            return self.pack[: self.nnz], self.val[: self.nnz]
        ph = il_phys(self.items[:, 1], self.items[:, 2] - self.items[:, 1])
        return self._logical_all(self.pack[ph], self.val[ph])

    def emulate_rmatvec(self, r: torch.Tensor, square: bool = False) -> torch.Tensor:
        pk, vl = self.logical()
        p = pk.to(torch.int64) & 0xFFFFFFFF
        row = p >> self.cbits
        tile_of_entry = torch.repeat_interleave(self.items[:, 0].to(torch.int64), self.unit_counts())
        col = (tile_of_entry << self.cbits) + (p & ((1 << self.cbits) - 1))
        v = vl.to(torch.float64)
        if square:
            v = v * v
        g = torch.zeros(self.dim, dtype=torch.float64, device=p.device)
        return g.index_add_(0, col, v * r.to(torch.float64)[row])


class TLTMulti:

    def __init__(self, chunks: Sequence["TLTChunk"], row_starts: Sequence[int], dim: int,
                 tile_range: Optional[Tuple[int, int]] = None, tile_offsets: Optional[Sequence[int]] = None):
        from .native import TLTMultiDesc
        dev = chunks[0].pack.device
        self.cbits = chunks[0].cbits
        self.il = chunks[0].il
        if any(ch.il != self.il for ch in chunks):
            raise ValueError("TLTMulti: chunks mix interleaved and plain streams")
        its = []
        for c, ch in enumerate(chunks):
            it = ch.items[: ch.nitems].cpu().numpy().astype(np.int64).reshape(-1, 6)
            toff = 0 if tile_offsets is None else int(tile_offsets[c])
            its.append(np.column_stack([np.full(len(it), c), it[:, 0] + toff, it[:, 1], it[:, 2],
                                        np.full(len(it), row_starts[c]), it[:, 4], it[:, 5]]))
        it = np.concatenate(its) if its else np.zeros((0, 7), np.int64)
        src_all = np.arange(len(it))
        if tile_range is not None:
            in_range = (it[:, 1] >= tile_range[0]) & (it[:, 1] < tile_range[1])
            it = it[in_range]
        n = len(it)
        tile = it[:, 1]
        order = np.lexsort((np.arange(n), tile))
        ts = tile[order]
        starts = np.flatnonzero(np.r_[True, ts[1:] != ts[:-1]]) if n else np.zeros(0, np.int64)
        k = np.diff(np.r_[starts, n])
        multi_tile = np.repeat(k > 1, k)
        part = np.full(n, -1, np.int64)
        part[order[multi_tile]] = np.arange(int(multi_tile.sum()))
        km = k[k > 1]
        plo = np.cumsum(km) - km
        sg = np.maximum(COMBINE_SEG, np.ceil(np.sqrt(km)).astype(np.int64)) if len(km) else km
        nu = -(-km // sg)
        u_tile = np.repeat(np.arange(len(km)), nu)
        u_first = np.repeat(plo, nu) + np.repeat(sg, nu) * (np.arange(int(nu.sum())) - np.repeat(np.cumsum(nu) - nu, nu))
        u_last = np.minimum(u_first + np.repeat(sg, nu), np.repeat(plo + km, nu))
        self.nitems, self.nparts, self.ncu, self.nmt = n, int(km.sum()), int(nu.sum()), len(km)
        rows = np.column_stack([it[:, 0], it[:, 1], it[:, 2], it[:, 3], part, it[:, 4], it[:, 5],
                                it[:, 6]]).astype(np.int32)
        src = src_all if tile_range is None else src_all[in_range]
        if XCD_GROUPS > 1 and n > XCD_GROUPS:
            xo = xcd_order(it[:, 0], XCD_GROUPS)
            rows, src = rows[xo], src[xo]
        self._src = torch.from_numpy(src.astype(np.int64)).to(dev)
        self.items = torch.tensor(rows.reshape(-1, 8), device=dev)
        self.mt_tiles = torch.tensor(np.r_[ts[starts][k > 1], 0].astype(np.int32)[: max(self.nmt, 1)], device=dev)
        self.mt_ptr = torch.tensor(np.r_[0, np.cumsum(nu)].astype(np.int32), device=dev)
        self.cu = torch.tensor(np.column_stack([u_tile, u_first, u_last]).astype(np.int32).reshape(-1, 3)
                               if self.ncu else np.zeros((1, 3), np.int32), device=dev)
        self.ptrs = stream_ptr_table(chunks, dev)
        self._chunks = list(chunks)
        self.desc = TLTMultiDesc(self.items.data_ptr(), n, self.cbits, self.ptrs.data_ptr(),
                                 self.mt_tiles.data_ptr(), self.mt_ptr.data_ptr(), self.nmt, dim,
                                 self.cu.data_ptr(), self.ncu, self.nparts, self.il)

    @property
    def parts_needed(self) -> int:
        return (self.nparts + self.ncu) << self.cbits

    def restreamed(self, chunks: Sequence["TLTChunk"]) -> "TLTMulti":
        import copy
        from .native import TLTMultiDesc
        dev = self.items.device
        cat = torch.cat([ch.items[: ch.nitems].to(torch.int64) for ch in chunks]) if chunks else None
        rows = self.items.to(torch.int64).clone()
        if self.nitems:
            sel = cat[self._src]
            rows[:, 2:4] = sel[:, 1:3]
            rows[:, 6:8] = sel[:, 4:6]
        new = copy.copy(self)
        new.items = rows.to(torch.int32).contiguous()
        new.ptrs = stream_ptr_table(chunks, dev)
        new._chunks = list(chunks)
        d = self.desc
        new.desc = TLTMultiDesc(new.items.data_ptr(), d.nitems, d.cbits, new.ptrs.data_ptr(), d.mt_tiles, d.mt_ptr,
                                d.nmt, d.dim, d.cu, d.ncu, d.nparts_total, d.il)
        return new

    def emulate_rmatvec(self, r: torch.Tensor, square: bool = False) -> torch.Tensor:
        C = 1 << self.cbits
        dim = self.desc.dim
        ntiles = (dim + C - 1) // C
        G = torch.zeros(ntiles * C, dtype=torch.float64)
        parts = torch.zeros((max(self.nparts, 1), C), dtype=torch.float64)
        r = r.to(torch.float64).cpu()
        for c, tile, e_lo, e_hi, part, rb, n_lo, n_hi in self.items.cpu().tolist():
            ch = self._chunks[c]
            pk, vl = ch.window(e_lo, e_hi)
            npk, nvl = ch.narrow_window(n_lo, n_hi)
            p = torch.cat([npk.cpu(), pk.to(torch.int64).cpu() & 0xFFFFFFFF])
            v = torch.cat([nvl.cpu(), vl.cpu()]).to(torch.float64)
            if square:
                v = v * v
            acc = torch.zeros(C, dtype=torch.float64).index_add_(0, p & (C - 1), v * r[rb + (p >> self.cbits)])
            if part < 0:
                G[tile * C:(tile + 1) * C] += acc
            else:
                parts[part] = acc
        cu = self.cu.cpu().tolist()
        l1 = [parts[a:b].sum(0) for _, a, b in cu[: self.ncu]]
        mp = self.mt_ptr.cpu().tolist()
        for t, tile in enumerate(self.mt_tiles.cpu().tolist()[: self.nmt]):
            s = torch.zeros(C, dtype=torch.float64)
            for u in range(mp[t], mp[t + 1]):
                s += l1[u]
            G[tile * C:(tile + 1) * C] += s
        return G[:dim]


def stream_ptr_table(chunks, device) -> torch.Tensor:
    wb = lambda ch: 0 if getattr(ch, "wbase", None) is None else ch.wbase.data_ptr()
    return torch.tensor([[ch.pack.data_ptr(), ch.val.data_ptr(), ch.npack.data_ptr(),
                          0 if ch.fused else ch.nval.data_ptr(), ch.nbase.data_ptr(), wb(ch)] for ch in chunks],
                        dtype=torch.int64, device=device).reshape(-1)


CMP_SEG = 8


def _cmp_segments(ch, narrow: bool):
    cache = ch.__dict__.setdefault("_cmp_seg", {})
    if cache.get(narrow) is not None:
        return cache[narrow]
    t = ch._table().to(torch.int64)
    dev = t.device
    lo, hi = ch._ew
    nn = t[:, 5] - t[:, 4]
    R = (t[:, hi] - t[:, lo] + IL_ROUND - 1) // IL_ROUND + (nn if narrow else 0)
    ns = (R + CMP_SEG - 1) // CMP_SEG
    S = int(ns.sum())
    su = torch.repeat_interleave(torch.arange(t.shape[0], device=dev), ns, output_size=S)
    first = (torch.cumsum(ns, 0) - ns)[su]
    r_lo = (torch.arange(S, device=dev) - first) * CMP_SEG
    r_hi = torch.minimum(r_lo + CMP_SEG, R[su])
    if not narrow:
        r_lo, r_hi = r_lo + nn[su], r_hi + nn[su]
    seg = torch.stack([su, r_lo, r_hi], 1).to(torch.int32).contiguous()
    cache[narrow] = (seg, su, first, S, IL_ROUND * int(nn.sum()))
    return cache[narrow]


class RowCompaction:

    def __init__(self, ch, keep: torch.Tensor, forward: bool, filter_narrow: bool = False):
        from .native import CmpArgs, check, require_game_lib, stream_handle
        if not ch.il:
            raise ValueError("row-sampled copies need the interleaved layout")
        self.ch, self.keep, self.forward = ch, keep, forward
        dev = ch.pack.device
        self.filter_narrow = bool(filter_narrow)
        seg, su, first, S, self.n_narrow = _cmp_segments(ch, self.filter_narrow)
        table = ch._table()
        lo, hi = ch._ew
        self.seg_cnt = torch.zeros(max(S, 1), dtype=torch.int32, device=dev)
        self._keep_alive = (seg, table, keep)
        self.args = CmpArgs(table.data_ptr(), lo, 0 if forward else -1, seg.data_ptr(), S, ch._sbits,
                            0 if forward else 1, ch.pack.data_ptr(), ch.val.data_ptr(), ch.npack.data_ptr(),
                            None if ch.fused else ch.nval.data_ptr(), ch.nbase.data_ptr(), keep.data_ptr(),
                            self.seg_cnt.data_ptr(),
                            None, None, None, None, table.shape[1], getattr(ch, "ubits", ch._sbits) if forward
                            else ch._sbits)
        self.lib, self.stream = require_game_lib(), stream_handle(dev)
        self.vbytes = ch.val.element_size()
        if S:
            check(self.lib.pml_tl_compact(0, self.vbytes, ctypes.byref(self.args), self.stream), "tl_compact count")
        cnt = self.seg_cnt[:S].to(torch.int64)
        U = table.shape[0]
        self.unit_cnt = torch.zeros(U, dtype=torch.int64, device=dev).index_add_(0, su, cnt)
        padded = (self.unit_cnt + IL_ROUND - 1) // IL_ROUND * IL_ROUND
        self.unit_lo = (torch.cumsum(padded, 0) - padded).contiguous()
        excl = torch.cumsum(cnt, 0) - cnt
        self.seg_first = (excl - excl[first]).contiguous() if S else excl
        self.total, self.kept = padded.sum(), self.unit_cnt.sum()

    def finish(self, total: int, kept: int):
        import copy
        from .native import TLFwdDesc, TLTDesc, check
        ch = self.ch
        dev = ch.pack.device
        opack = torch.zeros(total + _PAD, dtype=torch.int32, device=dev)
        oval = torch.zeros(total + _PAD, dtype=ch.val.dtype, device=dev)
        a = self.args
        a.seg_first, a.unit_lo = self.seg_first.data_ptr(), self.unit_lo.data_ptr()
        a.opack, a.oval = opack.data_ptr(), oval.data_ptr()
        if a.nseg:
            check(self.lib.pml_tl_compact(1, self.vbytes, ctypes.byref(a), self.stream), "tl_compact write")
        lo, hi = ch._ew
        table = ch._table().to(torch.int64).clone()
        table[:, lo] = self.unit_lo
        table[:, hi] = self.unit_lo + self.unit_cnt
        if self.filter_narrow:
            table[:, 4:9] = 0
        table = table.to(torch.int32).contiguous()
        nc = copy.copy(ch)
        nc._cmp_seg = {}
        nc.pack, nc.val = opack, oval
        if self.filter_narrow:
            nc._set_narrow(*_empty_narrow(oval))
            nc.nnz = kept
        else:
            nc.nnz = kept + self.n_narrow
        if self.forward:
            nc.blk = table
            nc.desc = TLFwdDesc(table.data_ptr(), nc.nblk, nc.rbits, opack.data_ptr(), oval.data_ptr(), 1, nc.nar,
                                tbits=nc.tbits)
        else:
            nc.items = table
            nc.desc = TLTDesc(table.data_ptr(), nc.nitems, nc.cbits, opack.data_ptr(), oval.data_ptr(),
                              nc.mt_tiles.data_ptr(), nc.mt_ptr.data_ptr(), nc.nmt, nc.dim, nc.cu.data_ptr(), nc.ncu,
                              nc.nparts, 1, nc.nar)
        return nc
```

photon_ml_amd/ops/warmup.py:

```python
from __future__ import annotations

import time

import torch

_DONE = set()


def runtime_warmup(device, force: bool = False) -> float:
    dev = torch.device(device)
    if dev.type != "cuda":
        return 0.0
    key = dev.index if dev.index is not None else torch.cuda.current_device()
    if key in _DONE and not force:
        return 0.0
    torch.cuda.synchronize(dev)
    t0 = time.perf_counter()
    from .native import (auc_counts, batched_gemv, batched_trsv, check_lds_add_order, csr_gather_rows,
                         key_histogram)
    x = torch.linspace(0.0, 1.0, 4096, dtype=torch.float64, device=dev)
    i = torch.arange(4096, dtype=torch.int64, device=dev)
    torch.linalg.vector_norm(x)
    torch.dot(x, x)
    (x * x).sum()
    torch.where(x > 0.5, x, torch.zeros_like(x)).square().sum()
    torch.isfinite(x).all()
    torch.cumsum(i, 0)
    torch.sort(i.flip(0), stable=True)
    torch.argsort(x.flip(0), stable=True)
    torch.searchsorted(i, i)
    torch.unique(i % 7, sorted=True, return_inverse=True)
    torch.repeat_interleave(i[:8], i[:8] % 3)
    torch.nonzero(i % 5 == 0)
    x[i.flip(0)]
    torch.zeros_like(x).index_copy_(0, i, x)
    torch.zeros(8, dtype=torch.int64, device=dev).scatter_reduce_(0, i % 8, i, reduce="amax")
    torch.segment_reduce(x, "sum", lengths=torch.full((64,), 64, dtype=torch.int64, device=dev))
    x.to(torch.float32).to(torch.bfloat16)
    check_lds_add_order(dev)
    from .device import DeviceGLMData
    tiny = DeviceGLMData.from_device_csr(torch.arange(0, 18, 2, device=dev), i[:16] % 5, x[:16].to(torch.float32),
                                         torch.zeros(8), torch.zeros(8), torch.ones(8), 5, dev, "f32", tall=True)
    tiny.matvec(torch.zeros(5, dtype=torch.float64, device=dev))
    z = torch.zeros(8, dtype=torch.float64, device=dev)
    tiny._fwd(0, torch.zeros(5, dtype=torch.float32, device=dev), 0, 0, 0.0, None, None, z_out=z, stats=False)
    key_histogram(i % 13, 13)
    csr_gather_rows(torch.tensor([0, 2], dtype=torch.int64, device=dev), i[:2], x[:2],
                    torch.zeros(1, dtype=torch.int64, device=dev), torch.tensor([0, 4], dtype=torch.int64, device=dev))
    auc_counts(x.flip(0).contiguous(), (i % 2).to(torch.uint8))
    L = torch.eye(65, dtype=torch.float64, device=dev).unsqueeze(0).contiguous()
    batched_trsv(L, torch.ones(1, 65, dtype=torch.float64, device=dev))
    batched_gemv(L[:, :8, :8].contiguous(), torch.ones(1, 8, dtype=torch.float64, device=dev))
    from .native import re_lbfgs_csr, re_lbfgs_grid
    p01 = torch.tensor([0, 1], dtype=torch.int64, device=dev)
    one = torch.ones(1, dtype=torch.float64, device=dev)
    i32 = lambda: torch.zeros(1, dtype=torch.int32, device=dev)
    re_lbfgs_csr(i32(), p01, p01, p01, torch.zeros(1, dtype=torch.int16, device=dev), one, one, torch.zeros_like(one),
                 one, torch.empty(4, dtype=torch.float64, device=dev), torch.zeros_like(one), torch.empty_like(one),
                 i32(), i32(), torch.empty_like(one), 0, 0.0, 0.1, 1e-3, 2, 256,
                 torch.empty(2 * 10 * 256, dtype=torch.float64, device=dev), i32(), min(re_lbfgs_grid(256), 1))
    torch.cuda.Stream(dev, priority=-1)
    torch.cuda.Stream(dev, priority=0)
    torch.cuda.synchronize(dev)
    _DONE.add(key)
    return time.perf_counter() - t0
```

Measured before the change: 3.668 billion examples/sec.

## Group four adjacent column tiles per block in the transpose (rmatvec) kernel

```diff
diff --git a/photon_ml_amd/data/synthetic.py b/photon_ml_amd/data/synthetic.py
--- a/photon_ml_amd/data/synthetic.py
+++ b/photon_ml_amd/data/synthetic.py
@@ -105,7 +105,7 @@
                           seed: int = 1234567890, chunk_rows: int = 1 << 20, zipf_s: float = 1.1,
                           task=TaskType.LOGISTIC_REGRESSION, rank: int = 0, progress=None, layout: str = "auto"):
     from ..ops.device import DeviceGLMData, SegChunk, VAL_DTYPE, resolve_layout
-    from ..ops.tiled import TLFwdChunk, TLTChunk, shard_tall
+    from ..ops.tiled import TLFwdChunk, TLTChunk, shard_tall, shard_tgroup
 
     dev = torch.device(device)
     prec = {"bf16": 0, "f32": 1, "f64": 2}[precision]
@@ -164,7 +164,8 @@
             col = idx.to(torch.int64)
             del idx
             csr.append(TLFwdChunk(rp, col, val, n_features, tall=shard_tall(n_features, min(chunk_rows, n_rows))))
-            csc.append(TLTChunk(rp, col, val, n_features, chunk_rows, cbits=cbits, item_entries=item_entries))
+            csc.append(TLTChunk(rp, col, val, n_features, chunk_rows, cbits=cbits, item_entries=item_entries,
+                                tgroup=shard_tgroup(n_features, n_rows, chunk_rows)))
             raw[ci] = None
             del col, val, rp
             if progress is not None:
diff --git a/photon_ml_amd/ops/csrc/glm_kernels.hip b/photon_ml_amd/ops/csrc/glm_kernels.hip
--- a/photon_ml_amd/ops/csrc/glm_kernels.hip
+++ b/photon_ml_amd/ops/csrc/glm_kernels.hip
@@ -1165,6 +1165,93 @@
                                             (const VT*)pc[1], nar, x + q[5], G, dim, parts, acc);
 }
 
+#define TL_TG_BITS 12
+#define TL_TG_SUB 10
+#define TL_TG_COLS 24
+#define TL_TG_EMPTY (-2)
+template <typename VT, typename XT, bool SQ, int PT>
+__device__ __forceinline__ void tl_t_group(const int* __restrict__ q, const uint32_t* __restrict__ pack,
+                                           const VT* __restrict__ val, const TLNarrow& nar,
+                                           const XT* __restrict__ x, double* __restrict__ G, int dim,
+                                           double* __restrict__ parts, double* acc) {
+  constexpr int NW = 4, C = 1 << TL_TG_SUB, NS = (1 << TL_TG_BITS) / (NW * 64);
+  for (int i = threadIdx.x; i < (1 << TL_TG_BITS); i += NW * 64) acc[i] = 0.0;
+  const int w = __builtin_amdgcn_readfirstlane(threadIdx.x >> 6);
+  const int n_lo = q[5 + w], nn = q[9 + w] - n_lo;
+  double tot[NS];
+  __syncthreads();
+#pragma unroll 1
+  for (int k = 0; k < 4; ++k) {
+    const int a = n_lo + (nn * k) / 4, b = n_lo + (nn * (k + 1)) / 4;
+    if (b > a) tl_narrow<VT, XT, double, SQ, 1, (PT >= 5 ? 4 : 2)>(nar, a, b, TL_TG_SUB, x, acc + (w << TL_TG_SUB));
+    __syncthreads();
+    const int e_lo = q[13 + k], e_hi = q[17 + k];
+    if (w == k && e_hi > e_lo) {
+      if (PT == 6) tl_stream_ring<VT, XT, double, SQ, 1, 5, 2>(pack, val, x, e_lo, e_hi, TL_TG_BITS, acc, nullptr);
+      else if (PT == 5) tl_stream_ring<VT, XT, double, SQ, 1, 3, 1>(pack, val, x, e_lo, e_hi, TL_TG_BITS, acc, nullptr);
+      else tl_stream_ring<VT, XT, double, SQ, 1, 2, 0>(pack, val, x, e_lo, e_hi, TL_TG_BITS, acc, nullptr);
+    }
+    __syncthreads();
+#pragma unroll
+    for (int j = 0; j < NS; ++j) {
+      const int i = threadIdx.x + j * NW * 64;
+      tot[j] = k == 0 ? acc[i] : tot[j] + acc[i];
+      acc[i] = 0.0;
+    }
+    __syncthreads();
+  }
+#pragma unroll
+  for (int j = 0; j < NS; ++j) {
+    const int i = threadIdx.x + j * NW * 64, t = i >> TL_TG_SUB, c = i & (C - 1);
+    const int part = q[1 + t];
+    if (part >= 0) parts[(size_t)part * C + c] = tot[j];
+    else if (part == -1) {
+      const int col = ((q[0] + t) << TL_TG_SUB) + c;
+      if (col < dim) G[col] += tot[j];
+    }
+  }
+}
+
+template <typename VT, typename XT, bool SQ, int PT>
+__global__ __launch_bounds__(256, 5) void tl_tg_kernel(const int* __restrict__ groups,
+                                                     const uint32_t* __restrict__ pack, const VT* __restrict__ val,
+                                                     TLNarrow nar, const XT* __restrict__ x, double* __restrict__ G,
+                                                     int dim, double* __restrict__ parts,
+                                                     const unsigned char* __restrict__ live) {
+  __shared__ double acc[1 << TL_TG_BITS];
+  if (live && !live[blockIdx.x]) return;
+  tl_t_group<VT, XT, SQ, PT>(groups + TL_TG_COLS * blockIdx.x, pack, val, nar, x, G, dim, parts, acc);
+}
+
+template <typename VT, typename XT, bool SQ, int PT>
+__global__ __launch_bounds__(256, 5) void tl_tg_multi_kernel(const int* __restrict__ groups, int ngroups,
+                                                              const int* __restrict__ items,
+                                                              const unsigned long long* __restrict__ ptrs,
+                                                              const XT* __restrict__ x, double* __restrict__ G, int dim,
+                                                              double* __restrict__ parts,
+                                                              const unsigned char* __restrict__ live,
+                                                              const unsigned char* __restrict__ live_g,
+                                                              const int* __restrict__ gate) {
+  __shared__ double acc[1 << TL_TG_BITS];
+  if (gate && *gate == 0) return;
+  const int b = __builtin_amdgcn_readfirstlane(blockIdx.x);
+  if (b < ngroups) {
+    if (live_g && !live_g[b]) return;
+    const int* q = groups + TL_TG_COLS * b;
+    const unsigned long long* pc = ptrs + 6 * q[21];
+    const TLNarrow nar = {(const uint16_t*)pc[2], (const void*)pc[3], (const int*)pc[4], nullptr};
+    tl_t_group<VT, XT, SQ, PT>(q, (const uint32_t*)pc[0], (const VT*)pc[1], nar, x + q[22], G, dim, parts, acc);
+  } else {
+    if (live && !live[b - ngroups]) return;
+    const int* q = items + 8 * (b - ngroups);
+    const unsigned long long* pc = ptrs + 6 * q[0];
+    const TLNarrow nar = {(const uint16_t*)pc[2], (const void*)pc[3], (const int*)pc[4], (const int*)pc[5]};
+    tl_t_item<VT, XT, double, SQ, 1 << TL_TG_SUB, 2, 4, 3>(q[1], q[2], q[3], q[4], q[6], q[7], TL_TG_SUB,
+                                                         (const uint32_t*)pc[0], (const VT*)pc[1], nar, x + q[5], G,
+                                                         dim, parts, (double(*)[1 << TL_TG_SUB])acc);
+  }
+}
+
 __device__ __forceinline__ double rows_sum64(const double* __restrict__ src, int C, int r0, int r1, int c,
                                              double* sh) {
   const int w = threadIdx.x >> 6, lane = threadIdx.x & 63;
@@ -1229,6 +1316,8 @@
   TLNarrow nar;
   const unsigned char* live;
   const unsigned char* live_mt;
+  const int* groups; int ngroups;
+  const unsigned char* live_g;
 };
 struct TLTMultiDesc {
   const int* items; int nitems; int cbits; const unsigned long long* ptrs;
@@ -1236,6 +1325,8 @@
   const int* cu; int ncu; int nparts_total; int il;
   const unsigned char* live;
   const unsigned char* live_mt;
+  const int* groups; int ngroups;
+  const unsigned char* live_g;
 };
 
 static int g_ablate = 0;
@@ -1402,8 +1493,34 @@
   return 0;
 }
 
+#define TL_TG_P 3
+template <typename XT, typename F>
+static int tl_with_tg(int cbits, int il, F f) {
+  if constexpr (sizeof(XT) == 8) {
+    return -22;
+  } else {
+    if (cbits != TL_TG_SUB || !il) return -22;
+    if constexpr (TL_EXPERIMENT) {
+      if (g_tl_deep_t == 2) f(std::integral_constant<int, 6>{});
+      else if (g_tl_deep_t) f(std::integral_constant<int, 5>{});
+      else f(std::integral_constant<int, 3>{});
+    } else {
+      f(std::integral_constant<int, TL_TG_P>{});
+    }
+    return 0;
+  }
+}
+
 template <typename VT, typename XT, bool SQ>
 static int tl_t_impl(const TLTDesc* c, const void* x, double* G, double* parts, hipStream_t st) {
+  if (c->ngroups > 0) {
+    const int rt = tl_with_tg<XT>(c->cbits, c->il, [&](auto pt) {
+      hipLaunchKernelGGL((tl_tg_kernel<VT, XT, SQ, decltype(pt)::value>), dim3(c->ngroups), dim3(256), 0, st,
+                         c->groups, c->pack, (const VT*)c->val, c->nar, (const XT*)x, G, c->dim, parts, c->live_g);
+    });
+    if (rt) return rt;
+    LAUNCH_CHECK();
+  }
   if (c->nitems <= 0) return 0;
   const int rc = tl_with_acc<XT>(c->cbits, [&](auto acc) {
     tl_with_pipe<4, 1>(c->il, g_tl_waves_t, g_tl_deep_t, g_tl_pipe_t, [&](auto pipe) {
@@ -1420,6 +1537,16 @@
 
 template <typename VT, typename XT, bool SQ>
 static int tl_t_multi_impl(const TLTMultiDesc* c, const void* x, double* G, double* parts, hipStream_t st) {
+  if (c->ngroups > 0) {
+    const int rt = tl_with_tg<XT>(c->cbits, c->il, [&](auto pt) {
+      hipLaunchKernelGGL((tl_tg_multi_kernel<VT, XT, SQ, decltype(pt)::value>), dim3(c->ngroups + (c->nitems > 0 ? c->nitems : 0)),
+                         dim3(256), 0, st, c->groups, c->ngroups, c->items, c->ptrs, (const XT*)x, G, c->dim, parts,
+                         c->live, c->live_g, g_gate);
+    });
+    if (rt) return rt;
+    LAUNCH_CHECK();
+    return tl_t_combine(c, G, parts, st);
+  }
   if (c->nitems <= 0) return 0;
   const int rc = tl_with_acc<XT>(c->cbits, [&](auto acc) {
     tl_with_pipe<4, 2>(c->il, g_tl_waves_t, g_tl_deep_t, g_tl_pipe_t, [&](auto pipe) {
@@ -1568,6 +1695,7 @@
 static int tl_colstats_impl(const TLTDesc* c, double* const* sums, double* mx, double* mn, double* parts,
                             hipStream_t st) {
   if (c->cbits < 1 || c->cbits > (sizeof(VT) == 8 ? 11 : TL_MAXBITS)) return -22;
+  if (c->ngroups > 0) return -22;
   if (c->nitems <= 0) return 0;
   for (int which = 0; which < 4; ++which) {
     auto launch = [&](auto maxr, auto nw) {
diff --git a/photon_ml_amd/ops/device.py b/photon_ml_amd/ops/device.py
--- a/photon_ml_amd/ops/device.py
+++ b/photon_ml_amd/ops/device.py
@@ -13,7 +13,7 @@
 from ..data.matrix import LabeledData
 from .native import SegChunkDesc, check, require_glm_lib, stream_handle
 from .reference import GLMComputable
-from .tiled import DEFAULT_ITEM_ENTRIES, TLFwdChunk, TLTChunk, shard_tall, tl_supported
+from .tiled import DEFAULT_ITEM_ENTRIES, TLFwdChunk, TLTChunk, shard_tall, shard_tgroup, tl_supported
 from ..utils.timing import phase, trace_range
 
 H2D_GATE = threading.Event()
@@ -211,14 +211,31 @@
                     raise ValueError(f"chunk {c}: transpose item window outside the stream")
                 if int(it[:, 3].max()) >= max(t.nparts, 1) and t.nparts:
                     raise ValueError(f"chunk {c}: transpose partial-row slot out of range")
-                self._validate_narrow(c, t, it, m, "transpose")
+                self._validate_narrow(c, t, t.narrow_table().cpu(), m, "transpose")
                 tp, _ = t.logical()
                 q = tp.cpu().to(torch.int64) & 0xFFFFFFFF
                 if q.numel() and int((q >> t.cbits).max()) >= m:
                     raise ValueError(f"chunk {c}: transpose gather row >= chunk rows")
-                cols = (torch.repeat_interleave(it[:, 0], t.unit_counts().cpu()) << t.cbits) + (q & ((1 << t.cbits) - 1))
+                cols = ((torch.repeat_interleave(t.unit_tiles().cpu(), t.unit_counts().cpu()) << t.cbits)
+                        + (q & ((1 << t.cbits) - 1)))
                 if q.numel() and int(cols.max()) >= t.dim:
                     raise ValueError(f"chunk {c}: transpose column >= dim")
+            if getattr(t, "ngroups", 0):
+                g = t.groups.cpu().to(torch.int64)
+                if (int(g[:, 13:17].min()) < 0 or bool((g[:, 13:17] % 256 != 0).any())
+                        or int(((g[:, 17:21] + 255) // 256 * 256).max()) > t.pack.numel()
+                        or bool((g[:, 17:21] < g[:, 13:17]).any())):
+                    raise ValueError(f"chunk {c}: tile-group window outside the stream")
+                if int(g[:, 5:9].min()) < 0 or int(g[:, 9:13].max()) > t.nbase.numel() or bool(
+                        (g[:, 9:13] < g[:, 5:9]).any()):
+                    raise ValueError(f"chunk {c}: tile-group narrow rounds out of range")
+                if int(g[:, 0].min()) < 0 or ((int(g[:, 0].max()) + 4) << t.cbits) > ((t.dim + 1023) >> 10 << 10):
+                    raise ValueError(f"chunk {c}: tile group outside the column window")
+                if not t.nitems:
+                    self._validate_narrow(c, t, t.narrow_table().cpu(), m, "transpose")
+                    gp, _ = t.logical()
+                    if gp.numel() and int(((gp.cpu().to(torch.int64) & 0xFFFFFFFF) >> t.cbits).max()) >= m:
+                        raise ValueError(f"chunk {c}: transpose gather row >= chunk rows")
         if self.parts.numel() < max([c.parts_needed for c in self.csr + self.csc] + [1]):
             raise ValueError("partial-row scratch too small")
         self._validate_multi()
@@ -243,6 +260,14 @@
                 if ch.il and r.shape[0] and (int(r[:, 2].min()) < 0 or int((r[:, 2] + (r[:, 3] - r[:, 2] + 255) // 256 * 256).max())
                                    > ch.pack.numel() or int(r[:, 7].max()) > ch.nbase.numel() * (ch.n_narrow_rounds > 0)):
                     raise ValueError(f"chunk {c}: shard-wide transpose table outside the chunk's streams")
+            g = mt.groups.cpu().to(torch.int64)
+            for c, ch in enumerate(self.csc):
+                r = g[g[:, 21] == c]
+                if r.shape[0] and (int(r[:, 13:17].min()) < 0 or int(((r[:, 17:21] + 255) // 256 * 256).max()) > ch.pack.numel()
+                                   or int(r[:, 9:13].max()) > ch.nbase.numel() * (ch.n_narrow_rounds > 0)
+                                   or int(r[:, 1:5].max()) >= max(mt.nparts, 1)
+                                   or int(r[:, 22].min()) != self.row_starts[c] or int(r[:, 22].max()) != self.row_starts[c]):
+                    raise ValueError(f"chunk {c}: shard-wide tile-group table outside the chunk's streams")
 
     @staticmethod
     def _validate_narrow(c: int, ch, table: torch.Tensor, xlen: int, what: str):
@@ -326,7 +351,8 @@
                 col = torch.from_numpy(xc.indices.astype(np.int64)).to(dev)
                 val = torch.from_numpy(xc.data.astype(np.float64)).to(dev).to(vdt)
                 csr.append(TLFwdChunk(rp, col, val, dc, tall=shard_tall(dmax, min(chunk_rows, n))))
-                csc.append(TLTChunk(rp, col, val, dc, chunk_rows, cbits=cbits, item_entries=item_entries))
+                csc.append(TLTChunk(rp, col, val, dc, chunk_rows, cbits=cbits, item_entries=item_entries,
+                                    tgroup=shard_tgroup(dmax, n, chunk_rows)))
                 continue
             sp_ = (xc.indptr - xc.indptr[0]).astype(np.int32)
             csr.append(SegChunk(sp_, torch.from_numpy(xc.indices.astype(np.int32)),
@@ -385,7 +411,7 @@
     def from_device_csr(indptr: torch.Tensor, col: torch.Tensor, val: torch.Tensor, y, offsets, weights, dim: int,
                         device="cuda", precision: str = "f64", chunk_rows: int = 1 << 20,
                         item_entries: Optional[int] = None, col_windows: bool = False,
-                        tall: Optional[bool] = None):
+                        tall: Optional[bool] = None, tgroup: Optional[bool] = None):
         dev = torch.device(device)
         vdt = VAL_DTYPE[PRECISIONS[precision]]
         indptr = indptr.to(dev, torch.int64)
@@ -421,7 +447,8 @@
             v = val[ea:eb].to(dev).to(vdt)
             csr.append(TLFwdChunk(rp, c, v, hi - lo,
                                   tall=shard_tall(dmax, min(chunk_rows, n)) if tall is None else tall))
-            csc.append(TLTChunk(rp, c, v, hi - lo, chunk_rows, cbits=cbits, item_entries=item_entries))
+            csc.append(TLTChunk(rp, c, v, hi - lo, chunk_rows, cbits=cbits, item_entries=item_entries,
+                                tgroup=shard_tgroup(dmax, n, chunk_rows) if tgroup is None else tgroup))
             col_lo.append(lo)
             del c, v
         chunk_phase.__exit__(None, None, None)
@@ -448,11 +475,21 @@
             self._build_multi_t()
         frac = float(keep[:n].sum()) / max(n, 1)
         filt = frac < NARROW_FILTER_BELOW
+        csc, multi_t, grouped = self.csc, self._multi_t, any(getattr(ch, "ngroups", 0) for ch in self.csc)
+        if grouped:
+            if getattr(self, "_csc_plain", None) is None:
+                from .tiled import TLTMulti
+                plain = [ch.ungrouped() for ch in self.csc]
+                C = 1 << plain[0].cbits
+                self._csc_plain = (plain, None if self._multi_t is None else TLTMulti(
+                    plain, self.row_starts, self.dim,
+                    tile_offsets=[lo // C for lo in self.col_lo] if any(self.col_lo) else None))
+            csc, multi_t = self._csc_plain
         jobs = []
         for c in range(len(self.csr)):
             kc = keep[self.row_starts[c]: self.row_starts[c + 1]]
             jobs.append(RowCompaction(self.csr[c], kc, True, filt))
-            jobs.append(RowCompaction(self.csc[c], kc, False, filt))
+            jobs.append(RowCompaction(csc[c], kc, False, filt))
         sizes = torch.stack([torch.stack([j.total, j.kept]) for j in jobs]).tolist()
         out = [j.finish(int(t), int(k)) for j, (t, k) in zip(jobs, sizes)]
         view = DeviceGLMData(out[0::2], out[1::2], self.row_starts, self.y, self.o, self.wt, self.dim,
@@ -478,9 +515,9 @@
             view._multi_ptrs = stream_ptr_table(view.csr, self.device)
             view._multi = TLFwdMultiDesc(nb.data_ptr(), nb.shape[0], self._multi.rbits, view._multi_ptrs.data_ptr(),
                                          self._multi.il, tbits=self._multi.tbits)
-        view._multi_t = None if self._multi_t is None else self._multi_t.restreamed(view.csc)
+        view._multi_t = None if multi_t is None else multi_t.restreamed(view.csc)
         gb = getattr(self, "_gbuckets", None)
-        if gb is not None and gb[1] is not None:
+        if gb is not None and gb[1] is not None and not grouped:
             view._gbuckets = (gb[0], [(mt.restreamed(view.csc), c0, c1) for mt, c0, c1 in gb[1]])
         view.parts = self.parts
         if os.environ.get("PML_CHECK_KERNEL_INPUTS", "0") == "1":
@@ -914,7 +951,12 @@
             for t in (ch.items[: ch.nitems, 0].to(torch.int64), ch.mt_tiles[: ch.nmt].to(torch.int64)):
                 firsts.append(col_entity[(self.col_lo[c] + t * C).clamp(0, nc - 1)])
                 lasts.append(col_entity[torch.clamp(self.col_lo[c] + (t + 1) * C - 1, max=hi).clamp(0, nc - 1)])
-            i_off.append(i_off[-1] + int(ch.nitems) + int(ch.nmt))
+            ng = int(getattr(ch, "ngroups", 0))
+            if ng:
+                t = ch.groups[:, 0].to(torch.int64)
+                firsts.append(col_entity[(self.col_lo[c] + t * C).clamp(0, nc - 1)])
+                lasts.append(col_entity[torch.clamp(self.col_lo[c] + (t + 4) * C - 1, max=hi).clamp(0, nc - 1)])
+            i_off.append(i_off[-1] + int(ch.nitems) + int(ch.nmt) + ng)
             m_off.append(i_off[-2] + int(ch.nitems))
         t0, t1 = torch.cat(firsts), torch.cat(lasts)
         self._mgeo = (f0, f1, f_off, t0, t1, i_off, m_off)
@@ -945,6 +987,7 @@
             d = dup(ch.desc)
             d.live = live_t.data_ptr() + i_off[c]
             d.live_mt = live_t.data_ptr() + m_off[c + 1]
+            d.live_g = live_t.data_ptr() + m_off[c + 1] + int(ch.nmt)
             tdescs.append(d)
         self._masked = (fdesc, tdescs, keep)
         if MASK_STATS is not None:
@@ -966,8 +1009,16 @@
         for ch in self.csc:
             it = ch.items[: ch.nitems].cpu().numpy().astype(np.int64)
             np.add.at(work, it[:, 0], it[:, 2] - it[:, 1])
+            if getattr(ch, "ngroups", 0):
+                g = ch.groups.cpu().numpy().astype(np.int64)
+                np.add.at(work, g[:, 0], (g[:, 17:21] - g[:, 13:17]).sum(1))
         cum = np.cumsum(work)
         cuts = [0] + [int(np.searchsorted(cum, cum[-1] * k / nb, side="right")) for k in range(1, nb)] + [ntiles]
+        if any(getattr(ch, "ngroups", 0) for ch in self.csc):
+            if any((lo // C) % 4 for lo in self.col_lo):
+                self._gbuckets = (nb, None)
+                return None
+            cuts = [c if c == ntiles else c - c % 4 for c in cuts]
         cuts = sorted(set(min(max(c, 0), ntiles) for c in cuts))
         out = []
         for t0, t1 in zip(cuts[:-1], cuts[1:]):
@@ -1223,7 +1274,7 @@
                 torch.full((self.dim,), float("-inf"), dtype=torch.float64, device=self.device),
                 torch.full((self.dim,), float("inf"), dtype=torch.float64, device=self.device)]
         for c, ch in enumerate(self.csc):
-            tl_colstats(self.prec, ch, self.col_lo[c], outs, self.parts)
+            tl_colstats(self.prec, ch.ungrouped(cache=False), self.col_lo[c], outs, self.parts)
         return tuple(self._unperm(t) for t in outs)
 
     def margins(self, w, margin_shift: float = 0.0, with_offsets: bool = False):
diff --git a/photon_ml_amd/ops/native.py b/photon_ml_amd/ops/native.py
--- a/photon_ml_amd/ops/native.py
+++ b/photon_ml_amd/ops/native.py
@@ -42,7 +42,8 @@
 class TLTMultiDesc(ctypes.Structure):
     _fields_ = [("items", c_void_p), ("nitems", c_int), ("cbits", c_int), ("ptrs", c_void_p),
                 ("mt_tiles", c_void_p), ("mt_ptr", c_void_p), ("nmt", c_int), ("dim", c_int), ("cu", c_void_p),
-                ("ncu", c_int), ("nparts_total", c_int), ("il", c_int), ("live", c_void_p), ("live_mt", c_void_p)]
+                ("ncu", c_int), ("nparts_total", c_int), ("il", c_int), ("live", c_void_p), ("live_mt", c_void_p),
+                ("groups", c_void_p), ("ngroups", c_int), ("live_g", c_void_p)]
 
 
 class CmpArgs(ctypes.Structure):
@@ -71,6 +72,7 @@
         ("mt_tiles", c_void_p), ("mt_ptr", c_void_p), ("nmt", c_int), ("dim", c_int),
         ("cu", c_void_p), ("ncu", c_int), ("nparts_total", c_int), ("il", c_int), ("nar", TLNarrow),
         ("live", c_void_p), ("live_mt", c_void_p),
+        ("groups", c_void_p), ("ngroups", c_int), ("live_g", c_void_p),
     ]
 
 
diff --git a/photon_ml_amd/ops/tiled.py b/photon_ml_amd/ops/tiled.py
--- a/photon_ml_amd/ops/tiled.py
+++ b/photon_ml_amd/ops/tiled.py
@@ -50,6 +50,13 @@
 TALL_SUB_BITS = 10
 TALL_MIN_DIM = 1 << 16
 TALL_COLS = 10
+TGROUP_DEFAULT = True
+TG_MIN_CHUNKS = 96
+TG_BITS = 12
+TG_SUB_BITS = 10
+TG_MIN_DIM = 1 << 16
+TG_COLS = 24
+TG_EMPTY = -2
 
 
 def narrow_width(sbits: int) -> int:
@@ -252,6 +259,21 @@
     if tall is None:
         tall = TALL_DEFAULT and dim >= TALL_MIN_DIM and m >= (1 << TALL_BITS)
     return bool(tall)
+
+
+def tgroup_engages(tgroup: Optional[bool], dim: int, chunk_rows: int, dtype, il: int, cbits: int) -> bool:
+    if not (il and NARROW and dtype != torch.float64 and cbits == TG_SUB_BITS
+            and _bits(chunk_rows) + TG_BITS <= 32):
+        return False
+    if tgroup is None and os.environ.get("PML_TL_TGROUP") is not None:
+        tgroup = bool(int(os.environ["PML_TL_TGROUP"]))
+    return bool(tgroup)
+
+
+def shard_tgroup(dim: int, n_rows: int, chunk_rows: int) -> Optional[bool]:
+    if os.environ.get("PML_TL_TGROUP") is not None:
+        return None
+    return bool(TGROUP_DEFAULT and dim >= TG_MIN_DIM and n_rows >= TG_MIN_CHUNKS * chunk_rows)
 
 
 def shard_tall(dim: int, chunk_rows: int) -> Optional[bool]:
@@ -455,10 +477,12 @@
     kind = "tl"
 
     def __init__(self, rowptr: torch.Tensor, col: torch.Tensor, val: torch.Tensor, dim: int, chunk_rows: int,
-                 cbits: Optional[int] = None, item_entries: Optional[int] = None, il: Optional[int] = None):
+                 cbits: Optional[int] = None, item_entries: Optional[int] = None, il: Optional[int] = None,
+                 tgroup: Optional[bool] = None):
         self.il = INTERLEAVE if il is None else int(il)
         if item_entries is None:
             item_entries = int(os.environ.get("PML_TL_ITEM_ENTRIES", DEFAULT_ITEM_ENTRIES))
+        self._chunk_rows, self._item_entries = chunk_rows, item_entries
         dev = val.device
         rowptr = rowptr.to(dev, torch.int64)
         col = col.to(dev, torch.int64)
@@ -506,17 +530,44 @@
         items = np.column_stack([it_tile, lo, hi, part_of]).astype(np.int64).reshape(-1, 4)
         items = np.column_stack([items, np.zeros((len(items), 2), np.int64)])
         self._sbits, self._ew = self.cbits, (1, 2)
+        gsel = np.zeros(len(items), dtype=bool)
+        gok = np.zeros(0, dtype=bool)
+        if len(items) and ntiles >= 4 and tgroup_engages(tgroup, dim, max(chunk_rows, m), val.dtype, self.il,
+                                                          self.cbits):
+            k_of_tile = np.zeros(ntiles, np.int64)
+            k_of_tile[nz] = n_it
+            gok = k_of_tile[: (ntiles >> 2) << 2].reshape(-1, 4).max(1) == 1
+            g_of_item = items[:, 0] >> 2
+            gsel = (g_of_item < len(gok)) & gok[np.minimum(g_of_item, len(gok) - 1)]
+        groups = np.zeros((0, TG_COLS), np.int64)
         if self.il:
             cnt = torch.from_numpy(items[:, 2] - items[:, 1]).to(dev)
             wp, wv, wn, npk, nvl, nbs, nr = split_narrow(pack.to(torch.int64) & 0xFFFFFFFF, val, cnt, self.cbits, m)
             del pack, val
-            self.pack, self.val, new_lo = _interleave(_to_u32_bits(wp), wv, wn)
-            del wp, wv
-            items[:, 1] = new_lo.cpu().numpy()
-            items[:, 2] = items[:, 1] + wn.cpu().numpy()
             nr = nr.cpu().numpy()
             items[:, 5] = np.cumsum(nr)
             items[:, 4] = items[:, 5] - nr
+            if gsel.any():
+                wp, wv, wn, gcnt = self._merge_groups(wp, wv, wn, items[:, 0], gsel, len(gok))
+                gidx = np.flatnonzero(gok)
+                groups = np.zeros((len(gidx), TG_COLS), np.int64)
+                it_of_tile = np.full(ntiles, -1, np.int64)
+                it_of_tile[items[gsel, 0]] = np.flatnonzero(gsel)
+                it4 = it_of_tile[gidx[:, None] * 4 + np.arange(4)[None, :]]
+                groups[:, 0] = gidx * 4
+                groups[:, 1:5] = np.where(it4 >= 0, -1, TG_EMPTY)
+                groups[:, 5:9] = np.where(it4 >= 0, items[it4, 4], 0)
+                groups[:, 9:13] = np.where(it4 >= 0, items[it4, 5], 0)
+                items = items[~gsel]
+            self.pack, self.val, new_lo = _interleave(_to_u32_bits(wp), wv, wn)
+            del wp, wv
+            new_lo, wn = new_lo.cpu().numpy(), wn.cpu().numpy()
+            items[:, 1] = new_lo[: len(items)]
+            items[:, 2] = items[:, 1] + wn[: len(items)]
+            if len(groups):
+                groups[:, 13:17] = new_lo[len(items):].reshape(-1, 4)
+                groups[:, 17:21] = groups[:, 13:17] + wn[len(items):].reshape(-1, 4)
+            self.nitems = len(items)
         else:
             self.pack, self.val = _pad(pack), _pad(val.contiguous())
             npk, nvl, nbs = _empty_narrow(val)
@@ -527,9 +578,47 @@
         self.mt_ptr = torch.tensor(np.asarray(mt_ptr, dtype=np.int32), device=dev)
         self.cu = torch.tensor(np.asarray(cu if len(cu) else [(0, 0, 0)], dtype=np.int32).reshape(-1, 3), device=dev)
         self.m, self.nnz, self.dim = m, nnz, dim
+        self.ngroups = len(groups)
+        self.groups = torch.tensor(groups.astype(np.int32), device=dev).reshape(-1, TG_COLS)
+        self._make_desc()
+
+    def _make_desc(self):
         self.desc = TLTDesc(self.items.data_ptr(), self.nitems, self.cbits, self.pack.data_ptr(),
-                            self.val.data_ptr(), self.mt_tiles.data_ptr(), self.mt_ptr.data_ptr(), self.nmt, dim,
-                            self.cu.data_ptr(), self.ncu, self.nparts, self.il, self.nar)
+                            self.val.data_ptr(), self.mt_tiles.data_ptr(), self.mt_ptr.data_ptr(), self.nmt, self.dim,
+                            self.cu.data_ptr(), self.ncu, self.nparts, self.il, self.nar,
+                            groups=self.groups.data_ptr() if self.ngroups else None, ngroups=self.ngroups)
+
+    @staticmethod
+    def _merge_groups(wp, wv, wn, tile_of_item, gsel, ngroups_all):
+        dev = wp.device
+        S, T = TG_SUB_BITS, TG_BITS
+        gs = torch.from_numpy(gsel).to(dev)
+        n_items = wn.numel()
+        tot = int(wn.sum())
+        item = torch.repeat_interleave(torch.arange(n_items, device=dev), wn, output_size=tot)
+        eg = gs[item]
+        it_g = item[eg]
+        j = torch.arange(tot, device=dev)[eg] - (torch.cumsum(wn, 0) - wn)[it_g]
+        del item
+        nrw = (wn + IL_ROUND - 1) // IL_ROUND
+        quarter = (4 * (j // IL_ROUND) + 3) // nrw[it_g]
+        tile = torch.from_numpy(np.ascontiguousarray(tile_of_item)).to(dev)[it_g]
+        del j, it_g
+        p = wp[eg]
+        p12 = ((p >> S) << T) | ((tile & 3) << S) | (p & ((1 << S) - 1))
+        win = (tile >> 2) * 4 + quarter
+        del p, tile, quarter
+        skey = (win << 32) | p12
+        order = torch.sort(skey, stable=True).indices
+        del skey
+        gp, gv = p12[order], wv[eg][order]
+        bounds = torch.searchsorted(win[order].contiguous(), torch.arange(4 * ngroups_all + 1, device=dev))
+        wcnt = (bounds[1:] - bounds[:-1]).view(-1, 4)
+        gok = torch.zeros(ngroups_all, dtype=torch.bool, device=dev)
+        gok[torch.from_numpy(np.unique(tile_of_item[gsel] >> 2)).to(dev)] = True
+        gcnt = wcnt[gok].reshape(-1)
+        keep = ~eg
+        return (torch.cat([wp[keep], gp]), torch.cat([wv[keep], gv]), torch.cat([wn[~gs], gcnt]), gcnt)
 
     @property
     def parts_needed(self) -> int:
@@ -540,7 +629,66 @@
 
     def nbytes(self) -> int:
         return sum(t.numel() * t.element_size() for t in (self.items, self.mt_tiles, self.mt_ptr, self.cu, self.pack,
-                                                           self.val, self.npack, self.nval, self.nbase))
+                                                           self.val, self.npack, self.nval, self.nbase, self.groups))
+
+    def unit_tiles(self) -> torch.Tensor:
+        t = self.items[:, 0].to(torch.int64)
+        if not self.ngroups:
+            return t
+        g0 = self.groups[:, 0].to(torch.int64)
+        return torch.cat([t, (g0[:, None] + torch.arange(4, device=t.device)[None, :]).reshape(-1)])
+
+    def unit_counts(self) -> torch.Tensor:
+        c = super().unit_counts()
+        if not self.ngroups:
+            return c
+        return torch.cat([c, self._group_units()[3]])
+
+    def narrow_table(self) -> torch.Tensor:
+        t = self.items[: self.nitems].to(torch.int64)
+        if not self.ngroups:
+            return t
+        g = self.groups.to(torch.int64)
+        gt = torch.zeros((4 * g.shape[0], 6), dtype=torch.int64, device=t.device)
+        gt[:, 0] = (g[:, :1] + torch.arange(4, device=t.device)[None, :]).reshape(-1)
+        gt[:, 4], gt[:, 5] = g[:, 5:9].reshape(-1), g[:, 9:13].reshape(-1)
+        gt = gt[g[:, 1:5].reshape(-1) != TG_EMPTY]
+        allt = torch.cat([t[:, :6], gt])
+        return allt[torch.sort(allt[:, 0], stable=True).indices]
+
+    @property
+    def n_narrow_rounds(self) -> int:
+        g = self.groups.to(torch.int64)
+        return _NarrowMixin.n_narrow_rounds.fget(self) + (int((g[:, 9:13] - g[:, 5:9]).sum()) if self.ngroups else 0)
+
+    def _group_units(self):
+        if getattr(self, "_gunits", None) is not None:
+            return self._gunits
+        S, T = TG_SUB_BITS, TG_BITS
+        g = self.groups.to(torch.int64)
+        dev = g.device
+        G = g.shape[0]
+        wcnt = (g[:, 17:21] - g[:, 13:17]).reshape(-1)
+        ph = il_phys(g[:, 13:17].reshape(-1), wcnt).to(self.pack.device)
+        wp = (self.pack[ph].to(torch.int64) & 0xFFFFFFFF).to(dev)
+        wv = self.val[ph].to(dev)
+        gw = torch.repeat_interleave(torch.arange(4 * G, device=dev), wcnt) >> 2
+        unit_w = gw * 4 + ((wp >> S) & 3)
+        wp = ((wp >> T) << S) | (wp & ((1 << S) - 1))
+        n_lo, nn = g[:, 5:9].reshape(-1), (g[:, 9:13] - g[:, 5:9]).reshape(-1) * IL_ROUND
+        if int(nn.sum()):
+            npk, nvl = narrow_logical(self.npack, self.nval, self.nbase, 0, int(g[:, 9:13].max()), S)
+            unit_n = torch.repeat_interleave(torch.arange(4 * G, device=dev), nn)
+            pos = n_lo[unit_n] * IL_ROUND + torch.arange(int(nn.sum()), device=dev) - (torch.cumsum(nn, 0) - nn)[unit_n]
+            unit = torch.cat([unit_n, unit_w])
+            order = torch.sort(unit, stable=True).indices
+            unit, pk, vl = unit[order], torch.cat([npk[pos], wp])[order], torch.cat([nvl[pos], wv])[order]
+        else:
+            order = torch.sort(unit_w, stable=True).indices
+            unit, pk, vl = unit_w[order], wp[order], wv[order]
+        b = torch.searchsorted(unit.contiguous(), torch.arange(4 * G + 1, device=dev))
+        self._gunits = (unit, pk, vl, b[1:] - b[:-1])
+        return self._gunits
 
     def window(self, e_lo: int, e_hi: int):
         if not self.il:
@@ -552,13 +700,38 @@
         if not self.il:
             return self.pack[: self.nnz], self.val[: self.nnz]
         ph = il_phys(self.items[:, 1], self.items[:, 2] - self.items[:, 1])
-        return self._logical_all(self.pack[ph], self.val[ph])
+        pk, vl = self._logical_all(self.pack[ph], self.val[ph])
+        if not self.ngroups:
+            return pk, vl
+        _, gp, gv, _ = self._group_units()
+        return torch.cat([pk.to(torch.int64) & 0xFFFFFFFF, gp]), torch.cat([vl, gv])
+
+    def coo(self):
+        pk, vl = self.logical()
+        p = pk.to(torch.int64) & 0xFFFFFFFF
+        tile = torch.repeat_interleave(self.unit_tiles(), self.unit_counts())
+        key = ((p >> self.cbits) << 32) | (tile << self.cbits) | (p & ((1 << self.cbits) - 1))
+        key, order = torch.sort(key, stable=True)
+        return key >> 32, key & 0xFFFFFFFF, vl[order]
+
+    def ungrouped(self, cache: bool = True) -> "TLTChunk":
+        if not self.ngroups:
+            return self
+        twin = getattr(self, "_ungrouped", None)
+        if twin is None:
+            row, col, val = self.coo()
+            rowptr = torch.searchsorted(row.contiguous(), torch.arange(self.m + 1, device=row.device))
+            twin = TLTChunk(rowptr, col, val, self.dim, self._chunk_rows, cbits=self.cbits,
+                            item_entries=self._item_entries, il=self.il, tgroup=False)
+            if cache:
+                self._ungrouped = twin
+        return twin
 
     def emulate_rmatvec(self, r: torch.Tensor, square: bool = False) -> torch.Tensor:
         pk, vl = self.logical()
         p = pk.to(torch.int64) & 0xFFFFFFFF
         row = p >> self.cbits
-        tile_of_entry = torch.repeat_interleave(self.items[:, 0].to(torch.int64), self.unit_counts())
+        tile_of_entry = torch.repeat_interleave(self.unit_tiles(), self.unit_counts())
         col = (tile_of_entry << self.cbits) + (p & ((1 << self.cbits) - 1))
         v = vl.to(torch.float64)
         if square:
@@ -577,17 +750,36 @@
         self.il = chunks[0].il
         if any(ch.il != self.il for ch in chunks):
             raise ValueError("TLTMulti: chunks mix interleaved and plain streams")
-        its = []
+        its, grps = [], []
+        n_grp = 0
         for c, ch in enumerate(chunks):
             it = ch.items[: ch.nitems].cpu().numpy().astype(np.int64).reshape(-1, 6)
             toff = 0 if tile_offsets is None else int(tile_offsets[c])
             its.append(np.column_stack([np.full(len(it), c), it[:, 0] + toff, it[:, 1], it[:, 2],
-                                        np.full(len(it), row_starts[c]), it[:, 4], it[:, 5]]))
-        it = np.concatenate(its) if its else np.zeros((0, 7), np.int64)
-        src_all = np.arange(len(it))
+                                        np.full(len(it), row_starts[c]), it[:, 4], it[:, 5], np.full(len(it), -1)]))
+            if getattr(ch, "ngroups", 0):
+                g = ch.groups.cpu().numpy().astype(np.int64).reshape(-1, TG_COLS).copy()
+                g[:, 0] += toff
+                g[:, 21], g[:, 22], g[:, 23] = c, row_starts[c], np.arange(len(g))
+                gi, k = np.nonzero(g[:, 1:5] != TG_EMPTY)
+                z = np.zeros(len(gi), np.int64)
+                its.append(np.column_stack([z + c, g[gi, 0] + k, z, z, z + row_starts[c], z, z,
+                                            4 * (n_grp + gi) + k]))
+                grps.append(g)
+                n_grp += len(g)
+        it = np.concatenate(its) if its else np.zeros((0, 8), np.int64)
+        grp = np.concatenate(grps) if grps else np.zeros((0, TG_COLS), np.int64)
+        real = it[:, 7] < 0
+        src_all = np.cumsum(real) - 1
         if tile_range is not None:
             in_range = (it[:, 1] >= tile_range[0]) & (it[:, 1] < tile_range[1])
+            gin = np.zeros(len(grp), np.int64)
+            np.add.at(gin, it[~real, 7] >> 2, np.where(in_range[~real], 1, 1 << 20))
+            if np.any((gin % (1 << 20) > 0) & (gin >= (1 << 20))):
+                raise ValueError("TLTMulti: tile_range cuts a tile group (round the range to multiples of 4 tiles)")
             it = it[in_range]
+            src_all = src_all[in_range]
+            real = real[in_range]
         n = len(it)
         tile = it[:, 1]
         order = np.lexsort((np.arange(n), tile))
@@ -604,10 +796,17 @@
         u_tile = np.repeat(np.arange(len(km)), nu)
         u_first = np.repeat(plo, nu) + np.repeat(sg, nu) * (np.arange(int(nu.sum())) - np.repeat(np.cumsum(nu) - nu, nu))
         u_last = np.minimum(u_first + np.repeat(sg, nu), np.repeat(plo + km, nu))
-        self.nitems, self.nparts, self.ncu, self.nmt = n, int(km.sum()), int(nu.sum()), len(km)
+        self.nparts, self.ncu, self.nmt = int(km.sum()), int(nu.sum()), len(km)
+        slot = it[~real, 7]
+        grp[slot >> 2, 1 + (slot & 3)] = part[~real]
+        used = np.zeros(len(grp), dtype=bool)
+        used[slot >> 2] = True
+        grp = grp[used]
+        it, part, src = it[real], part[real], src_all[real]
+        n = len(it)
+        self.nitems, self.ngroups = n, len(grp)
         rows = np.column_stack([it[:, 0], it[:, 1], it[:, 2], it[:, 3], part, it[:, 4], it[:, 5],
                                 it[:, 6]]).astype(np.int32)
-        src = src_all if tile_range is None else src_all[in_range]
         if XCD_GROUPS > 1 and n > XCD_GROUPS:
             xo = xcd_order(it[:, 0], XCD_GROUPS)
             rows, src = rows[xo], src[xo]
@@ -619,9 +818,11 @@
                                if self.ncu else np.zeros((1, 3), np.int32), device=dev)
         self.ptrs = stream_ptr_table(chunks, dev)
         self._chunks = list(chunks)
+        self.groups = torch.tensor(grp.astype(np.int32), device=dev).reshape(-1, TG_COLS)
         self.desc = TLTMultiDesc(self.items.data_ptr(), n, self.cbits, self.ptrs.data_ptr(),
                                  self.mt_tiles.data_ptr(), self.mt_ptr.data_ptr(), self.nmt, dim,
-                                 self.cu.data_ptr(), self.ncu, self.nparts, self.il)
+                                 self.cu.data_ptr(), self.ncu, self.nparts, self.il,
+                                 groups=self.groups.data_ptr() if self.ngroups else None, ngroups=self.ngroups)
 
     @property
     def parts_needed(self) -> int:
@@ -630,8 +831,10 @@
     def restreamed(self, chunks: Sequence["TLTChunk"]) -> "TLTMulti":
         import copy
         from .native import TLTMultiDesc
+        if self.ngroups or any(getattr(ch, "ngroups", 0) for ch in chunks):
+            raise ValueError("TLTMulti.restreamed: row-sampled copies are made of chunks without tile groups")
         dev = self.items.device
-        cat = torch.cat([ch.items[: ch.nitems].to(torch.int64) for ch in chunks]) if chunks else None
+        cat =torch.cat([ch.items[: ch.nitems].to(torch.int64) for ch in chunks]) if chunks else None
         rows = self.items.to(torch.int64).clone()
         if self.nitems:
             sel = cat[self._src]
@@ -666,6 +869,23 @@
                 G[tile * C:(tile + 1) * C] += acc
             else:
                 parts[part] = acc
+        for g in self.groups.cpu().tolist():
+            ch = self._chunks[g[21]]
+            unit, pk, vl, cnt = ch._group_units()
+            ends = torch.cumsum(cnt, 0).cpu().tolist()
+            for k in range(4):
+                part, u = g[1 + k], 4 * g[23] + k
+                if part == TG_EMPTY:
+                    continue
+                p = pk[ends[u] - int(cnt[u]):ends[u]].cpu()
+                v = vl[ends[u] - int(cnt[u]):ends[u]].cpu().to(torch.float64)
+                if square:
+                    v = v * v
+                acc = torch.zeros(C, dtype=torch.float64).index_add_(0, p & (C - 1), v * r[g[22] + (p >> self.cbits)])
+                if part < 0:
+                    G[(g[0] + k) * C:(g[0] + k + 1) * C] += acc
+                else:
+                    parts[part] = acc
         cu = self.cu.cpu().tolist()
         l1 = [parts[a:b].sum(0) for _, a, b in cu[: self.ncu]]
         mp = self.mt_ptr.cpu().tolist()
@@ -715,6 +935,8 @@
         from .native import CmpArgs, check, require_game_lib, stream_handle
         if not ch.il:
             raise ValueError("row-sampled copies need the interleaved layout")
+        if getattr(ch, "ngroups", 0):
+            raise ValueError("row-sampled copies are made of a transpose chunk's ungrouped() copy")
         self.ch, self.keep, self.forward = ch, keep, forward
         dev = ch.pack.device
         self.filter_narrow = bool(filter_narrow)
diff --git a/photon_ml_amd/ops/warmup.py b/photon_ml_amd/ops/warmup.py
--- a/photon_ml_amd/ops/warmup.py
+++ b/photon_ml_amd/ops/warmup.py
@@ -44,6 +44,11 @@
     tiny.matvec(torch.zeros(5, dtype=torch.float64, device=dev))
     z = torch.zeros(8, dtype=torch.float64, device=dev)
     tiny._fwd(0, torch.zeros(5, dtype=torch.float32, device=dev), 0, 0, 0.0, None, None, z_out=z, stats=False)
+    tiny = DeviceGLMData.from_device_csr(torch.arange(0, 18, 2, device=dev), (i[:16] * 512) % 4096,
+                                         x[:16].to(torch.float32), torch.zeros(8), torch.zeros(8), torch.ones(8), 4096,
+                                         dev, "f32", tgroup=True)
+    tiny.rmatvec(torch.zeros(8, dtype=torch.float64, device=dev), build_multi=False)
+    tiny.rmatvec(torch.zeros(8, dtype=torch.float64, device=dev))
     key_histogram(i % 13, 13)
     csr_gather_rows(torch.tensor([0, 2], dtype=torch.int64, device=dev), i[:2], x[:2],
                     torch.zeros(1, dtype=torch.int64, device=dev), torch.tensor([0, 4], dtype=torch.int64, device=dev))
```

Result: faster. 3.737 billion examples/sec, median of 6 (+1.9%).
